# wzx99/DCFP

Measured on AMD Instinct MI355X. Metric: training images/sec at 1024x2048 DeepLabv3-R101, higher is better.
Workload: dtype f32; 1 GPU; DeepLabv3-resnet101+ASPP os8, 4x3x1024x2048 per GPU, CE+0.4*deepsup CE (fused upsample), 3x3 stride-1 convs with >= 256 channels as fp32 Winograd F(2x2,3x3) (fwd / dgrad / wgrad), all other convs direct implicit GEMM, EIC step, SGD m0.9 wd5e-4; global_batch=4, parallelism=dp1

## Files before the change

### dcfp_amd/_lib.py

```python
import ctypes as C
import os
import subprocess
import threading

_HERE = os.path.dirname(os.path.abspath(__file__))
LIB_PATH = os.environ.get("DCFP_LIB") or os.path.join(_HERE, "libdcfp_hip.so")
CSRC = os.path.join(_HERE, "csrc")

_lib = None
_lock = threading.Lock()


class ConvDesc(C.Structure):
    _fields_ = [(n, C.c_int32) for n in
                ("N", "Cin", "H", "W", "Cout", "KH", "KW", "stride", "pad", "dil", "Hout", "Wout",
                 "x_pitch", "dy_pitch")]


class ConvF16Desc(C.Structure):
    _fields_ = [(n, C.c_int32) for n in
                ("N", "H", "W", "Cin8", "x_pitch", "Cout", "K", "stride", "pad", "dil", "Hout", "Wout",
                 "y_pitch", "y_off", "res_pitch", "res_off", "relu")]


class ConvF8Desc(C.Structure):
    _fields_ = [(n, C.c_int32) for n in
                ("N", "H", "W", "Cin16", "x_pitch", "Cout", "K", "stride", "pad", "dil", "Hout", "Wout",
                 "y_pitch", "y_off", "res_pitch", "res_off", "relu")] + [("res_mul", C.c_float)]


class EicEntry(C.Structure):
    _fields_ = [("gamma", C.c_void_p), ("grad", C.c_void_p), ("eic", C.c_void_p),
                ("n", C.c_int32), ("pad_", C.c_int32)]


class SgdEntry(C.Structure):
    _fields_ = [("param", C.c_void_p), ("grad", C.c_void_p), ("momentum_buf", C.c_void_p),
                ("n", C.c_int64), ("first_chunk", C.c_int64),
                ("weight_decay", C.c_float), ("pad_", C.c_int32)]


class GateEntry(C.Structure):
    _fields_ = [("gamma", C.c_void_p), ("beta", C.c_void_p), ("ggrad", C.c_void_p), ("bgrad", C.c_void_p),
                ("score", C.c_void_p), ("n", C.c_int32), ("pad_", C.c_int32)]


class FilterEntry(C.Structure):
    _fields_ = [("w", C.c_void_p), ("g", C.c_void_p), ("out", C.c_void_p), ("rows", C.c_int32), ("K", C.c_int32),
                ("first_unit", C.c_int64)]


class FpgmEntry(C.Structure):
    _fields_ = [("w", C.c_void_p), ("out", C.c_void_p), ("C", C.c_int32), ("K", C.c_int32),
                ("first_tile", C.c_int64), ("ws_off", C.c_int64)]


class AdamEntry(C.Structure):
    _fields_ = [("param", C.c_void_p), ("grad", C.c_void_p), ("exp_avg", C.c_void_p), ("exp_avg_sq", C.c_void_p),
                ("n", C.c_int64), ("first_chunk", C.c_int64)]


class BnRunning(C.Structure):
    _fields_ = [("running_mean", C.c_void_p), ("running_var", C.c_void_p), ("num_batches_tracked", C.c_void_p),
                ("momentum", C.c_float), ("pad_", C.c_int32)]


class WpEntry(C.Structure):
    _fields_ = [("w", C.c_void_p), ("wp", C.c_void_p), ("first_block", C.c_int64), ("n_blocks", C.c_int64)] + \
               [(n, C.c_int32) for n in ("T", "Ck", "CkP", "M", "Mpad", "sAm", "sAc", "perm8")]


class AugTap(C.Structure):
    _fields_ = [(n, C.c_int32) for n in ("src", "c0", "c1", "lsrc")]


class AugSample(C.Structure):
    _fields_ = [("image", C.c_void_p), ("label", C.c_void_p)] + \
               [(n, C.c_int32) for n in ("src_h", "src_w", "col_off", "row_off", "lut_a_off", "lut_b_off",
                                         "hsv_flags", "hue_delta")] + \
               [("sat_alpha", C.c_float), ("pad_", C.c_int32)]


class CcSample(C.Structure):
    _fields_ = [("label", C.c_void_p)] + \
               [(n, C.c_int32) for n in ("src_h", "src_w", "dst_h", "dst_w", "Hp", "Wp", "row_off", "col_off", "cls",
                                         "pad_")] + \
               [("work_off", C.c_int64)]


class VoteMap(C.Structure):
    _fields_ = [("logits", C.c_void_p)] + [(n, C.c_int32) for n in ("h", "w", "hs", "ws", "flip")] + \
               [("weight", C.c_float)]


class SlidePass(C.Structure):
    _fields_ = [("logits", C.c_void_p)] + \
               [(n, C.c_int32) for n in ("lh", "lw", "hs", "ws", "th", "tw", "rows", "cols", "flip")] + \
               [("weight", C.c_float)]


class EngineInfo(C.Structure):
    _fields_ = [(n, C.c_int32) for n in ("format", "num_classes", "in_channels", "align_corner", "model", "n_records",
                                         "n_buffers", "n_slots", "has_input_table")]


SLIDE_MAX_PASSES, SLIDE_MAX_TILES_PER_AXIS = 16, 32
AUG_SATURATION, AUG_HUE = 1, 2
SGD_CHUNK = 16384
FILTER_ABS_SUM, FILTER_L2, FILTER_DOT_SQ_ACC = 0, 1, 2
FPGM_TILE = 64
CONV_FWD, CONV_DGRAD, CONV_WGRAD = 0, 1, 2
E_BADDESC, E_UNSUPPORTED, E_WORKSPACE = -1, -2, -3

_P, _I, _L, _F, _Z = C.c_void_p, C.c_int, C.c_int64, C.c_float, C.c_size_t
_D = C.POINTER(ConvDesc)
_R = C.POINTER(BnRunning)
_H = C.POINTER(ConvF16Desc)
_H8 = C.POINTER(ConvF8Desc)

SIGNATURES = {
    "dcfp_abi_version": (_I, []),
    "dcfp_conv2d_workspace_bytes": (_Z, [_D, _I]),
    "dcfp_conv2d_wp_layout": (_I, [_D, _I, C.POINTER(WpEntry)]),
    "dcfp_conv2d_permute_weights_multi_f32": (_I, [_P, _I, _L, _P]),
    "dcfp_conv2d_pitch_supported": (_I, [_D]),
    "dcfp_conv2d_kernel_name": (_I, [_D, _I, C.c_char_p, _I]),
    "dcfp_conv2d_executed_fraction": (C.c_double, [_D, _I]),
    "dcfp_conv2d_workspace_is_scratch": (_I, [_D, _I]),
    "dcfp_conv2d_dgrad_fanin_supported": (_I, [_D]),
    "dcfp_conv2d_dgrad_fanin_f32_nchw": (_I, [_D, _P, _L, _P, _P, _P, _P, _P, _Z, _I, _P]),
    "dcfp_conv2d_dgrad_fanin_red_slots": (_L, [_D]),
    "dcfp_conv2d_dgrad_fanin_red_f32_nchw": (_I, [_D, _P, _L, _P, _P, _P, _P, _P, _P, _P, _P, _P, _Z, _I, _P]),
    "dcfp_bn_bwd_sums_from_partials_f32": (_I, [_P, _L, _I, _P, _F, _P, _P, _P, _P, _P]),
    "dcfp_conv2d_xform_bytes": (_Z, [_D]),
    "dcfp_conv2d_fwd_keep_f32_nchw": (_I, [_D, _P, _P, _P, _L, _P, _Z, _P, _P, _Z, _P]),
    "dcfp_conv2d_wgrad_kept_f32_nchw": (_I, [_D, _P, _L, _P, _Z, _P, _P, _Z, _P]),
    "dcfp_conv2d_fwd_f32_nchw": (_I, [_D, _P, _P, _P, _P, _L, _P, _Z, _I, _P]),
    "dcfp_conv2d_fwd_fused_f32_nchw": (_I, [_D, _P, _P, _P, _P, _P, _I, _P, _P, _Z, _I, _P]),
    "dcfp_conv2d_dgrad_f32_nchw": (_I, [_D, _P, _L, _P, _P, _I, _P, _Z, _I, _P]),
    "dcfp_conv2d_wgrad_f32_nchw": (_I, [_D, _P, _L, _P, _P, _P, _P, _Z, _P]),
    "dcfp_bn_workspace_bytes": (_Z, [_I, _I, _I]),
    "dcfp_bn_stats_f32": (_I, [_P, _L, _I, _I, _I, _P, _P, _R, _P, _Z, _P]),
    "dcfp_bn_apply_f32": (_I, [_P, _P, _P, _P, _P, _F, _P, _I, _P, _L, _I, _I, _I, _I, _I, _P]),
    "dcfp_bn_bwd_reduce_f32": (_I, [_P, _L, _P, _P, _L, _P, _P, _P, _P, _F, _I, _I, _I, _I, _P, _P, _P, _P,
                                    _P, _Z, _P]),
    "dcfp_bn_update_running_f32": (_I, [_P, _P, _I, _F, _F, _P, _P, _P, _P]),
    "dcfp_syncbn_combine_f32": (_I, [_P, _I, _I, _P, _P, _P, _R, _P]),
    "dcfp_syncbn_p2p_mailbox_bytes": (_Z, [_I, _I]),
    "dcfp_p2p_alloc": (_I, [_Z, _I, C.POINTER(C.c_void_p)]),
    "dcfp_p2p_free": (_I, [_P]),
    "dcfp_p2p_export": (_I, [_P, _P]),
    "dcfp_p2p_import": (_I, [_P, C.POINTER(C.c_void_p)]),
    "dcfp_p2p_unmap": (_I, [_P]),
    "dcfp_syncbn_p2p_exchange_f32": (_I, [C.POINTER(C.c_void_p), _I, _I, C.c_uint32, _I, _P, _I, _I, _P, _R,
                                          C.c_uint32, _P, _P]),
    "dcfp_bn_apply_relu_mask_f32": (_I, [_P, _P, _P, _P, _P, _F, _P, _P, _P, _I, _I, _I, _P]),
    "dcfp_conv2d_fwd_stat_slots": (_L, [_D, _P, _L]),
    "dcfp_conv2d_fwd_stats_f32_nchw": (_I, [_D, _P, _P, _P, _L, _P, _P, _Z, _I, _P]),
    "dcfp_bn_stats_from_partials_f32": (_I, [_P, _L, _I, _I, _P, _P, _R, _P]),
    "dcfp_bn_bwd_apply_f32": (_I, [_P, _L, _P, _P, _L, _P, _P, _P, _P, _F, _P, _P, _F, _P, _I, _P, _P,
                                   _I, _I, _I, _I, _I, _P]),
    "dcfp_bn_bwd_fused_sync_bytes": (_Z, [_I, _I, _I]),
    "dcfp_bn_bwd_fused_f32": (_I, [_P, _L, _P, _P, _L, _P, _P, _P, _P, _F, _F, _I, _P, _P, _I, _I, _I, _I, _I,
                                   _P, _P, _P, _P, _P, _Z, C.c_uint32, C.c_uint32, _P, _P]),
    "dcfp_maxpool3x3s2_fwd_f32": (_I, [_P, _P, _P, _I, _I, _I, _I, _I, _I, _P]),
    "dcfp_maxpool3x3s2_bwd_f32": (_I, [_P, _P, _P, _I, _I, _I, _I, _I, _I, _P]),
    "dcfp_rowsum_f32": (_I, [_P, _L, _P, _F, _I, _I, _I, _P]),
    "dcfp_broadcast_hw_f32": (_I, [_P, _F, _P, _L, _I, _I, _I, _I, _P]),
    "dcfp_add_f32": (_I, [_P, _P, _P, _L, _P]),
    "dcfp_channel_scale_f32": (_I, [_P, _P, _P, _I, _I, _I, _P]),
    "dcfp_upsample_bilinear_fwd_f32": (_I, [_P, _P, _I, _I, _I, _I, _I, _I, _I, _P]),
    "dcfp_upsample_bilinear_bwd_f32": (_I, [_P, _P, _I, _I, _I, _I, _I, _I, _I, _P]),
    "dcfp_resize_bilinear_into_f32": (_I, [_P, _L, _I, _I, _I, _I, _P, _L, _I, _I, _I, _I, _P]),
    "dcfp_resize_bilinear_adjoint_f32": (_I, [_P, _L, _I, _I, _I, _I, _I, _P, _L, _I, _I, _I, _I, _P]),
    "dcfp_ppm_pool_f32": (_I, [_P, _I, _I, _I, _I, _I, _P, _P, _I, _P, _L, _I, _P]),
    "dcfp_ppm_pool_adjoint_f32": (_I, [_P, _I, _I, _I, _I, _I, _P, _P, _L, _I, _P, _P]),
    "dcfp_ppm_resize_adjoint_f32": (_I, [_P, _L, _I, _I, _I, _I, _I, _P, _P, _I, _P]),
    "dcfp_upsample_ce_workspace_bytes": (_Z, [_I, _I, _I]),
    "dcfp_upsample_ce_fwd_f32": (_I, [_P, _P, _P, _I, _I, _I, _I, _I, _I, _I, _I, _P, _P, _P, _P,
                                      _Z, _P]),
    "dcfp_upsample_ce_bwd_f32": (_I, [_P, _P, _P, _I, _I, _I, _I, _I, _I, _I, _I, _P, _P, _P, _P]),
    "dcfp_upsample_ce_bwd_plan": (_I, [_I, _I, _I, _I, _I, _I, C.POINTER(C.c_int), C.POINTER(C.c_int),
                                       C.POINTER(C.c_int)]),
    "dcfp_ohem_zoom_gt_prob_f32": (_I, [_P, _P, _P, _I, _I, _I, _I, _I, _I, _I, _I, _I, _P, _P, _P]),
    "dcfp_ohem_threshold_f32": (_I, [_P, _P, _L, _I, _F, _L, _P, _P]),
    "dcfp_ohem_keep_mask_u8": (_I, [_P, _P, _L, _P, _P]),
    "dcfp_upsample_margin_f32": (_I, [_P, _I, _I, _I, _I, _I, _I, _I, _P, _P]),
    "dcfp_maxfilter2d_s1_f32": (_I, [_P, _P, _I, _I, _I, _I, _P]),
    "dcfp_upsample_wce_workspace_bytes": (_Z, [_I, _I, _I]),
    "dcfp_upsample_wce_fwd_f32": (_I, [_P, _P, _P, _I, _I, _I, _I, _I, _I, _I, _I, _P, _P, _P, _Z, _P]),
    "dcfp_upsample_wce_bwd_f32": (_I, [_P, _P, _P, _I, _I, _I, _I, _I, _I, _I, _I, _P, _P, _P, _P]),
    "dcfp_upsample_argmax_f32": (_I, [_P, _I, _I, _I, _I, _I, _I, _I, _P, _P]),
    "dcfp_confusion_matrix_i64": (_I, [_P, _P, _I, _L, _I, _P, _P]),
    "dcfp_vote_multiscale_f32": (_I, [C.POINTER(VoteMap), _I, _I, _I, _I, _I, _I, _I, _I, _P, _P, _P, _I, _P, _P]),
    "dcfp_gather_tiles_f32": (_I, [_P, _I, _I, _I, _I, _P, _I, _P, _I, _I, _I, _I, _P, _P]),
    "dcfp_vote_sliding_f32": (_I, [C.POINTER(SlidePass), _I, _P, _P, _I, _I, _I, _I, _I, _I, _I, _P, _P, _P, _I, _P, _P]),
    "dcfp_label_boundary_workspace_bytes": (_Z, [_I, _I, _I]),
    "dcfp_label_boundary_i32": (_I, [_P, _P, _I, _I, _I, _I, _I, _I, _P, _Z, _P]),
    "dcfp_label_boundary_i64": (_I, [_P, _P, _I, _I, _I, _I, _I, _I, _P, _Z, _P]),
    "dcfp_png_deflate_bound": (_Z, [_I, _I]),
    "dcfp_png_deflate_workspace_bytes": (_Z, [_I, _I, _I, _I]),
    "dcfp_png_deflate_labels_i32": (_I, [_P, _I, _I, _I, _P, _I, _P, _Z, _P, _P, _P, _Z, _P]),
    "dcfp_augment_u8_to_f32_nchw": (_I, [C.POINTER(AugSample), _I, _I, _I, _P, _L, _P, _L, _P, _L, _P, _I, _P, _P, _P, _P]),
    "dcfp_balance_weight_f32": (_I, [_P, _P, _P, _I, _L, _I, _I, _I, C.c_double, _P, _P]),
    "dcfp_components_workspace_bytes": (_Z, [_I, _I]),
    "dcfp_label_components_u8": (_I, [C.POINTER(CcSample), _I, _P, _L, _P, _P, _Z, _P, _P]),
    "dcfp_component_pixel_i32": (_I, [C.POINTER(CcSample), _I, _P, _Z, _P, _P, _P, _P, _P]),
    "dcfp_eic_update_f32": (_I, [_P, _I, _F, _F, _P]),
    "dcfp_sgd_momentum_f32": (_I, [_P, _I, _L, _F, _F, _I, _P]),
    "dcfp_adamw_f32": (_I, [_P, _I, _L, _F, _F, _F, _F, _F, _F, _F, _P]),
    "dcfp_conv2d_fwd_f16_nhwc": (_I, [_H, _P, _P, _P, _P, _P, _P]),
    "dcfp_conv2d_fwd_f16_nhwc_to_f32_nchw": (_I, [_H, _P, _P, _P, _P, _P]),
    "dcfp_maxpool3x3s2_nhwc_f16": (_I, [_P, _P, _I, _I, _I, _I, _I, _I, _I, _I, _P]),
    "dcfp_avgpool_nhwc_f16_workspace_bytes": (_Z, [_I, _I, _L]),
    "dcfp_avgpool_nhwc_f16": (_I, [_P, _P, _I, _L, _I, _I, _I, _P, _Z, _P]),
    "dcfp_broadcast_nhwc_f16": (_I, [_P, _I, _P, _I, _L, _I, _I, _I, _P]),
    "dcfp_nchw_f32_to_nhwc_f16": (_I, [_P, _P, _I, _I, _I, _I, _I, _P]),
    "dcfp_conv2d_fwd_f8_nhwc": (_I, [_H8, _P, _P, _P, _P, _P, _P, _P]),
    "dcfp_conv2d_fwd_f8_nhwc_to_f32_nchw": (_I, [_H8, _P, _P, _P, _P, _P, _P]),
    "dcfp_cast_nhwc_f16_to_f8": (_I, [_P, _I, _P, _I, _I, _L, _I, _F, _P]),
    "dcfp_maxpool3x3s2_nhwc_f8": (_I, [_P, _P, _I, _I, _I, _I, _I, _I, _I, _I, _P]),
    "dcfp_avgpool_nhwc_f8_to_f16": (_I, [_P, _P, _I, _L, _I, _I, _I, _F, _P, _Z, _P]),
    "dcfp_broadcast_nhwc_f16_to_f8": (_I, [_P, _I, _P, _I, _L, _I, _I, _I, _F, _P]),
    "dcfp_resize_bilinear_nhwc_f16": (_I, [_P, _I, _I, _I, _I, _I, _P, _I, _I, _I, _I, _I, _P]),
    "dcfp_pyramid_pool_nhwc_f16_workspace_bytes": (_Z, [_I, _I, _I, _I, _I, _P]),
    "dcfp_pyramid_pool_nhwc_f16": (_I, [_P, _I, _I, _I, _I, _I, _I, _I, _P, _P, _P, _P, _Z, _P]),
    "dcfp_kd_workspace_bytes": (_Z, [_I, _I, _I, _I, _I]),
    "dcfp_kd_fwd_f32": (_I, [_P, _P, _I, _I, _I, _I, _I, _F, _P, _Z, _P, _P, _P]),
    "dcfp_pairwise_workspace_bytes": (_Z, [_I, _I, _I, _I, _I, _I, _I]),
    "dcfp_pairwise_fwd_f32": (_I, [_P, _P, _I, _L, _I, _I, _I, _I, _I, _I, _P, _Z, _P, _I, _P]),
    "dcfp_pairwise_bwd_f32": (_I, [_I, _I, _I, _I, _I, _I, _P, _Z, _P, _P, _P]),
    "dcfp_lovasz_workspace_bytes": (_Z, [_I, _I]),
    "dcfp_lovasz_hist_f32": (_I, [_P, _P, _I, _I, _I, _I, _I, _I, _I, _I, _I, _P, _P, _Z, _P]),
    "dcfp_lovasz_scan_f32": (_I, [_I, _I, _P, _Z, _P, _P, _P]),
    "dcfp_lovasz_bwd_f32": (_I, [_P, _P, _I, _I, _I, _I, _I, _I, _I, _I, _I, _P, _P, _P, _P, _P, _P]),
    "dcfp_lovasz_errors_u32": (_I, [_P, _P, _I, _I, _I, _I, _I, _I, _I, _I, _P, _P]),
    "dcfp_gate_taylor_f32": (_I, [_P, _I, _P]),
    "dcfp_gate_l1reg_f32": (_I, [_P, _I, _F, _P]),
    "dcfp_filter_reduce_units": (_L, [_I, _I]),
    "dcfp_filter_reduce_f32": (_I, [_P, _I, _L, _I, _P]),
    "dcfp_fpgm_workspace_bytes": (_Z, [_I]),
    "dcfp_fpgm_f32": (_I, [_P, _I, _L, _P, _Z, _P]),
    "dcfp_engine_open": (_I, [C.c_char_p, C.POINTER(_P), C.c_char_p, _Z]),
    "dcfp_engine_open_memory": (_I, [_P, _Z, C.POINTER(_P), C.c_char_p, _Z]),
    "dcfp_engine_close": (None, [_P]),
    "dcfp_engine_info": (_I, [_P, C.POINTER(EngineInfo)]),
    "dcfp_engine_weight_bytes": (_Z, [_P]),
    "dcfp_engine_upload": (_I, [_P, _P, _P]),
    "dcfp_engine_output_shape": (_I, [_P, _I, _I, _I, C.POINTER(_I), C.POINTER(_I), C.POINTER(_I)]),
    "dcfp_engine_buffer_shapes": (_I, [_P, _I, _I, C.POINTER(_I), _I]),
    "dcfp_engine_workspace_bytes": (_Z, [_P, _I, _I, _I]),
    "dcfp_engine_run_f32": (_I, [_P, _P, _P, _I, _I, _I, _P, _Z, _P, _P]),
    "dcfp_engine_run_u8": (_I, [_P, _P, _P, _Z, _I, _I, _I, _P, _Z, _P, _P]),
    "dcfp_image_u8_hwc_to_nhwc_f16": (_I, [_P, _Z, _I, _I, _I, _P, C.POINTER(_I), _P, _I, _P]),
}


def build(verbose=False):
    cmd = ["make", "-C", CSRC, "-j", str(min(8, os.cpu_count() or 1))]
    r = subprocess.run(cmd, capture_output=True, text=True)
    if verbose or r.returncode != 0:
        print(r.stdout[-4000:])
        print(r.stderr[-4000:])
    if r.returncode != 0:
        raise RuntimeError("building libdcfp_hip.so failed")
    return LIB_PATH


def lib():
    global _lib
    if _lib is not None:
        return _lib
    with _lock:
        if _lib is not None:
            return _lib
        if not os.path.exists(LIB_PATH):
            raise RuntimeError(
                f"{LIB_PATH} not found: run `python -c 'import __graft_entry__ as g; g.build()'` "
                "(or `make -C dcfp_amd/csrc`). dcfp_amd has no non-HIP fallback.")
        try:
            import torch
        except Exception:
            pass
        handle = C.CDLL(LIB_PATH, mode=C.RTLD_GLOBAL)
        for name, (res, args) in SIGNATURES.items():
            fn = getattr(handle, name)
            fn.restype = res
            fn.argtypes = args
        _lib = handle
    return _lib


def check(status, what):
    if status != 0:
        kind = "descriptor/shape" if status < 0 else "hipError_t"
        raise RuntimeError(f"{what} failed: status {status} ({kind})")
```

### dcfp_amd/csrc/conv_dispatch.h

```cpp
#pragma once
#include "common.h"
#include <stdlib.h>
#include <string.h>

struct Igemm2Params;

inline int check_desc(const DcfpConvDesc* d) {
    if (!d) return DCFP_E_BADDESC;
    if (d->N <= 0 || d->Cin <= 0 || d->Cout <= 0 || d->H <= 0 || d->W <= 0 || d->stride <= 0 ||
        d->dil <= 0 || d->pad < 0)
        return DCFP_E_BADDESC;
    if (d->KH != d->KW || (d->KH != 1 && d->KH != 3)) return DCFP_E_UNSUPPORTED;
    const int ho = (d->H + 2 * d->pad - d->dil * (d->KH - 1) - 1) / d->stride + 1;
    const int wo = (d->W + 2 * d->pad - d->dil * (d->KW - 1) - 1) / d->stride + 1;
    if (ho != d->Hout || wo != d->Wout || ho <= 0 || wo <= 0) return DCFP_E_BADDESC;
    if ((d->x_pitch != 0 && (d->x_pitch < d->W || (d->x_pitch & 3))) ||
        (d->dy_pitch != 0 && (d->dy_pitch < d->Wout || (d->dy_pitch & 3))))
        return DCFP_E_BADDESC;
    if ((long long)d->Cin * d->H * (d->x_pitch ? d->x_pitch : d->W) >= (1LL << 29) ||
        (long long)d->Cout * d->Hout * (d->dy_pitch ? d->dy_pitch : d->Wout) >= (1LL << 29) ||
        (long long)d->Cout * d->Cin * d->KH * d->KW >= (1LL << 29))
        return DCFP_E_UNSUPPORTED;
    return DCFP_OK;
}

inline bool same_size_3x3(const DcfpConvDesc* d) {
    return d->KH == 3 && d->KW == 3 && d->stride == 1 && d->pad == d->dil && d->Hout == d->H && d->Wout == d->W;
}

inline bool math_bf16x3() {
    static const bool v = [] { const char* e = getenv("DCFP_CONV_MATH"); return e && !strcmp(e, "bf16x3"); }();
    return v;
}
inline int conv_winograd_mode() {
    static const int v = [] { const char* e = getenv("DCFP_CONV_WINOGRAD"); return e ? atoi(e) : 1; }();
    return v;
}
inline bool igemm_dma_on() {
    static const bool v = [] { const char* e = getenv("DCFP_IGEMM_DMA"); return !e || atoi(e) != 0; }();
    return v;
}
inline int igemm_2d_mode() {
    static const int v = [] { const char* e = getenv("DCFP_IGEMM_2D"); return e ? atoi(e) : 5; }();
    return v;
}
inline int wino_fused_mode() {
    static const int v = [] { const char* e = getenv("DCFP_WINO_FUSED"); return e ? atoi(e) : 1; }();
    return v;
}
inline int wino_wgrad_fused_mode() {
    static const int v = [] { const char* e = getenv("DCFP_WINO_WGRAD_FUSED"); return e ? atoi(e) : 1; }();
    return v;
}
inline bool wgrad_dma_on() {
    static const bool v = [] { const char* e = getenv("DCFP_WGRAD_DMA"); return !e || atoi(e) != 0; }();
    return v;
}

struct GemmProblem {
    int T, M, Ck, N, Hi, Wi, Ho, Wo, sn, sd, off0, offstep;
    int in_pitch;
    int sAm, sAc;
    long long in_nstride, out_nstride;
    int P() const { return Ho * Wo; }
    long long px() const { return (long long)N * Ho * Wo; }
    int HiWi() const { return Hi * Wi; }
    bool pitched() const { return in_pitch > 0 && in_pitch != Wi; }
};

inline GemmProblem gemm_problem(const DcfpConvDesc* d, int pass, long long nstride_override) {
    GemmProblem g;
    g.T = d->KH * d->KW; g.N = d->N;
    if (pass == DCFP_CONV_FWD) {
        g.M = d->Cout; g.Ck = d->Cin; g.Hi = d->H; g.Wi = d->W; g.Ho = d->Hout; g.Wo = d->Wout;
        g.sn = d->stride; g.sd = 1; g.off0 = -d->pad; g.offstep = d->dil;
        g.in_pitch = d->x_pitch; g.sAm = d->Cin * g.T; g.sAc = g.T;
        g.in_nstride = (long long)d->Cin * d->H * (d->x_pitch ? d->x_pitch : d->W);
        g.out_nstride = nstride_override ? nstride_override : (long long)d->Cout * d->Hout * d->Wout;
    } else {
        g.M = d->Cin; g.Ck = d->Cout; g.Hi = d->Hout; g.Wi = d->Wout; g.Ho = d->H; g.Wo = d->W;
        g.sn = 1; g.sd = d->stride; g.off0 = d->pad; g.offstep = -d->dil;
        g.in_pitch = d->dy_pitch; g.sAm = g.T; g.sAc = d->Cin * g.T;
        g.in_nstride = nstride_override ? nstride_override
                                        : (long long)d->Cout * d->Hout * (d->dy_pitch ? d->dy_pitch : d->Wout);
        g.out_nstride = (long long)d->Cin * d->H * d->W;
    }
    return g;
}

struct WinoProblem {
    int N, H, W, d, M, Ck;
    long long in_nstride;
    int in_pitch;
};
inline WinoProblem wino_problem(const GemmProblem& g) {
    return {g.N, g.Ho, g.Wo, g.offstep < 0 ? -g.offstep : g.offstep, g.M, g.Ck, g.in_nstride, g.in_pitch};
}

struct GemmExtras {
    const float* bias = nullptr;
    const float* scale = nullptr;
    const float* shift = nullptr;
    const float* residual = nullptr;
    int relu = 0;
    float* stat_part = nullptr;
    int accumulate = 0;
    int wp_valid = 0;
    long long wp_nstride = 0;
    const float* fan_src = nullptr;
    const unsigned long long* fan_mask = nullptr;
    const Igemm2Red* red = nullptr;
    float* xform_out = nullptr;
};

enum Igemm2Family { IGEMM2_TILE, IGEMM2_DMA, IGEMM2_DMA1P, IGEMM2_DMA8 };
struct Igemm2Route {
    int family;
    int cfg, bm, bn;
    bool dma_shape;
    bool mixed;
    int Mpad, CkP, tile2d;
    int tiles_per_img, tiles_n_total, tiles_m;
    int Hc, Wc, tiles_per_phase, zfold;
};
Igemm2Route igemm2_route(const GemmProblem& g, const GemmExtras& x, bool vec_store);
int dcfp_igemm2_run(const GemmProblem& g, const float* in, const float* w, float* out, void* workspace, size_t workspace_bytes,
                    const GemmExtras& x, hipStream_t stream);
size_t dcfp_igemm2_workspace_bytes(const GemmProblem& g);
int dcfp_igemm2_cfg_id(const GemmProblem& g);
const char* dcfp_igemm2_cfg_args(const GemmProblem& g);
bool dcfp_igemm2_dma_shape(const GemmProblem& g);
bool dcfp_igemm2_use_dma8(const GemmProblem& g);
double dcfp_igemm2_exec_fraction(const GemmProblem& g);
void dcfp_igemm2_wp_layout(const GemmProblem& g, DcfpWpEntry* e);
long long dcfp_igemm2_stat_slots(const GemmProblem& g, const float* out);
bool dcfp_igemm2_persist();
int dcfp_igemm2_ck_pad();
int dcfp_igemm2_permute_multi(const DcfpWpEntry* table, int n, long long total_blocks, hipStream_t stream);
int dcfp_igemm2n_launch(const Igemm2Params& p, int T, hipStream_t stream);
int dcfp_igemm2p_launch(const Igemm2Params& p, hipStream_t stream);
bool dcfp_igemm2p_fan_red_ok(int Mpad, int CkP);

size_t dcfp_igemm3_workspace_bytes(int T, int M, int Ck);
int dcfp_igemm3_run(const GemmProblem& g, const float* in, const float* w, float* out, void* workspace, size_t workspace_bytes,
                    const GemmExtras& x, hipStream_t stream);

bool dcfp_wino_ok(const WinoProblem& q);
size_t dcfp_wino_workspace_bytes(const WinoProblem& q);
double dcfp_wino_exec_fraction(const WinoProblem& q);
long long dcfp_wino_stat_slots(const WinoProblem& q);
size_t dcfp_wino_xform_bytes(const WinoProblem& q);
int dcfp_wino_run(const GemmProblem& g, const float* in, const float* w, float* out, void* workspace, size_t workspace_bytes,
                  const GemmExtras& x, hipStream_t stream);
bool dcfp_wino_fused_ok(const WinoProblem& q);
size_t dcfp_wino_fused_workspace_bytes(const WinoProblem& q);
void dcfp_wino_fused_pads(const WinoProblem& q, int* CkP, int* Mpad);
int dcfp_wino_fused_run(const GemmProblem& g, const float* in, const float* w, float* out, void* workspace,
                        size_t workspace_bytes, const GemmExtras& x, hipStream_t stream);
bool dcfp_wino_wgrad_ok(int N, int H, int W, int d, int M, int C);
size_t dcfp_wino_wgrad_workspace_bytes(int N, int H, int W, int d, int M, int C);
int dcfp_wino_wgrad_run(const float* dy, long long dy_nstride, int dy_pitch, const float* x, long long x_nstride,
                        int x_pitch, float* dw, int N, int M, int C, int H, int W, int d, void* workspace,
                        size_t workspace_bytes, hipStream_t stream, const float* xform_in);
bool dcfp_wino_wgrad_fused_ok(int N, int H, int W, int d, int M, int C, long long x_nstride, int x_pitch,
                              long long dy_nstride, int dy_pitch);
size_t dcfp_wino_wgrad_fused_workspace_bytes(int N, int H, int W, int d, int M, int C);
int dcfp_wino_wgrad_fused_run(const float* dy, long long dy_nstride, int dy_pitch, const float* x, long long x_nstride,
                              int x_pitch, float* dw, int N, int M, int C, int H, int W, int d, void* workspace,
                              size_t workspace_bytes, hipStream_t stream);

bool dcfp_stem_shape(const DcfpConvDesc* d);
long long dcfp_stem_stat_slots(const DcfpConvDesc* d, const float* y, long long y_nstride);
int dcfp_stem_fwd(const DcfpConvDesc* d, const float* x, const float* w, float* y, long long y_nstride, const GemmExtras& ex,
                  hipStream_t stream);
size_t dcfp_stem_wgrad_workspace_bytes(const DcfpConvDesc* d);
int dcfp_stem_wgrad(const DcfpConvDesc* d, const float* dy, long long dy_nstride, const float* x, float* dw, void* workspace,
                    size_t workspace_bytes, hipStream_t stream);
bool dcfp_gemv_shape(const DcfpConvDesc* d);
int dcfp_gemv_fwd(const DcfpConvDesc* d, const float* x, const float* w, const float* bias, float* y, long long y_nstride,
                  hipStream_t stream);
int dcfp_gemv_dgrad(const DcfpConvDesc* d, const float* dy, long long dy_nstride, const float* w, float* dx, int accumulate,
                    hipStream_t stream);
int dcfp_gemv_wgrad(const DcfpConvDesc* d, const float* dy, long long dy_nstride, const float* x, float* dw, hipStream_t stream);

int dcfp_wgrad_kernel_name(const DcfpConvDesc* d, char* buf, int buf_len);
double dcfp_wgrad_exec_fraction(const DcfpConvDesc* d);
bool dcfp_wgrad_is_winograd(const DcfpConvDesc* d);
bool dcfp_wgrad_wants_xform(const DcfpConvDesc* d);
bool dcfp_wgrad_pitch_ok(const DcfpConvDesc* d);
size_t dcfp_wgrad_batched_workspace_bytes(int batch, int M, int C, long long K, int* splits_out);
int dcfp_wgrad_batched_run(const float* a, const float* bmat, float* out, int batch, int M, int C, long long K,
                           void* workspace, size_t workspace_bytes, hipStream_t stream);
int dcfp_wgrad3_launch(const float* dy, long long dy_nstride, const float* x, long long x_nstride,
                       float* out, int N, int M, int Cin, int T, int H, int W, int Ho, int Wo, int pad,
                       int dil, int Kpix, int kchunk, int splits, int tiles_m, int tiles_n,
                       hipStream_t stream);
size_t dcfp_conv2d_fwd_dgrad_workspace_bytes_(const DcfpConvDesc* d, int pass);
```

### dcfp_amd/csrc/conv_igemm.hip

```cpp
#include "conv_dispatch.h"
#include <stdio.h>

extern "C" int dcfp_abi_version(void) { return 2; }

static bool igemm3_ok(const GemmProblem& g) {
    return math_bf16x3() && g.sn == 1 && g.sd == 1 && dcfp_igemm2_cfg_id(g) == 4;
}

static int wino_kind(const DcfpConvDesc* d, int pass) {
    const int mode = conv_winograd_mode();
    if (mode == 0 || !same_size_3x3(d) || math_bf16x3()) return 0;
    const bool fwd = pass == DCFP_CONV_FWD;
    const GemmProblem g = gemm_problem(d, pass, 0);
    const WinoProblem q = wino_problem(g);
    const int M = g.M, Ck = g.Ck;
    const bool three = dcfp_wino_ok(q), fused = dcfp_wino_fused_ok(q);
    if (!three && !fused) return 0;
    if (mode == 2) return three ? 1 : 2;
    const double nominal = 2.0 * d->N * (double)d->H * d->W * (double)M * Ck * 9.0;
    const double f_direct = dcfp_igemm2_exec_fraction(g);
    const double t_direct = nominal * f_direct / (M % 256 != 0 ? 115e12 : 143e12);
    const double f_wino = dcfp_wino_exec_fraction(q);
    double t_wino = 1e30;
    if (three) {
        const double tiles = f_wino * 9.0 / 16.0 * d->N * (double)d->H * d->W;
        const double rate = Ck <= 256 ? (M >= 1024 ? 130e12 : 118e12) : (M <= 256 ? 127e12 : 135e12);
        const double pix = (double)d->N * d->H * d->W;
        const double t_in = (4.0 * pix * Ck + 64.0 * tiles * Ck) / 4.2e12;
        const double t_out = (64.0 * tiles * M + 4.0 * pix * M * (fwd ? 1.0 : 2.0)) / 5.4e12;
        const double mpad = (double)((M + 255) / 256 * 256) / M;
        t_wino = nominal * f_wino * mpad / rate + t_in + t_out + 20e-6;
    }
    if (fused) {
        const double nk = (double)((Ck + 15) / 16 * 2);
        const double mpad = (double)((M + 63) / 64 * 64) / M;
        const double t_f = nominal * f_wino * mpad / (125e12 * nk / (nk + 4.0)) + 10e-6;
        if (t_f < t_wino) t_wino = t_f;
    }
    if (!(t_wino < 0.97 * t_direct)) return 0;
    return three ? 1 : 2;
}
static bool wino_pass(const DcfpConvDesc* d, int pass) { return wino_kind(d, pass) != 0; }

static bool wino_keeps_u(const DcfpConvDesc* d, int pass) {
    static const bool on = [] { const char* e = getenv("DCFP_WINO_KEEP_U"); return !e || atoi(e) != 0; }();
    if (!on || (pass != DCFP_CONV_FWD && pass != DCFP_CONV_DGRAD) || !wino_pass(d, pass)) return false;
    const WinoProblem q = wino_problem(gemm_problem(d, pass, 0));
    if (!dcfp_wino_fused_ok(q)) return false;
    if (pass == DCFP_CONV_FWD && q.Ck > 256 && dcfp_wino_ok(q) && dcfp_conv2d_xform_bytes(d) > 0) return false;
    return true;
}

extern "C" int dcfp_conv2d_workspace_is_scratch(const DcfpConvDesc* d, int pass) {
    if (check_desc(d) != DCFP_OK || pass == DCFP_CONV_WGRAD) return 0;
    return (wino_pass(d, pass) && !wino_keeps_u(d, pass)) ? 1 : 0;
}

size_t dcfp_conv2d_fwd_dgrad_workspace_bytes_(const DcfpConvDesc* d, int pass) {
    if (check_desc(d) != DCFP_OK) return 0;
    const GemmProblem g = gemm_problem(d, pass, 0);
    if (const int wk = wino_kind(d, pass)) {
        const WinoProblem q = wino_problem(g);
        if (wino_keeps_u(d, pass)) {
            const size_t u = dcfp_wino_fused_workspace_bytes(q), direct = dcfp_igemm2_workspace_bytes(g);
            return u > direct ? u : direct;
        }
        return wk == 1 ? dcfp_wino_workspace_bytes(q) : dcfp_wino_fused_workspace_bytes(q);
    }
    const size_t b2 = dcfp_igemm2_workspace_bytes(g);
    const size_t b3 = igemm3_ok(g) ? dcfp_igemm3_workspace_bytes(g.T, g.M, g.Ck) : 0;
    return b2 > b3 ? b2 : b3;
}

extern "C" int dcfp_conv2d_kernel_name(const DcfpConvDesc* d, int pass, char* buf, int buf_len) {
    int rc = check_desc(d);
    if (rc) return rc;
    if (!buf || buf_len <= 0) return DCFP_E_BADDESC;
    if (dcfp_gemv_shape(d)) return snprintf(buf, buf_len, "gemv_1x1_map_kernel");
    if (pass == DCFP_CONV_WGRAD) return dcfp_wgrad_kernel_name(d, buf, buf_len);
    if (pass == DCFP_CONV_FWD && dcfp_stem_shape(d)) return snprintf(buf, buf_len, "stem_fwd_kernel");
    if (const int wk = wino_kind(d, pass))
        return wk == 1 ? snprintf(buf, buf_len, "winograd_f2x2_3x3 (igemm2_dma1p_kernel<false,true>)")
                       : snprintf(buf, buf_len, "winograd_f2x2_3x3 fused (wino_fused_kernel)");
    const GemmProblem g = gemm_problem(d, pass, 0);
    if (igemm3_ok(g)) return snprintf(buf, buf_len, "igemm3_kernel<%d>", g.T);
    const Igemm2Route r = igemm2_route(g, GemmExtras(), true);
    switch (r.family) {
        case IGEMM2_DMA8: return snprintf(buf, buf_len, "igemm2_dma8_kernel<%d>", g.T);
        case IGEMM2_DMA1P: return snprintf(buf, buf_len, "igemm2_dma1p_kernel");
        case IGEMM2_DMA: return snprintf(buf, buf_len, "igemm2_dma_kernel<%d,%s>", g.T, r.mixed ? "true" : "false");
        default: return snprintf(buf, buf_len, "igemm2_kernel<%d,%s>", g.T, dcfp_igemm2_cfg_args(g));
    }
}

extern "C" double dcfp_conv2d_executed_fraction(const DcfpConvDesc* d, int pass) {
    if (check_desc(d) != DCFP_OK) return 1.0;
    if (pass == DCFP_CONV_WGRAD) return dcfp_wgrad_exec_fraction(d);
    const GemmProblem g = gemm_problem(d, pass, 0);
    if (wino_pass(d, pass)) return dcfp_wino_exec_fraction(wino_problem(g));
    if (igemm3_ok(g)) return 1.0;
    return dcfp_igemm2_exec_fraction(g);
}

extern "C" size_t dcfp_conv2d_xform_bytes(const DcfpConvDesc* d) {
    if (check_desc(d) != DCFP_OK) return 0;
    if (!wino_pass(d, DCFP_CONV_FWD) || !dcfp_wgrad_wants_xform(d)) return 0;
    return dcfp_wino_xform_bytes(wino_problem(gemm_problem(d, DCFP_CONV_FWD, 0)));
}

static int wino_wp_valid(const DcfpConvDesc* d, int pass, int wp_valid) { return (wp_valid && wino_keeps_u(d, pass)) ? 1 : 0; }

extern "C" int dcfp_conv2d_fwd_keep_f32_nchw(const DcfpConvDesc* d, const float* x, const float* w, float* y,
                                             int64_t y_nstride, float* xform_out, size_t xform_bytes,
                                             float* stat_partials, void* workspace, size_t workspace_bytes,
                                             dcfp_stream_t stream) {
    int rc = check_desc(d);
    if (rc) return rc;
    if (!x || !w || !y || !xform_out) return DCFP_E_BADDESC;
    const size_t need = dcfp_conv2d_xform_bytes(d);
    if (need == 0) return DCFP_E_UNSUPPORTED;
    if (xform_bytes < need) return DCFP_E_WORKSPACE;
    GemmExtras ex;
    ex.xform_out = xform_out;
    if (stat_partials && dcfp_conv2d_fwd_stat_slots(d, y, y_nstride) > 0) ex.stat_part = stat_partials;
    return dcfp_wino_run(gemm_problem(d, DCFP_CONV_FWD, y_nstride), x, w, y, workspace, workspace_bytes, ex, dcfp_s(stream));
}

extern "C" int dcfp_conv2d_fwd_f32_nchw(const DcfpConvDesc* d, const float* x, const float* w,
                                        const float* bias, float* y, int64_t y_nstride,
                                        void* workspace, size_t workspace_bytes, int wp_valid,
                                        dcfp_stream_t stream) {
    int rc = check_desc(d);
    if (rc) return rc;
    if (!x || !w || !y) return DCFP_E_BADDESC;
    const GemmProblem g = gemm_problem(d, DCFP_CONV_FWD, y_nstride);
    if (g.pitched() && math_bf16x3()) return DCFP_E_UNSUPPORTED;
    GemmExtras ex;
    ex.bias = bias; ex.wp_valid = wp_valid;
    if (dcfp_gemv_shape(d)) return dcfp_gemv_fwd(d, x, w, bias, y, y_nstride, dcfp_s(stream));
    if (dcfp_stem_shape(d)) return dcfp_stem_fwd(d, x, w, y, y_nstride, ex, dcfp_s(stream));
    if (!bias && wino_pass(d, DCFP_CONV_FWD)) {
        ex.wp_valid = wino_wp_valid(d, DCFP_CONV_FWD, wp_valid);
        return dcfp_wino_run(g, x, w, y, workspace, workspace_bytes, ex, dcfp_s(stream));
    }
    if (!bias && igemm3_ok(g)) return dcfp_igemm3_run(g, x, w, y, workspace, workspace_bytes, ex, dcfp_s(stream));
    return dcfp_igemm2_run(g, x, w, y, workspace, workspace_bytes, ex, dcfp_s(stream));
}

extern "C" int64_t dcfp_conv2d_fwd_stat_slots(const DcfpConvDesc* d, const float* y, int64_t y_nstride) {
    if (check_desc(d) != DCFP_OK) return 0;
    if (dcfp_stem_shape(d)) return dcfp_stem_stat_slots(d, y, y_nstride);
    const GemmProblem g = gemm_problem(d, DCFP_CONV_FWD, y_nstride);
    if (wino_pass(d, DCFP_CONV_FWD))
        return (y_nstride % 4 == 0 && dcfp_aligned16(y)) ? dcfp_wino_stat_slots(wino_problem(g)) : 0;
    if (igemm3_ok(g)) return 0;
    return dcfp_igemm2_stat_slots(g, y);
}

extern "C" int dcfp_conv2d_fwd_stats_f32_nchw(const DcfpConvDesc* d, const float* x, const float* w,
                                              float* y, int64_t y_nstride, float* stat_partials,
                                              void* workspace, size_t workspace_bytes, int wp_valid,
                                              dcfp_stream_t stream) {
    int rc = check_desc(d);
    if (rc) return rc;
    if (!x || !w || !y || !stat_partials) return DCFP_E_BADDESC;
    if (dcfp_conv2d_fwd_stat_slots(d, y, y_nstride) <= 0) return DCFP_E_UNSUPPORTED;
    const GemmProblem g = gemm_problem(d, DCFP_CONV_FWD, y_nstride);
    GemmExtras ex;
    ex.stat_part = stat_partials; ex.wp_valid = wp_valid;
    if (dcfp_stem_shape(d)) return dcfp_stem_fwd(d, x, w, y, y_nstride, ex, dcfp_s(stream));
    if (wino_pass(d, DCFP_CONV_FWD)) {
        ex.wp_valid = wino_wp_valid(d, DCFP_CONV_FWD, wp_valid);
        return dcfp_wino_run(g, x, w, y, workspace, workspace_bytes, ex, dcfp_s(stream));
    }
    return dcfp_igemm2_run(g, x, w, y, workspace, workspace_bytes, ex, dcfp_s(stream));
}

extern "C" int dcfp_conv2d_dgrad_f32_nchw(const DcfpConvDesc* d, const float* dy,
                                          int64_t dy_nstride, const float* w, float* dx,
                                          int accumulate, void* workspace, size_t workspace_bytes,
                                          int wp_valid, dcfp_stream_t stream) {
    int rc = check_desc(d);
    if (rc) return rc;
    if (!dy || !w || !dx) return DCFP_E_BADDESC;
    const GemmProblem g = gemm_problem(d, DCFP_CONV_DGRAD, dy_nstride);
    if (g.pitched() && math_bf16x3()) return DCFP_E_UNSUPPORTED;
    GemmExtras ex;
    ex.accumulate = accumulate ? 1 : 0; ex.wp_valid = wp_valid;
    if (dcfp_gemv_shape(d)) return dcfp_gemv_dgrad(d, dy, dy_nstride, w, dx, ex.accumulate, dcfp_s(stream));
    if (wino_pass(d, DCFP_CONV_DGRAD)) {
        ex.wp_valid = wino_wp_valid(d, DCFP_CONV_DGRAD, wp_valid);
        return dcfp_wino_run(g, dy, w, dx, workspace, workspace_bytes, ex, dcfp_s(stream));
    }
    if (igemm3_ok(g)) return dcfp_igemm3_run(g, dy, w, dx, workspace, workspace_bytes, ex, dcfp_s(stream));
    return dcfp_igemm2_run(g, dy, w, dx, workspace, workspace_bytes, ex, dcfp_s(stream));
}

extern "C" int dcfp_conv2d_dgrad_fanin_supported(const DcfpConvDesc* d) {
    if (check_desc(d) != DCFP_OK || d->KH != 1 || d->stride != 1 || d->pad != 0 || math_bf16x3()) return 0;
    const GemmProblem g = gemm_problem(d, DCFP_CONV_DGRAD, 0);
    if (g.M % 256 != 0 || g.P() % 256 != 0 || !dcfp_igemm2_persist()) return 0;
    if (igemm3_ok(g)) return 0;
    return dcfp_igemm2_dma_shape(g) ? 1 : 0;
}

extern "C" int dcfp_conv2d_dgrad_fanin_f32_nchw(const DcfpConvDesc* d, const float* dy, int64_t dy_nstride, const float* w,
                                                float* dx, const float* fan_src, const void* fan_mask, void* workspace,
                                                size_t workspace_bytes, int wp_valid, dcfp_stream_t stream) {
    int rc = check_desc(d);
    if (rc) return rc;
    if (!dy || !w || !dx || !fan_src || !fan_mask) return DCFP_E_BADDESC;
    if (!dcfp_conv2d_dgrad_fanin_supported(d)) return DCFP_E_UNSUPPORTED;
    GemmExtras ex;
    ex.wp_valid = wp_valid; ex.fan_src = fan_src; ex.fan_mask = static_cast<const unsigned long long*>(fan_mask);
    return dcfp_igemm2_run(gemm_problem(d, DCFP_CONV_DGRAD, dy_nstride), dy, w, dx, workspace, workspace_bytes, ex, dcfp_s(stream));
}

extern "C" int64_t dcfp_conv2d_dgrad_fanin_red_slots(const DcfpConvDesc* d) {
    if (!dcfp_conv2d_dgrad_fanin_supported(d)) return 0;
    const GemmProblem g = gemm_problem(d, DCFP_CONV_DGRAD, 0);
    const Igemm2Route r = igemm2_route(g, GemmExtras(), true);
    if (!dcfp_igemm2p_fan_red_ok(r.Mpad, r.CkP)) return 0;
    return g.px() / 128;
}

extern "C" int dcfp_conv2d_dgrad_fanin_red_f32_nchw(const DcfpConvDesc* d, const float* dy, int64_t dy_nstride,
                                                    const float* w, float* dx, const float* fan_src, const void* fan_mask,
                                                    const float* red_x, const void* red_mask, const float* red_mean,
                                                    float* red_part, void* workspace, size_t workspace_bytes, int wp_valid,
                                                    dcfp_stream_t stream) {
    int rc = check_desc(d);
    if (rc) return rc;
    if (!dy || !w || !dx || !fan_src || !fan_mask || !red_x || !red_mask || !red_mean || !red_part) return DCFP_E_BADDESC;
    if (dcfp_conv2d_dgrad_fanin_red_slots(d) <= 0) return DCFP_E_UNSUPPORTED;
    if (reinterpret_cast<uintptr_t>(red_part) & 7u) return DCFP_E_BADDESC;
    const Igemm2Red red = {red_x, static_cast<const unsigned long long*>(red_mask), red_mean, red_part};
    GemmExtras ex;
    ex.wp_valid = wp_valid; ex.fan_src = fan_src; ex.fan_mask = static_cast<const unsigned long long*>(fan_mask);
    ex.red = &red;
    return dcfp_igemm2_run(gemm_problem(d, DCFP_CONV_DGRAD, dy_nstride), dy, w, dx, workspace, workspace_bytes, ex, dcfp_s(stream));
}

extern "C" int dcfp_conv2d_fwd_fused_f32_nchw(const DcfpConvDesc* d, const float* x, const float* w,
                                              const float* scale, const float* shift,
                                              const float* residual, int relu, float* y,
                                              void* workspace, size_t workspace_bytes, int wp_valid,
                                              dcfp_stream_t stream) {
    int rc = check_desc(d);
    if (rc) return rc;
    if (!x || !w || !y || !scale || !shift) return DCFP_E_BADDESC;
    const GemmProblem g = gemm_problem(d, DCFP_CONV_FWD, 0);
    GemmExtras ex;
    ex.scale = scale; ex.shift = shift; ex.residual = residual; ex.relu = relu ? 1 : 0;
    if (wino_pass(d, DCFP_CONV_FWD))
        return dcfp_wino_run(g, x, w, y, workspace, workspace_bytes, ex, dcfp_s(stream));
    ex.wp_valid = wp_valid;
    if (igemm3_ok(g)) return dcfp_igemm3_run(g, x, w, y, workspace, workspace_bytes, ex, dcfp_s(stream));
    return dcfp_igemm2_run(g, x, w, y, workspace, workspace_bytes, ex, dcfp_s(stream));
}

extern "C" int dcfp_conv2d_wp_layout(const DcfpConvDesc* d, int pass, DcfpWpEntry* e) {
    int rc = check_desc(d);
    if (rc) return rc;
    if (!e || (pass != DCFP_CONV_FWD && pass != DCFP_CONV_DGRAD)) return DCFP_E_BADDESC;
    const GemmProblem g = gemm_problem(d, pass, 0);
    if (wino_pass(d, pass)) {
        if (!wino_keeps_u(d, pass)) return DCFP_E_UNSUPPORTED;
        e->T = 16; e->M = g.M; e->Ck = g.Ck;
        dcfp_wino_fused_pads(wino_problem(g), &e->CkP, &e->Mpad);
        e->sAm = g.sAm; e->sAc = g.sAc; e->perm8 = pass == DCFP_CONV_FWD ? 2 : 3;
        const long long pairs = (long long)e->CkP * e->Mpad;
        e->n_blocks = (pairs + DCFP_WP_BLOCK_ELEMS - 1) / DCFP_WP_BLOCK_ELEMS;
        return DCFP_OK;
    }
    if (igemm3_ok(g)) return DCFP_E_UNSUPPORTED;
    dcfp_igemm2_wp_layout(g, e);
    const long long total = (long long)e->T * e->CkP * e->Mpad;
    e->n_blocks = (total + DCFP_WP_BLOCK_ELEMS - 1) / DCFP_WP_BLOCK_ELEMS;
    return DCFP_OK;
}

extern "C" int dcfp_conv2d_permute_weights_multi_f32(const DcfpWpEntry* table, int n, int64_t total_blocks,
                                                     dcfp_stream_t stream) {
    if (n == 0 || total_blocks == 0) return DCFP_OK;
    if (!table || n < 0 || total_blocks < 0 || total_blocks > 0x7fffffffLL) return DCFP_E_BADDESC;
    return dcfp_igemm2_permute_multi(table, n, total_blocks, dcfp_s(stream));
}

extern "C" int dcfp_conv2d_pitch_supported(const DcfpConvDesc* d) {
    if (check_desc(d) != DCFP_OK || math_bf16x3() || !same_size_3x3(d)) return 0;
    const int xp = d->x_pitch ? d->x_pitch : d->W, dp = d->dy_pitch ? d->dy_pitch : d->Wout;
    if (xp < d->W + d->pad && xp != d->W) return 0;
    if (dp < d->Wout + d->pad && dp != d->Wout) return 0;
    if (xp != d->W && dp != d->Wout && wino_kind(d, DCFP_CONV_FWD) == 2 && wino_kind(d, DCFP_CONV_DGRAD) == 2)
        return dcfp_wgrad_pitch_ok(d) ? 1 : 0;
    for (const int pass : {DCFP_CONV_FWD, DCFP_CONV_DGRAD}) {
        GemmProblem g = gemm_problem(d, pass, 0);
        if (!g.pitched()) g.in_pitch = g.Wi + 4;
        if (igemm2_route(g, GemmExtras(), true).family == IGEMM2_TILE) return 0;
    }
    return dcfp_wgrad_pitch_ok(d) ? 1 : 0;
}
```

### dcfp_amd/csrc/conv_wgrad.hip

```cpp
#include "conv_dispatch.h"
#include <stdio.h>
#include <type_traits>

namespace {

typedef float f32x16 __attribute__((ext_vector_type(16)));

constexpr int BK = 16;
constexpr int BKP = 20;

struct WgradParams {
    const float* dy;
    const float* x;
    float* out;
    long long dy_nstride, x_nstride;
    int N, M, Cin, Nn;
    int H, W, Ho, Wo, P, stride, pad, dil;
    int Kpix;
    int kchunk, splits, tiles_m, tiles_n;
    int quad_ok;
    int x_pitch, dy_pitch;
    int batch;
    long long dy_bstride, x_bstride;
};
// ... 571 lines not shown
        static_for<0, TM>([&](auto i_) {
            constexpr int i = decltype(i_)::value;
            af[0][i] = *reinterpret_cast<const f32x4*>(a + i * 32 * BK + f0);
        });
        static_for<0, TN>([&](auto j_) {
            constexpr int j = decltype(j_)::value;
            bf[0][j] = *reinterpret_cast<const f32x4*>(b + j * 32 * BK + f0);
        });
        static_for<0, 8>([&](auto s_) {
            constexpr int s = decltype(s_)::value;
            constexpr int kq = s / 4, e = s % 4;
            static_for<0, TM>([&](auto i_) {
                constexpr int i = decltype(i_)::value;
                static_for<0, TN>([&](auto j_) {
                    constexpr int j = decltype(j_)::value;
                    constexpr int n = i * TN + j;
                    if (!WIDE || i < nb)
                        acc[i][j] = __builtin_amdgcn_mfma_f32_32x32x2f32(af[kq][i][e], bf[kq][j][e], acc[i][j], 0, 0, 0);
                    if constexpr (s == 0 && n == 0) {
                        static_for<0, TM>([&](auto i2_) {
                            constexpr int i2 = decltype(i2_)::value;
                            af[1][i2] = *reinterpret_cast<const f32x4*>(a + i2 * 32 * BK + f1);
                        });
                        static_for<0, TN>([&](auto j2_) {
                            constexpr int j2 = decltype(j2_)::value;
                            bf[1][j2] = *reinterpret_cast<const f32x4*>(b + j2 * 32 * BK + f1);
                        });
                    }
                    if constexpr (TAPS == 1 && !MIXED) {
                        if constexpr (s == 0 && n == 1) {
                            if (more) issue1(cur ^ 1);
                            __builtin_amdgcn_sched_barrier(0);
                        }
                    } else if constexpr (s == 0 && (n & 1) == 1) {
                        if (more) {
                            constexpr int piece = n / 2;
                            if constexpr (piece < 4) issue_a(cur ^ 1, std::integral_constant<int, piece>{});
                            else issue_b(cur ^ 1, std::integral_constant<int, piece - 4>{});
                            if constexpr (piece == 7) advance();
                        }
                        __builtin_amdgcn_sched_barrier(0);
                    }
                });
            });
            __builtin_amdgcn_sched_barrier(0);
        });
        retire();
    }

    float* o = p.out + ((long long)split * p.batch + bi) * p.M * p.Nn;
    int ncol = n0 + wn * (TN * 32) + l31;
    asm volatile("" : "+v"(ncol));
#pragma unroll
    for (int i = 0; i < TM; ++i) {
#pragma unroll
        for (int r = 0; r < 16; ++r) {
            const int row = (r & 3) + 8 * (r >> 2) + 4 * lhi;
            const int m = m0 + wm * (TM * 32) + i * 32 + row;
            if (m >= p.M) continue;
#pragma unroll
            for (int j = 0; j < TN; ++j) {
                const int nn = ncol + j * 32;
                if (nn < p.Nn) o[(long long)m * p.Nn + nn] = acc[i][j][r];
            }
        }
    }
}

struct Plan {
    int bm, bn, cfg;
    int tiles_m, tiles_n, splits, kchunk;
    bool wide;
    bool half;
};

bool dma_geometry(const DcfpConvDesc* d) {
    return wgrad_dma_on() && d->stride == 1 && d->Hout == d->H && d->Wout == d->W && d->W % 16 == 0;
}

Plan make_plan(const DcfpConvDesc* d) {
    Plan pl;
    const int M = d->Cout, Nn = d->Cin * d->KH * d->KW;
    static const bool lopsided = [] { const char* e = getenv("DCFP_WGRAD_LOPSIDED"); return !e || atoi(e) != 0; }();
    if (M > 128 && Nn > 128) { pl.cfg = 0; pl.bm = 256; pl.bn = 256; }
    else if (M > 64 && Nn > 128) {
        pl.cfg = 1; pl.bm = 128; pl.bn = 256;
        static const bool t192 = [] { const char* e = getenv("DCFP_WGRAD_T192"); return !e || atoi(e) != 0; }();
        if (t192 && (Nn + 191) / 192 * 192 < (Nn + 255) / 256 * 256) { pl.cfg = 5; pl.bn = 192; }
    }
    else if (lopsided && M > 128 && Nn > 64) { pl.cfg = 3; pl.bm = 256; pl.bn = 128; }
    else if (lopsided && M > 128 && Nn > 32) { pl.cfg = 4; pl.bm = 256; pl.bn = 64; }
    else { pl.cfg = 2; pl.bm = 64; pl.bn = 64; }
    pl.wide = false;
    {
        static const int mode = [] { const char* e = getenv("DCFP_WGRAD_WIDE"); return e ? atoi(e) : 1; }();
        const bool mixed = d->KH == 3 && ((d->pad | d->dil) & 3) != 0;
        const bool x_pitched = d->x_pitch && d->x_pitch != d->W;
        const bool eligible = mode != 0 && !math_bf16x3() && dma_geometry(d) && Nn > 128 && (!mixed || x_pitched) &&
                              !(d->KH == 3 && d->pad != d->dil);
        if (eligible) {
            const long long old_rows = (long long)((M + pl.bm - 1) / pl.bm) * pl.bm, new_rows = (long long)((M + 31) / 32) * 32;
            const bool narrow = d->KH == 3 && M <= 128 && Nn <= 1152;
            if (mode == 2 || (!narrow && (pl.cfg != 0 || (M % pl.bm != 0 && 10 * new_rows <= 9 * old_rows)))) {
                pl.wide = true; pl.cfg = 0; pl.bm = 256; pl.bn = 256;
            }
        }
    }
    pl.half = false;
    {
        static const bool on = [] { const char* e = getenv("DCFP_WGRAD_HALF"); return !e || atoi(e) != 0; }();
        if (on && pl.cfg == 0 && !pl.wide && d->KH == 1 && M % 128 == 0 && !math_bf16x3() && dma_geometry(d)) {
            pl.half = true; pl.bm = 128;
        }
    }
    pl.tiles_m = (M + pl.bm - 1) / pl.bm;
    pl.tiles_n = (Nn + pl.bn - 1) / pl.bn;
    const long long tiles = (long long)pl.tiles_m * pl.tiles_n;
    const long long Kpix = (long long)d->N * d->Hout * d->Wout;
    const int cus = num_cus();
    const long long per_cu = pl.cfg == 2 ? 8 : (pl.cfg == 0 && !pl.half) ? 1 : 2;
    const long long slots = (long long)cus * per_cu;
    const long long max_splits = (Kpix + BK * 8 - 1) / (BK * 8);
    long long splits = 1;
    if (const char* e = getenv("DCFP_DBG_WGRAD_BLOCKS")) {
        splits = (atoll(e) + tiles - 1) / tiles;
    } else {
        double best = -1.0;
        for (long long sp = 1; sp <= max_splits && tiles * sp <= 4 * slots; ++sp) {
            const long long blocks = tiles * sp;
            const long long rounds = (blocks + slots - 1) / slots;
            double eff = (double)blocks / (double)(rounds * slots);
            if (blocks < slots) eff *= 0.999;
            if (eff > best + 0.02) { best = eff; splits = sp; }
        }
    }
    if (splits > max_splits) splits = max_splits;
    if (splits < 1) splits = 1;
    long long kchunk = (Kpix + splits - 1) / splits;
    kchunk = (kchunk + BK - 1) / BK * BK;
    splits = (Kpix + kchunk - 1) / kchunk;
    pl.splits = (int)splits;
    pl.kchunk = (int)kchunk;
    return pl;
}

static bool wgrad3_ok(const DcfpConvDesc* d, int cfg) {
    return math_bf16x3() && cfg == 0 && d->stride == 1 && (d->Wout % 4 == 0);
}


template <int TAPS, int TM, int TN, int WM, int WN>
int launch_cfg(const WgradParams& p, long long blocks, hipStream_t stream) {
    constexpr int BM = WM * TM * 32, BN = WN * TN * 32, NT = 64 * WM * WN;
    const size_t lds = (size_t)2 * (BM + BN) * BKP * sizeof(float);
    auto kern = wgrad2_kernel<TAPS, TM, TN, WM, WN>;
    if (lds > 64 * 1024) {
        hipError_t e = hipFuncSetAttribute(reinterpret_cast<const void*>(kern),
                                           hipFuncAttributeMaxDynamicSharedMemorySize, (int)lds);
        if (e != hipSuccess) return (int)e;
    }
    hipLaunchKernelGGL(kern, dim3((unsigned)blocks), dim3(NT), lds, stream, p);
    DCFP_RETURN_LAUNCH();
}

static bool wgrad_dma_ok(const DcfpConvDesc* d, int cfg) {
    static const bool mixed_too = [] { const char* e = getenv("DCFP_WGRAD_DMA_MIXED"); return !e || atoi(e) != 0; }();
    const bool mixed = d->KH == 3 && ((d->pad | d->dil) & 3) != 0;
    return cfg == 0 && dma_geometry(d) && (!mixed || mixed_too);
}
static bool wgrad_dma_mixed(const DcfpConvDesc* d) { return d->KH == 3 && ((d->pad | d->dil) & 3) != 0; }

template <int TAPS, bool MIXED, bool WIDE = false, bool BATCH = false, bool HALF = false>
int launch_dma(const WgradParams& p, long long blocks, hipStream_t stream) {
    const size_t lds = (size_t)2 * (HALF ? 384 : 512) * BK * sizeof(float);
    hipLaunchKernelGGL((wgrad_dma_kernel<TAPS, MIXED, WIDE, BATCH, HALF>), dim3((unsigned)blocks), dim3(256), lds, stream, p);
    DCFP_RETURN_LAUNCH();
}

template <int TAPS>
int launch_taps(const WgradParams& p, const Plan& pl, hipStream_t stream) {
    const long long blocks = (long long)pl.tiles_m * pl.tiles_n * pl.splits;
    if (blocks > 0x7fffffffLL) return DCFP_E_UNSUPPORTED;
    switch (pl.cfg) {
        case 0: return launch_cfg<TAPS, 4, 4, 2, 2>(p, blocks, stream);
        case 1: return launch_cfg<TAPS, 2, 4, 2, 2>(p, blocks, stream);
        case 3: return launch_cfg<TAPS, 4, 2, 2, 2>(p, blocks, stream);
        case 4: return launch_cfg<TAPS, 4, 1, 2, 2>(p, blocks, stream);
        case 5: return launch_cfg<TAPS, 2, 3, 2, 2>(p, blocks, stream);
        default: return launch_cfg<TAPS, 2, 2, 1, 1>(p, blocks, stream);
    }
}

}

static void launch_splitk_reduce(const float* slabs, float* out, long long wn, int splits, hipStream_t stream) {
    if (wn % 4 == 0 && dcfp_aligned16(slabs) && dcfp_aligned16(out)) {
        const long long n4 = wn / 4;
        hipLaunchKernelGGL(splitk_reduce_vec4_kernel, dim3((unsigned)((n4 + 255) / 256)), dim3(256), 0, stream, slabs, out, n4, wn,
                           splits);
    } else {
        long long b = (wn + 255) / 256;
        if (b > 4096) b = 4096;
        hipLaunchKernelGGL(splitk_reduce_kernel, dim3((unsigned)b), dim3(256), 0, stream, slabs, out, wn, splits);
    }
}

struct WgradOperands { int xp, dyp; long long xn, dyn; };
static WgradOperands wgrad_operands(const DcfpConvDesc* d, long long dy_nstride) {
    WgradOperands o;
    o.xp = d->x_pitch ? d->x_pitch : d->W;
    o.dyp = d->dy_pitch ? d->dy_pitch : d->Wout;
    o.xn = (long long)d->Cin * d->H * o.xp;
    o.dyn = dy_nstride ? dy_nstride : (long long)d->Cout * d->Hout * o.dyp;
    return o;
}

bool dcfp_wgrad_pitch_ok(const DcfpConvDesc* d) {
    if (check_desc(d) != DCFP_OK) return false;
    const Plan pl = make_plan(d);
    if (wgrad3_ok(d, pl.cfg)) return false;
    const int xp = wgrad_operands(d, 0).xp;
    if (xp != d->W && (d->KH != 3 || d->pad != d->dil || xp < d->W + d->pad)) return false;
    return true;
}

size_t dcfp_wgrad_batched_workspace_bytes(int batch, int M, int C, long long K, int* splits_out) {
    const long long tiles = (long long)((M + 255) / 256) * ((C + 255) / 256) * batch;
    const long long slots = num_cus();
    long long max_splits = K / (BK * 8);
    if (max_splits < 1) max_splits = 1;
    long long splits = 1;
    double best = -1.0;
    for (long long sp = 1; sp <= max_splits && tiles * sp <= 4 * slots; ++sp) {
        const long long blocks = tiles * sp, rounds = (blocks + slots - 1) / slots;
        double eff = (double)blocks / (double)(rounds * slots);
        if (blocks < slots) eff *= 0.999;
        if (eff > best + 0.02) { best = eff; splits = sp; }
    }
    long long kchunk = (K + splits - 1) / splits;
    kchunk = (kchunk + BK - 1) / BK * BK;
    splits = (K + kchunk - 1) / kchunk;
    if (splits_out) *splits_out = (int)splits;
    return splits > 1 ? (size_t)splits * batch * M * C * sizeof(float) : 0;
}

int dcfp_wgrad_batched_run(const float* a, const float* bmat, float* out, int batch, int M, int C, long long K,
                           void* workspace, size_t workspace_bytes, hipStream_t stream) {
    if (K % BK != 0 || K <= 0 || K >= (1LL << 30) || (long long)M * K >= (1LL << 29) || (long long)C * K >= (1LL << 29))
        return DCFP_E_UNSUPPORTED;
    int splits = 1;
    const size_t need = dcfp_wgrad_batched_workspace_bytes(batch, M, C, K, &splits);
    if (need && (!workspace || workspace_bytes < need || !dcfp_aligned16(workspace))) return DCFP_E_WORKSPACE;
    WgradParams p;
    p.dy = a; p.x = bmat;
    p.out = splits > 1 ? static_cast<float*>(workspace) : out;
    p.x_pitch = (int)K; p.dy_pitch = (int)K;
    p.dy_nstride = (long long)M * K; p.x_nstride = (long long)C * K;
    p.N = 1; p.M = M; p.Cin = C; p.Nn = C;
    p.H = 1; p.W = (int)K; p.Ho = 1; p.Wo = (int)K; p.P = (int)K;
    p.stride = 1; p.pad = 0; p.dil = 1;
    p.Kpix = (int)K;
    long long kchunk = (K + splits - 1) / splits;
    kchunk = (kchunk + BK - 1) / BK * BK;
    p.kchunk = (int)kchunk; p.splits = splits;
    p.tiles_m = (M + 255) / 256; p.tiles_n = (C + 255) / 256;
    p.quad_ok = 1;
    p.batch = batch; p.dy_bstride = (long long)M * K; p.x_bstride = (long long)C * K;
    const long long blocks = (long long)p.tiles_m * p.tiles_n * splits * batch;
    if (blocks > 0x7fffffffLL) return DCFP_E_UNSUPPORTED;
    const long long mp = (long long)p.tiles_m * 256, live = (long long)((M + 31) / 32) * 32;
    int rc = (M % 256 != 0 && 10 * live <= 9 * mp) ? launch_dma<1, false, true, true>(p, blocks, stream)
                                                   : launch_dma<1, false, false, true>(p, blocks, stream);
    if (rc) return rc;
    if (splits > 1) launch_splitk_reduce(static_cast<const float*>(workspace), out, (long long)batch * M * C, splits, stream);
    DCFP_RETURN_LAUNCH();
}

static bool wino_wgrad_pass(const DcfpConvDesc* d);
static int wino_wgrad_kind(const DcfpConvDesc* d);

int dcfp_wgrad_kernel_name(const DcfpConvDesc* d, char* buf, int buf_len) {
    if (dcfp_stem_shape(d)) return snprintf(buf, buf_len, "stem_wgrad_kernel");
    if (const int wk = wino_wgrad_kind(d))
        return wk == 2 ? snprintf(buf, buf_len, "winograd_f2x2_3x3 wgrad fused (wino_wgrad_fused_kernel)")
                       : snprintf(buf, buf_len, "winograd_f2x2_3x3 wgrad (wgrad_dma_kernel<1,false,false,true>)");
    const Plan pl = make_plan(d);
    const char* args = pl.cfg == 0 ? "4,4,2,2" : pl.cfg == 1 ? "2,4,2,2" : pl.cfg == 3 ? "4,2,2,2" :
                       pl.cfg == 4 ? "4,1,2,2" : pl.cfg == 5 ? "2,3,2,2" : "2,2,1,1";
    if (wgrad3_ok(d, pl.cfg)) return snprintf(buf, buf_len, "wgrad3_kernel<%d>", d->KH * d->KW);
    if (pl.wide) return snprintf(buf, buf_len, "wgrad_dma_kernel<%d,false,true>", d->KH * d->KW);
    if (wgrad_dma_ok(d, pl.cfg))
        return snprintf(buf, buf_len, "wgrad_dma_kernel<%d,%s>", d->KH * d->KW,
                        (wgrad_dma_mixed(d) && !(d->x_pitch && d->x_pitch != d->W)) ? "true" : "false");
    return snprintf(buf, buf_len, "wgrad2_kernel<%d,%s>", d->KH * d->KW, args);
}

static double wino_wgrad_fused_rate() {
    static const double v = [] { const char* e = getenv("DCFP_WINO_WGRAD_RATE"); return (e ? atof(e) : 118.0) * 1e12; }();
    return v;
}
static bool wino_wgrad_fused_forced() { return wino_wgrad_fused_mode() == 2; }

static double wino_fraction(const DcfpConvDesc* d) {
    return dcfp_wino_exec_fraction(wino_problem(gemm_problem(d, DCFP_CONV_FWD, 0)));
}
static int wino_wgrad_kind(const DcfpConvDesc* d) {
    const int mode = conv_winograd_mode();
    if (mode == 0 || !same_size_3x3(d) || math_bf16x3()) return 0;
    const WgradOperands o = wgrad_operands(d, 0);
    const bool batched = dcfp_wino_wgrad_ok(d->N, d->H, d->W, d->dil, d->Cout, d->Cin);
    const bool fused = dcfp_wino_wgrad_fused_ok(d->N, d->H, d->W, d->dil, d->Cout, d->Cin, o.xn, o.xp, o.dyn, o.dyp);
    if (!batched && !fused) return 0;
    if (mode == 2) return fused ? 2 : 1;
    const double pix = (double)d->N * d->H * d->W;
    const double nominal = 2.0 * pix * d->Cout * (double)d->Cin * 9.0;
    const bool dense_d1 = wgrad_dma_mixed(d) && !(d->x_pitch && d->x_pitch != d->W);
    const bool ragged = d->Cout % 256 != 0 || (d->Cin * 9) % 256 != 0;
    const double dpad = ragged ? (double)((d->Cout + 31) / 32 * 32) / d->Cout * (double)((d->Cin * 9 + 255) / 256 * 256) / (d->Cin * 9) * 1.15
                               : 1.0;
    const double t_direct = nominal * dpad / (d->Cout < 128 ? 100e12 : dense_d1 ? 123e12 : 130e12);
    const double f = wino_fraction(d);
    double t_b = 1e30, t_f = 1e30;
    if (batched) {
        const double tiles = f * 9.0 / 16.0 * pix;
        const double pad2 = (double)((d->Cout + 255) / 256 * 256) / d->Cout * (double)((d->Cin + 255) / 256 * 256) / d->Cin;
        t_b = nominal * f * pad2 / 125e12 + (4.0 * pix * d->Cin + 64.0 * tiles * d->Cin) / 4.2e12 +
              (4.0 * pix * d->Cout + 64.0 * tiles * d->Cout) / 5.0e12 + 30e-6;
    }
    if (fused) {
        const double pad64 = (double)((d->Cout + 63) / 64 * 64) / d->Cout * (double)((d->Cin + 63) / 64 * 64) / d->Cin;
        t_f = nominal * f * pad64 / wino_wgrad_fused_rate() + 40e-6;
    }
    if (fused && (t_f <= t_b || wino_wgrad_fused_forced())) return t_f < 0.97 * t_direct ? 2 : 0;
    return t_b < 0.97 * t_direct ? 1 : 0;
}
static bool wino_wgrad_pass(const DcfpConvDesc* d) { return wino_wgrad_kind(d) != 0; }

bool dcfp_wgrad_is_winograd(const DcfpConvDesc* d) { return wino_wgrad_pass(d); }
bool dcfp_wgrad_wants_xform(const DcfpConvDesc* d) { return wino_wgrad_kind(d) == 1; }

double dcfp_wgrad_exec_fraction(const DcfpConvDesc* d) {
    return wino_wgrad_pass(d) ? wino_fraction(d) : 1.0;
}

extern "C" size_t dcfp_conv2d_workspace_bytes(const DcfpConvDesc* d, int pass) {
    if (pass == DCFP_CONV_FWD || pass == DCFP_CONV_DGRAD) return dcfp_conv2d_fwd_dgrad_workspace_bytes_(d, pass);
    if (pass != DCFP_CONV_WGRAD || check_desc(d) != DCFP_OK) return 0;
    if (dcfp_stem_shape(d)) return dcfp_stem_wgrad_workspace_bytes(d);
    if (const int wk = wino_wgrad_kind(d)) {
        const size_t b1 = dcfp_wino_wgrad_ok(d->N, d->H, d->W, d->dil, d->Cout, d->Cin)
                              ? dcfp_wino_wgrad_workspace_bytes(d->N, d->H, d->W, d->dil, d->Cout, d->Cin) : 0;
        if (wk == 1) return b1;
        const size_t b2 = dcfp_wino_wgrad_fused_workspace_bytes(d->N, d->H, d->W, d->dil, d->Cout, d->Cin);
        const Plan pl = make_plan(d);
        const size_t b0 = pl.splits > 1 ? (size_t)pl.splits * d->Cout * d->Cin * d->KH * d->KW * sizeof(float) : 0;
        const size_t m = b1 > b0 ? b1 : b0;
        return b2 > m ? b2 : m;
    }
    const Plan pl = make_plan(d);
    if (pl.splits <= 1) return 0;
    return (size_t)pl.splits * d->Cout * d->Cin * d->KH * d->KW * sizeof(float);
}

extern "C" int dcfp_conv2d_wgrad_f32_nchw(const DcfpConvDesc* d, const float* dy,
                                          int64_t dy_nstride, const float* x, float* dw, float* db,
                                          void* workspace, size_t workspace_bytes,
                                          dcfp_stream_t stream) {
    int rc = check_desc(d);
    if (rc) return rc;
    if (!dy || !x || !dw) return DCFP_E_BADDESC;
    if (dcfp_gemv_shape(d) && !db)
        return dcfp_gemv_wgrad(d, dy, dy_nstride, x, dw, dcfp_s(stream));
    if (dcfp_stem_shape(d) && !db)
        return dcfp_stem_wgrad(d, dy, dy_nstride, x, dw, workspace, workspace_bytes, dcfp_s(stream));
    int wk = wino_wgrad_kind(d);
    const WgradOperands o = wgrad_operands(d, dy_nstride);
    if (wk == 2 && !dcfp_wino_wgrad_fused_ok(d->N, d->H, d->W, d->dil, d->Cout, d->Cin, o.xn, o.xp, o.dyn, o.dyp))
        wk = dcfp_wino_wgrad_ok(d->N, d->H, d->W, d->dil, d->Cout, d->Cin) ? 1 : 0;
    if (wk) {
        if (db && o.dyp != d->Wout) return DCFP_E_UNSUPPORTED;
        if (wk == 2)
            rc = dcfp_wino_wgrad_fused_run(dy, o.dyn, o.dyp, x, o.xn, o.xp, dw, d->N, d->Cout, d->Cin, d->H, d->W, d->dil,
                                           workspace, workspace_bytes, dcfp_s(stream));
        else
            rc = dcfp_wino_wgrad_run(dy, o.dyn, o.dyp, x, o.xn, o.xp, dw, d->N, d->Cout, d->Cin, d->H, d->W, d->dil, workspace,
                                     workspace_bytes, dcfp_s(stream), nullptr);
        if (rc) return rc;
        if (db)
            hipLaunchKernelGGL(bias_grad_kernel, dim3((unsigned)d->Cout), dim3(1024), 0, dcfp_s(stream), dy, o.dyn, db, d->N,
                               d->Hout * d->Wout, (int)((d->Hout * d->Wout) % 4 == 0 && o.dyn % 4 == 0 && dcfp_aligned16(dy)));
        DCFP_RETURN_LAUNCH();
    }
    const Plan pl = make_plan(d);
    const int T = d->KH * d->KW;
    const long long wn = (long long)d->Cout * d->Cin * T;
    const size_t need = pl.splits > 1 ? (size_t)pl.splits * wn * sizeof(float) : 0;
    if (need && (!workspace || workspace_bytes < need)) return DCFP_E_WORKSPACE;
    WgradParams p;
    p.dy = dy; p.x = x;
    p.out = pl.splits > 1 ? static_cast<float*>(workspace) : dw;
    p.x_pitch = o.xp; p.dy_pitch = o.dyp;
    const bool pitched = p.x_pitch != d->W || p.dy_pitch != d->Wout;
    if (pitched && !dcfp_wgrad_pitch_ok(d)) return DCFP_E_UNSUPPORTED;
    if (db && p.dy_pitch != d->Wout) return DCFP_E_UNSUPPORTED;
    p.dy_nstride = o.dyn; p.x_nstride = o.xn;
    p.N = d->N; p.M = d->Cout; p.Cin = d->Cin; p.Nn = d->Cin * T;
    p.H = d->H; p.W = d->W; p.Ho = d->Hout; p.Wo = d->Wout; p.P = d->Hout * d->Wout;
    p.stride = d->stride; p.pad = d->pad; p.dil = d->dil;
    if ((long long)d->N * p.P >= (1LL << 30)) return DCFP_E_UNSUPPORTED;
    p.Kpix = d->N * p.P;
    p.kchunk = pl.kchunk; p.splits = pl.splits; p.tiles_m = pl.tiles_m; p.tiles_n = pl.tiles_n;
    p.quad_ok = (d->Wout % 4 == 0) ? 1 : 0;
    p.batch = 1; p.dy_bstride = p.x_bstride = 0;
    {
        const long long span = (long long)pl.kchunk / p.P + 2;
        const long long big = p.dy_nstride > p.x_nstride ? p.dy_nstride : p.x_nstride;
        if (span * big * 4 >= (1LL << 31)) return DCFP_E_UNSUPPORTED;
    }
    if (wgrad3_ok(d, pl.cfg))
        rc = dcfp_wgrad3_launch(dy, p.dy_nstride, x, p.x_nstride, p.out, d->N, d->Cout, d->Cin, T, d->H, d->W,
                                d->Hout, d->Wout, d->pad, d->dil, p.Kpix, pl.kchunk, pl.splits, pl.tiles_m,
                                pl.tiles_n, dcfp_s(stream));
    else if (pl.wide) {
        const long long blocks = (long long)pl.tiles_m * pl.tiles_n * pl.splits;
        if (blocks > 0x7fffffffLL) return DCFP_E_UNSUPPORTED;
        rc = T == 1 ? launch_dma<1, false, true>(p, blocks, dcfp_s(stream)) : launch_dma<9, false, true>(p, blocks, dcfp_s(stream));
    } else if (wgrad_dma_ok(d, pl.cfg)) {
        const long long blocks = (long long)pl.tiles_m * pl.tiles_n * pl.splits;
        if (blocks > 0x7fffffffLL) return DCFP_E_UNSUPPORTED;
        rc = T == 1 ? (pl.half ? launch_dma<1, false, false, false, true>(p, blocks, dcfp_s(stream)) : launch_dma<1, false>(p, blocks, dcfp_s(stream)))
                    : (wgrad_dma_mixed(d) && p.x_pitch == d->W) ? launch_dma<9, true>(p, blocks, dcfp_s(stream))
                                                                 : launch_dma<9, false>(p, blocks, dcfp_s(stream));
    } else
        rc = T == 1 ? launch_taps<1>(p, pl, dcfp_s(stream)) : launch_taps<9>(p, pl, dcfp_s(stream));
    if (rc) return rc;
    if (pl.splits > 1) launch_splitk_reduce(static_cast<const float*>(workspace), dw, wn, pl.splits, dcfp_s(stream));
    if (db) {
        hipLaunchKernelGGL(bias_grad_kernel, dim3((unsigned)d->Cout), dim3(1024), 0, dcfp_s(stream),
                           dy, p.dy_nstride, db, d->N, p.P,
                           (int)(p.P % 4 == 0 && p.dy_nstride % 4 == 0 && dcfp_aligned16(dy) && p.dy_pitch == d->Wout));
    }
    DCFP_RETURN_LAUNCH();
}

extern "C" int dcfp_conv2d_wgrad_kept_f32_nchw(const DcfpConvDesc* d, const float* dy, int64_t dy_nstride,
                                               const float* xform, size_t xform_bytes, float* dw, void* workspace,
                                               size_t workspace_bytes, dcfp_stream_t stream) {
    int rc = check_desc(d);
    if (rc) return rc;
    if (!dy || !xform || !dw) return DCFP_E_BADDESC;
    const size_t need = dcfp_conv2d_xform_bytes(d);
    if (need == 0) return DCFP_E_UNSUPPORTED;
    if (xform_bytes < need || !dcfp_aligned16(xform)) return DCFP_E_WORKSPACE;
    const WgradOperands o = wgrad_operands(d, dy_nstride);
    return dcfp_wino_wgrad_run(dy, o.dyn, o.dyp, nullptr, 0, 0, dw, d->N, d->Cout, d->Cin, d->H, d->W, d->dil, workspace,
                               workspace_bytes, dcfp_s(stream), xform);
}
```

### dcfp_amd/csrc/conv_winograd.hip

```cpp
#include "igemm2_common.h"
#include "conv_dispatch.h"

namespace {

inline long long align64(long long v) { return (v + 63) / 64 * 64; }

struct WinoPlan {
    int TH, TW;
    long long T;
    long long T16;
    int CkP, Mpad;
    long long u_floats, v_floats, m_floats;
};

WinoPlan wino_plan(int N, int H, int W, int d, int M, int Ck) {
    WinoPlan pl;
    pl.TH = d * ((H + 2 * d - 1) / (2 * d));
    pl.TW = d * ((W + 2 * d - 1) / (2 * d));
    pl.TW = (pl.TW + 3) / 4 * 4;
    pl.T = (long long)N * pl.TH * pl.TW;
    pl.T16 = (pl.T + 15) / 16 * 16;
    pl.CkP = (Ck + dcfp_igemm2_ck_pad() - 1) / dcfp_igemm2_ck_pad() * dcfp_igemm2_ck_pad();
    pl.Mpad = (M + 255) / 256 * 256;
    pl.u_floats = align64(16LL * pl.CkP * pl.Mpad);
    pl.v_floats = align64(16LL * Ck * pl.T16);
    pl.m_floats = align64(16LL * M * pl.T16);
    return pl;
}

__global__ void __launch_bounds__(256) wino_filter_kernel(const float* __restrict__ w, int sAm, int sAc, int flip,
                                                          int M, int Ck, int CkP, int Mpad, float* __restrict__ U) {
    const long long plane = (long long)CkP * Mpad;
    for (long long idx = (long long)blockIdx.x * 256 + threadIdx.x; idx < plane; idx += (long long)gridDim.x * 256) {
        const int c = (int)(idx / Mpad), m = (int)(idx - (long long)c * Mpad);
        float g[9];
        if (m < M && c < Ck) {
            const float* src = w + (long long)m * sAm + (long long)c * sAc;
#pragma unroll
            for (int t = 0; t < 9; ++t) g[t] = src[flip ? 8 - t : t];
        } else {
#pragma unroll
            for (int t = 0; t < 9; ++t) g[t] = 0.f;
        }
        float r[4][3];
#pragma unroll
        for (int k = 0; k < 3; ++k) {
            const float g0 = g[k], g1 = g[3 + k], g2 = g[6 + k];
            r[0][k] = g0;
            r[1][k] = 0.5f * ((g0 + g2) + g1);
            r[2][k] = 0.5f * ((g0 + g2) - g1);
            r[3][k] = g2;
        }
#pragma unroll
        for (int i = 0; i < 4; ++i) {
            const float a = r[i][0], b = r[i][1], cc = r[i][2];
            U[(4 * i + 0) * plane + idx] = a;
            U[(4 * i + 1) * plane + idx] = 0.5f * ((a + cc) + b);
            U[(4 * i + 2) * plane + idx] = 0.5f * ((a + cc) - b);
            U[(4 * i + 3) * plane + idx] = cc;
        }
    }
}

template <int VEC>
struct VecT;
template <>
struct VecT<1> { typedef float type; };
template <>
struct VecT<2> { typedef float type __attribute__((ext_vector_type(2))); };
template <>
struct VecT<4> { typedef float type __attribute__((ext_vector_type(4))); };

template <int VEC>
__device__ __forceinline__ void vload(const float* p, float (&v)[VEC]) {
    if constexpr (VEC == 1) v[0] = *p;
    else {
        const typename VecT<VEC>::type t = *reinterpret_cast<const typename VecT<VEC>::type*>(p);
#pragma unroll
        for (int i = 0; i < VEC; ++i) v[i] = t[i];
    }
}
template <int VEC>
__device__ __forceinline__ void vstore(float* p, const float (&v)[VEC]) {
    if constexpr (VEC == 1) *p = v[0];
    else {
        typename VecT<VEC>::type t;
#pragma unroll
        for (int i = 0; i < VEC; ++i) t[i] = v[i];
        *reinterpret_cast<typename VecT<VEC>::type*>(p) = t;
    }
}

template <int VEC>
__global__ void __launch_bounds__(256) wino_input_kernel(const float* __restrict__ x, long long x_nstride, int pitch,
                                                         int N, int C, int H, int W, int d, int TH, int TW,
                                                         float* __restrict__ V, long long rowlen) {
    const int tpi = TH * TW;
    const long long tg = ((long long)blockIdx.x * 256 + threadIdx.x) * VEC;
    if (tg >= rowlen) return;
    const int c = blockIdx.z;
    const int n = (int)(tg / tpi), t = (int)(tg - (long long)n * tpi);
    const long long plane = (long long)C * rowlen;
    float* dst = V + (long long)c * rowlen + tg;
    float q[4][4][VEC];
    if (n >= N) {
        float z[VEC];
#pragma unroll
        for (int v = 0; v < VEC; ++v) z[v] = 0.f;
#pragma unroll
        for (int k = 0; k < 16; ++k) vstore<VEC>(dst + k * plane, z);
        return;
    }
    const int trow = t / TW, tcol = t - trow * TW;
    const int h0 = trow + d * (trow / d) - d, w0 = tcol + d * (tcol / d) - d;
    const float* src = x + (long long)n * x_nstride + (long long)c * H * pitch;
    float p[4][4][VEC];
#pragma unroll
    for (int r = 0; r < 4; ++r) {
        const int h = h0 + r * d;
        const bool hok = (unsigned)h < (unsigned)H;
#pragma unroll
        for (int s = 0; s < 4; ++s) {
            const int ww = w0 + s * d;
            if (hok && ww >= 0 && ww + VEC <= W) vload<VEC>(src + (long long)h * pitch + ww, p[r][s]);
            else {
#pragma unroll
                for (int v = 0; v < VEC; ++v)
                    p[r][s][v] = (hok && (unsigned)(ww + v) < (unsigned)W) ? src[(long long)h * pitch + ww + v] : 0.f;
            }
        }
    }
#pragma unroll
    for (int s = 0; s < 4; ++s)
#pragma unroll
        for (int v = 0; v < VEC; ++v) {
            q[0][s][v] = p[0][s][v] - p[2][s][v];
            q[1][s][v] = p[1][s][v] + p[2][s][v];
            q[2][s][v] = p[2][s][v] - p[1][s][v];
            q[3][s][v] = p[1][s][v] - p[3][s][v];
        }
#pragma unroll
    for (int r = 0; r < 4; ++r) {
        float o[4][VEC];
#pragma unroll
        for (int v = 0; v < VEC; ++v) {
            o[0][v] = q[r][0][v] - q[r][2][v];
            o[1][v] = q[r][1][v] + q[r][2][v];
            o[2][v] = q[r][2][v] - q[r][1][v];
            o[3][v] = q[r][1][v] - q[r][3][v];
        }
#pragma unroll
        for (int s = 0; s < 4; ++s) vstore<VEC>(dst + (4 * r + s) * plane, o[s]);
    }
}

template <int VEC>
__global__ void __launch_bounds__(256) wino_dy_kernel(const float* __restrict__ dy, long long dy_nstride, int pitch, int N,
                                                      int M, int H, int W, int d, int TH, int TW, float* __restrict__ Y,
                                                      long long rowlen) {
    const int tpi = TH * TW;
    const long long tg = ((long long)blockIdx.x * 256 + threadIdx.x) * VEC;
    if (tg >= rowlen) return;
    const int m = blockIdx.z;
    const int n = (int)(tg / tpi), t = (int)(tg - (long long)n * tpi);
    const long long plane = (long long)M * rowlen;
    float* dst = Y + (long long)m * rowlen + tg;
    float g[2][2][VEC];
#pragma unroll
    for (int r = 0; r < 2; ++r)
#pragma unroll
        for (int s = 0; s < 2; ++s)
#pragma unroll
            for (int v = 0; v < VEC; ++v) g[r][s][v] = 0.f;
    if (n < N) {
        const int trow = t / TW, tcol = t - trow * TW;
        const int ho = trow + d * (trow / d), wo = tcol + d * (tcol / d);
        const float* src = dy + (long long)n * dy_nstride + (long long)m * H * pitch;
#pragma unroll
        for (int r = 0; r < 2; ++r)
#pragma unroll
            for (int s = 0; s < 2; ++s) {
                const int h = ho + r * d, ww = wo + s * d;
                if (h < H && ww + VEC <= W) vload<VEC>(src + (long long)h * pitch + ww, g[r][s]);
                else {
#pragma unroll
                    for (int v = 0; v < VEC; ++v)
                        if (h < H && ww + v < W) g[r][s][v] = src[(long long)h * pitch + ww + v];
                }
            }
    }
#pragma unroll
    for (int r = 0; r < 4; ++r) {
        float o[4][VEC];
#pragma unroll
        for (int v = 0; v < VEC; ++v) {
            const float u0 = r == 0 ? g[0][0][v] : r == 1 ? g[0][0][v] + g[1][0][v] : r == 2 ? g[0][0][v] - g[1][0][v] : -g[1][0][v];
            const float u1 = r == 0 ? g[0][1][v] : r == 1 ? g[0][1][v] + g[1][1][v] : r == 2 ? g[0][1][v] - g[1][1][v] : -g[1][1][v];
            o[0][v] = u0; o[1][v] = u0 + u1; o[2][v] = u0 - u1; o[3][v] = -u1;
        }
#pragma unroll
        for (int s = 0; s < 4; ++s) vstore<VEC>(dst + (4 * r + s) * plane, o[s]);
    }
}

template <int VEC, bool STATS = false>
__global__ void __launch_bounds__(256) wino_output_kernel(const float* __restrict__ Mb, long long T, int K,
                                                          float* __restrict__ y, long long y_nstride, int H, int W,
                                                          int d, int TH, int TW, int accumulate,
                                                          float* __restrict__ stat_part,
                                                          const float* __restrict__ scale, const float* __restrict__ shift,
                                                          const float* __restrict__ residual, int relu) {
    const int tpi = TH * TW;
    const int t = (blockIdx.x * 256 + threadIdx.x) * VEC;
    if (t >= tpi) return;
    const int n = blockIdx.y, k = blockIdx.z;
    const int trow = t / TW, tcol = t - trow * TW;
    const int ho = trow + d * (trow / d), wo = tcol + d * (tcol / d);
    if (ho >= H || wo >= W) return;
    const long long plane = (long long)K * T;
    const float* src = Mb + (long long)k * T + (long long)n * tpi + t;
    float m[4][4][VEC];
#pragma unroll
    for (int r = 0; r < 4; ++r)
#pragma unroll
        for (int s = 0; s < 4; ++s) vload<VEC>(src + (4 * r + s) * plane, m[r][s]);
    float* dst = y + (long long)n * y_nstride + (long long)k * H * W;
    const float sc = scale ? scale[k] : 1.f, sf = scale ? shift[k] : 0.f;
    const float* rsd = residual ? residual + (long long)n * y_nstride + (long long)k * H * W : nullptr;
    float keep_o[2][2][VEC];
#pragma unroll
    for (int r = 0; r < 2; ++r) {
        const int h = ho + r * d;
        if (h >= H) continue;
        float u[4][VEC], o[2][VEC];
#pragma unroll
        for (int s = 0; s < 4; ++s)
#pragma unroll
            for (int v = 0; v < VEC; ++v)
                u[s][v] = r == 0 ? (m[0][s][v] + m[1][s][v]) + m[2][s][v] : (m[1][s][v] - m[2][s][v]) - m[3][s][v];
#pragma unroll
        for (int v = 0; v < VEC; ++v) {
            o[0][v] = (u[0][v] + u[1][v]) + u[2][v];
            o[1][v] = (u[1][v] - u[2][v]) - u[3][v];
            if constexpr (STATS) { keep_o[r][0][v] = o[0][v]; keep_o[r][1][v] = o[1][v]; }
        }
#pragma unroll
        for (int s = 0; s < 2; ++s) {
            const int ww = wo + s * d;
            float* e = dst + (long long)h * W + ww;
            if (scale) {
#pragma unroll
                for (int v = 0; v < VEC; ++v) {
                    float t = fmaf(o[s][v], sc, sf);
                    if (rsd && ww + v < W) t += rsd[(long long)h * W + ww + v];
                    o[s][v] = relu ? (t > 0.f ? t : 0.f) : t;
                }
            }
            if (ww + VEC <= W) {
                if (accumulate) {
                    float old[VEC];
                    vload<VEC>(e, old);
#pragma unroll
                    for (int v = 0; v < VEC; ++v) o[s][v] += old[v];
                }
                vstore<VEC>(e, o[s]);
            } else {
#pragma unroll
                for (int v = 0; v < VEC; ++v)
                    if (ww + v < W) e[v] = accumulate ? e[v] + o[s][v] : o[s][v];
            }
        }
    }
    if constexpr (STATS) {
        constexpr int G = 32 / VEC;
        float sum = 0.f;
#pragma unroll
        for (int r = 0; r < 2; ++r)
#pragma unroll
            for (int s2 = 0; s2 < 2; ++s2)
#pragma unroll
                for (int v = 0; v < VEC; ++v) sum += keep_o[r][s2][v];
#pragma unroll
        for (int off = G / 2; off > 0; off >>= 1) sum += __shfl_xor(sum, off, 64);
        const float mean = sum * (1.0f / 128.0f);
        float m2 = 0.f;
#pragma unroll
        for (int r = 0; r < 2; ++r)
#pragma unroll
            for (int s2 = 0; s2 < 2; ++s2)
#pragma unroll
                for (int v = 0; v < VEC; ++v) { const float dd = keep_o[r][s2][v] - mean; m2 += dd * dd; }
#pragma unroll
        for (int off = G / 2; off > 0; off >>= 1) m2 += __shfl_xor(m2, off, 64);
        if ((threadIdx.x & (G - 1)) == 0) {
            const long long slot = ((long long)n * tpi + t) >> 5;
            float* sp = stat_part + (slot * K + k) * 2;
            sp[0] = mean; sp[1] = m2;
        }
    }
}

__global__ void __launch_bounds__(256) wino_dw_kernel(const float* __restrict__ dU, long long mc, float* __restrict__ dw) {
    const long long i = (long long)blockIdx.x * 256 + threadIdx.x;
    if (i >= mc) return;
    float t[3][4];
#pragma unroll
    for (int s = 0; s < 4; ++s) {
        const float u0 = dU[(0 + s) * mc + i], u1 = dU[(4 + s) * mc + i], u2 = dU[(8 + s) * mc + i], u3 = dU[(12 + s) * mc + i];
        t[0][s] = u0 + 0.5f * (u1 + u2);
        t[1][s] = 0.5f * (u1 - u2);
        t[2][s] = 0.5f * (u1 + u2) + u3;
    }
    float* o = dw + i * 9;
#pragma unroll
    for (int r = 0; r < 3; ++r) {
        o[3 * r + 0] = t[r][0] + 0.5f * (t[r][1] + t[r][2]);
        o[3 * r + 1] = 0.5f * (t[r][1] - t[r][2]);
        o[3 * r + 2] = 0.5f * (t[r][1] + t[r][2]) + t[r][3];
    }
}

__global__ void __launch_bounds__(256) wino_output_kernel(const float* __restrict__ Mb, long long T, int K,
                                                          float* __restrict__ y, long long y_nstride, int H, int W,
                                                          int d, int TH, int TW, int accumulate) {
    const int tpi = TH * TW;
    const int t = blockIdx.x * 256 + threadIdx.x;
    if (t >= tpi) return;
    const int n = blockIdx.y, k = blockIdx.z;
    const int trow = t / TW, tcol = t - trow * TW;
    const int ho = trow + d * (trow / d), wo = tcol + d * (tcol / d);
    if (ho >= H || wo >= W) return;
    const long long plane = (long long)K * T;
    const float* src = Mb + (long long)k * T + (long long)n * tpi + t;
    float m[4][4];
#pragma unroll
    for (int r = 0; r < 4; ++r)
#pragma unroll
        for (int s = 0; s < 4; ++s) m[r][s] = src[(4 * r + s) * plane];
    float u[2][4];
#pragma unroll
    for (int s = 0; s < 4; ++s) {
        u[0][s] = (m[0][s] + m[1][s]) + m[2][s];
        u[1][s] = (m[1][s] - m[2][s]) - m[3][s];
    }
    float o[2][2];
#pragma unroll
    for (int r = 0; r < 2; ++r) {
        o[r][0] = (u[r][0] + u[r][1]) + u[r][2];
        o[r][1] = (u[r][1] - u[r][2]) - u[r][3];
    }
    float* dst = y + (long long)n * y_nstride + (long long)k * H * W;
#pragma unroll
    for (int r = 0; r < 2; ++r) {
        const int h = ho + r * d;
        if (h >= H) continue;
#pragma unroll
        for (int s = 0; s < 2; ++s) {
            const int ww = wo + s * d;
            if (ww >= W) continue;
            float* e = dst + (long long)h * W + ww;
            *e = accumulate ? *e + o[r][s] : o[r][s];
        }
    }
}

}

static int wino_vec(int d, int W, int pitch, const float* base, long long nstride, int TW) {
    static const int cap = [] { const char* e = getenv("DCFP_WINO_VEC"); return e ? atoi(e) : 4; }();
    for (int v = 4; v > 1; v >>= 1)
        if (v <= cap && d % v == 0 && W % v == 0 && pitch % v == 0 && nstride % v == 0 && TW % v == 0 &&
            (reinterpret_cast<uintptr_t>(base) & (4 * v - 1)) == 0)
            return v;
    return 1;
}

static WinoPlan wino_plan(const WinoProblem& q) { return wino_plan(q.N, q.H, q.W, q.d, q.M, q.Ck); }

static GemmProblem batched_gemm(const WinoPlan& pl, int M, int Ck) {
    GemmProblem g = {};
    g.T = 1; g.M = M; g.Ck = Ck; g.N = 16;
    g.Hi = g.Ho = 1; g.Wi = g.Wo = (int)pl.T16;
    g.sn = g.sd = 1; g.off0 = 0; g.offstep = 1;
    g.in_nstride = (long long)Ck * pl.T16; g.out_nstride = (long long)M * pl.T16;
    return g;
}

bool dcfp_wino_ok(const WinoProblem& q) {
    if (!dcfp_igemm2_persist()) return false;
    if (q.M < 129 || q.Ck < 128) return false;
    const WinoPlan pl = wino_plan(q);
    if (4 * pl.T > (long long)q.N * q.H * q.W * 27 / 20) return false;
    if (pl.T16 >= (1LL << 26) || 16LL * pl.T16 >= (1LL << 30)) return false;
    if ((long long)q.Ck * pl.T16 >= (1LL << 29) || (long long)q.M * pl.T16 >= (1LL << 29)) return false;
    return dcfp_igemm2_dma_shape(batched_gemm(pl, q.M, q.Ck));
}

size_t dcfp_wino_workspace_bytes(const WinoProblem& q) {
    const WinoPlan pl = wino_plan(q);
    return (size_t)(pl.u_floats + pl.v_floats + pl.m_floats) * sizeof(float);
}

double dcfp_wino_exec_fraction(const WinoProblem& q) {
    const WinoPlan pl = wino_plan(q);
    return 16.0 * (double)pl.T / (9.0 * (double)q.N * q.H * q.W);
}

long long dcfp_wino_stat_slots(const WinoProblem& q) {
    const int H = q.H, W = q.W, d = q.d;
    if (H % (2 * d) != 0 || W % (2 * d) != 0 || (W / 2) % 4 != 0) return 0;
    const long long tpi = (long long)(H / 2) * (W / 2);
    if (tpi % 32 != 0) return 0;
    return (long long)q.N * tpi / 32;
}

int dcfp_wino_run(const GemmProblem& g, const float* in, const float* w, float* out, void* workspace, size_t workspace_bytes,
                  const GemmExtras& x, hipStream_t stream) {
    const WinoProblem q = wino_problem(g);
    const int N = q.N, M = q.M, Ck = q.Ck, H = q.H, W = q.W, d = q.d, in_pitch = q.in_pitch;
    const int flip = g.offstep < 0;
    const long long in_nstride = g.in_nstride, out_nstride = g.out_nstride;
    float* const xform_out = x.xform_out;
    float* const stat_part = x.stat_part;
    const int accumulate = x.accumulate;
    const WinoPlan pl = wino_plan(q);
    if (!workspace || !dcfp_aligned16(workspace)) return DCFP_E_WORKSPACE;
    const bool three_ok = dcfp_wino_ok(q);
    const bool fused_wins = wino_fused_mode() == 2 || !three_ok || !(xform_out && Ck > 256);
    if (fused_wins && dcfp_wino_fused_ok(q) && workspace_bytes >= dcfp_wino_fused_workspace_bytes(q)) {
        if (stat_part && (!dcfp_wino_stat_slots(q) || accumulate)) return DCFP_E_UNSUPPORTED;
        return dcfp_wino_fused_run(g, in, w, out, workspace, workspace_bytes, x, stream);
    }
    if (!three_ok) return DCFP_E_UNSUPPORTED;
    if (workspace_bytes < dcfp_wino_workspace_bytes(q)) return DCFP_E_WORKSPACE;
    float* U = static_cast<float*>(workspace);
    float* V = xform_out ? xform_out : U + pl.u_floats;
    float* Mb = U + pl.u_floats + pl.v_floats;
    if (xform_out && !dcfp_aligned16(xform_out)) return DCFP_E_BADDESC;
    {
        long long b = ((long long)pl.CkP * pl.Mpad + 255) / 256;
        if (b > 4096) b = 4096;
        hipLaunchKernelGGL(wino_filter_kernel, dim3((unsigned)b), dim3(256), 0, stream, w, g.sAm, g.sAc, flip, M, Ck,
                           pl.CkP, pl.Mpad, U);
    }
    const int tpi = pl.TH * pl.TW;
    if (Ck > 65535 || M > 65535 || N > 65535) return DCFP_E_UNSUPPORTED;
    const int vec = wino_vec(d, W, in_pitch > 0 ? in_pitch : W, in, in_nstride, pl.TW);
    const unsigned gin = (unsigned)((pl.T16 / vec + 255) / 256);
#define DCFP_WINO_IN(VEC_) hipLaunchKernelGGL(wino_input_kernel<VEC_>, dim3(gin, 1, (unsigned)Ck), dim3(256), 0, stream, in, \
                                              in_nstride, in_pitch > 0 ? in_pitch : W, N, Ck, H, W, d, pl.TH, pl.TW, V, pl.T16)
    if (vec == 4) DCFP_WINO_IN(4); else if (vec == 2) DCFP_WINO_IN(2); else DCFP_WINO_IN(1);
#undef DCFP_WINO_IN
    GemmExtras gx;
    gx.wp_valid = 1;
    gx.wp_nstride = (long long)pl.CkP * pl.Mpad;
    const int rc = dcfp_igemm2_run(batched_gemm(pl, M, Ck), V, nullptr, Mb, U, (size_t)pl.u_floats * sizeof(float), gx, stream);
    if (rc) return rc;
    const int ovec = wino_vec(d, W, W, out, out_nstride, pl.TW);
    const unsigned gout = (unsigned)((tpi / ovec + 255) / 256);
#define DCFP_WINO_OUT(VEC_, ST_) hipLaunchKernelGGL((wino_output_kernel<VEC_, ST_>), dim3(gout, (unsigned)N, (unsigned)M), dim3(256), 0, \
                                               stream, Mb, pl.T16, M, out, out_nstride, H, W, d, pl.TH, pl.TW, accumulate, stat_part, x.scale, x.shift, x.residual, x.relu)
    if (stat_part) {
        if (!dcfp_wino_stat_slots(q) || accumulate) return DCFP_E_UNSUPPORTED;
        if (ovec == 4) DCFP_WINO_OUT(4, true); else if (ovec == 2) DCFP_WINO_OUT(2, true); else DCFP_WINO_OUT(1, true);
    } else if (ovec == 4) DCFP_WINO_OUT(4, false); else if (ovec == 2) DCFP_WINO_OUT(2, false); else DCFP_WINO_OUT(1, false);
#undef DCFP_WINO_OUT
    DCFP_RETURN_LAUNCH();
}


namespace {
struct WinoWgradPlan { WinoPlan pl; long long T16, v, y, du, slabs; };
WinoWgradPlan wino_wgrad_plan(int N, int H, int W, int d, int M, int C) {
    WinoWgradPlan w;
    w.pl = wino_plan(N, H, W, d, M, C);
    w.T16 = w.pl.T16;
    w.v = align64(16LL * C * w.T16);
    w.y = align64(16LL * M * w.T16);
    w.du = align64(16LL * M * C);
    w.slabs = align64((long long)(dcfp_wgrad_batched_workspace_bytes(16, M, C, w.T16, nullptr) / sizeof(float)));
    return w;
}
}

bool dcfp_wino_wgrad_ok(int N, int H, int W, int d, int M, int C) {
    if (M < 128 || C < 128) return false;
    const WinoWgradPlan w = wino_wgrad_plan(N, H, W, d, M, C);
    if (4 * w.pl.T > (long long)N * H * W * 27 / 20) return false;
    if (w.T16 >= (1LL << 30) || (long long)M * w.T16 >= (1LL << 29) || (long long)C * w.T16 >= (1LL << 29)) return false;
    return M <= 65535 && C <= 65535;
}

size_t dcfp_wino_wgrad_workspace_bytes(int N, int H, int W, int d, int M, int C) {
    const WinoWgradPlan w = wino_wgrad_plan(N, H, W, d, M, C);
    return (size_t)(w.v + w.y + w.du + w.slabs) * sizeof(float);
}

int dcfp_wino_wgrad_run(const float* dy, long long dy_nstride, int dy_pitch, const float* x, long long x_nstride,
                        int x_pitch, float* dw, int N, int M, int C, int H, int W, int d, void* workspace,
                        size_t workspace_bytes, hipStream_t stream, const float* xform_in) {
    const WinoWgradPlan w = wino_wgrad_plan(N, H, W, d, M, C);
    if (!workspace || !dcfp_aligned16(workspace) || workspace_bytes < dcfp_wino_wgrad_workspace_bytes(N, H, W, d, M, C))
        return DCFP_E_WORKSPACE;
    float* Vs = static_cast<float*>(workspace);
    const float* V = xform_in ? xform_in : Vs;
    float* Y = Vs + w.v;
    float* dU = Y + w.y;
    float* slabs = dU + w.du;
    const int xv = wino_vec(d, W, x_pitch > 0 ? x_pitch : W, x, x_nstride, w.pl.TW);
    const int yv = wino_vec(d, W, dy_pitch > 0 ? dy_pitch : W, dy, dy_nstride, w.pl.TW);
#define DCFP_WINO_IN(VEC_) hipLaunchKernelGGL(wino_input_kernel<VEC_>, dim3((unsigned)((w.T16 / VEC_ + 255) / 256), 1, (unsigned)C), \
                                              dim3(256), 0, stream, x, x_nstride, x_pitch > 0 ? x_pitch : W, N, C, H, W, d, \
                                              w.pl.TH, w.pl.TW, Vs, w.T16)
    if (xform_in) {  }
    else if (xv == 4) DCFP_WINO_IN(4); else if (xv == 2) DCFP_WINO_IN(2); else DCFP_WINO_IN(1);
#undef DCFP_WINO_IN
#define DCFP_WINO_DY(VEC_) hipLaunchKernelGGL(wino_dy_kernel<VEC_>, dim3((unsigned)((w.T16 / VEC_ + 255) / 256), 1, (unsigned)M), \
                                              dim3(256), 0, stream, dy, dy_nstride, dy_pitch > 0 ? dy_pitch : W, N, M, H, W, d, \
                                              w.pl.TH, w.pl.TW, Y, w.T16)
    if (yv == 4) DCFP_WINO_DY(4); else if (yv == 2) DCFP_WINO_DY(2); else DCFP_WINO_DY(1);
#undef DCFP_WINO_DY
    const int rc = dcfp_wgrad_batched_run(Y, V, dU, 16, M, C, w.T16, slabs, (size_t)w.slabs * sizeof(float), stream);
    if (rc) return rc;
    const long long mc = (long long)M * C;
    hipLaunchKernelGGL(wino_dw_kernel, dim3((unsigned)((mc + 255) / 256)), dim3(256), 0, stream, dU, mc, dw);
    DCFP_RETURN_LAUNCH();
}

size_t dcfp_wino_xform_bytes(const WinoProblem& q) {
    return (size_t)16 * q.Ck * wino_plan(q).T16 * sizeof(float);
}
```

### dcfp_amd/csrc/conv_winograd2.hip

```cpp
#include "wino_patch.h"
#include "conv_dispatch.h"
#include <stdlib.h>

namespace {

constexpr int FBK = 8;
constexpr int FSTAGE = 16 * FBK * 64;

struct WinoFusedParams {
    const float* in;
    const float* in_base;
    unsigned in_bytes;
    int lead;
    long long in_nstride;
    int pitch;
    const float* ug;
    float* out;
    long long out_nstride;
    float* xform_out;
    float* stat_part;
    const float* scale;
    const float* shift;
    const float* residual;
    int relu;
    int N, M, Ck, H, W, d, TH, TW;
    long long T, T16;
    int mblocks, tblocks, nk;
    int accumulate;
    int ragged_c;
    int vec_epi;
    unsigned out_bytes;
};

template <int DM, bool SIDE, bool RAGGED>
__global__ void __launch_bounds__(256, 1) wino_fused_kernel(const WinoFusedParams p) {
    constexpr int NV = PatchCfg<DM>::NV;
    extern __shared__ __attribute__((aligned(16))) float smem[];
    const int tid = threadIdx.x, lane = tid & 63, wid = tid >> 6, wm = wid >> 1, wn = wid & 1;
    const int l31 = lane & 31, lhi = lane >> 5;
    const int wid_s = __builtin_amdgcn_readfirstlane(wid);
    const int xcd = blockIdx.x & 7, jb = blockIdx.x >> 3;
    const int mb = jb % p.mblocks, tb = (jb / p.mblocks) * 8 + xcd;
    if (tb >= p.tblocks) return;
    const long long t0 = (long long)tb * 64;
    const int nk = p.nk, d = p.d, H = p.H, W = p.W, TW = p.TW, tpi = p.TH * p.TW, pitch = p.pitch;

    const unsigned lds0 = (unsigned)(size_t)(lds_ptr)smem;
    const u32x4 a_desc = make_desc(p.ug, 0x7ffffffcu);
    const unsigned lane16 = lane * 16u;

    const int ch = 2 * wid + lhi;
    const long long tp = t0 + 2 * l31;
    unsigned voff[NV];
    {
        const bool tvalid = tp < p.T;
        const long long tq = tvalid ? tp : 0;
        const int n = (int)(tq / tpi), tt = (int)(tq - (long long)n * tpi);
        const int trow = tt / TW, tcol = tt - trow * TW;
        const int h0 = trow + d * (trow / d) - d, w0 = tcol + d * (tcol / d) - d;
        const long long base = (long long)n * p.in_nstride + (long long)lhi * H * pitch + p.lead;
#pragma unroll
        for (int r = 0; r < 4; ++r) {
            const int h = h0 + r * d;
            const bool rok = tvalid && (unsigned)h < (unsigned)H;
            const long long row = base + (long long)h * pitch;
            if constexpr (DM == 1 || DM == 2) {
                voff[2 * r] = (rok && w0 < W) ? (unsigned)((row + w0) * 4) : kOob;
                voff[2 * r + 1] = (rok && w0 + 4 < W) ? (unsigned)((row + w0 + 4) * 4) : kOob;
            } else {
#pragma unroll
                for (int s = 0; s < 4; ++s) {
                    const int ww = w0 + s * d;
                    voff[4 * r + s] = (rok && (unsigned)ww < (unsigned)W) ? (unsigned)((row + ww) * 4) : kOob;
                }
            }
        }
    }
    const __amdgpu_buffer_rsrc_t in_rsrc = __builtin_amdgcn_make_buffer_rsrc(const_cast<float*>(p.in_base), 0,
                                                                             p.in_bytes, 0x00020000);
    const unsigned chan_bytes = (unsigned)(H * pitch) * 4u;
    float R[2][4][8], q[4][8];
    auto load_step = [&](int kt, auto b_) {
        constexpr int b = decltype(b_)::value;
        const unsigned soff = __builtin_amdgcn_readfirstlane((unsigned)(kt * FBK + 2 * wid_s) * chan_bytes);
        if constexpr (RAGGED) {
            unsigned vm[NV];
            const bool cok = kt * FBK + ch < p.Ck;
#pragma unroll
            for (int i = 0; i < NV; ++i) vm[i] = cok ? voff[i] : kOob;
            load_patches<DM>(in_rsrc, vm, soff, R[b]);
        } else {
            load_patches<DM>(in_rsrc, voff, soff, R[b]);
        }
    };
    auto issue_a = [&](int kt, int buf) {
        const unsigned abase = (unsigned)((kt * p.mblocks + mb) * FSTAGE) * 4u;
        static_for<0, 8>([&](auto q_) {
            constexpr int qq = decltype(q_)::value;
            const unsigned piece = (unsigned)(wid_s * 8 + qq);
            const unsigned la = __builtin_amdgcn_readfirstlane(lds0 + (unsigned)(buf * 2 * FSTAGE) * 4u + piece * 1024u);
            const unsigned a_s = __builtin_amdgcn_readfirstlane(abase + piece * 1024u);
            const unsigned av = lane16;
            const u32x4 ad = a_desc;
            asm volatile("s_mov_b32 m0, %0\n\ts_nop 0\n\tbuffer_load_dwordx4 %1, %2, %3 offen lds"
                         :: "s"(la), "v"(av), "s"(ad), "s"(a_s) : "memory", "m0");
        });
    };
    auto retire = [&]() {
        asm volatile("s_waitcnt vmcnt(0) lgkmcnt(0)" ::: "memory");
        __builtin_amdgcn_s_barrier();
    };
    auto retire_keep_loads = [&](bool stored) {
        if (SIDE && stored) {
            if constexpr (NV == 8) asm volatile("s_waitcnt vmcnt(24) lgkmcnt(0)" ::: "memory");
            else asm volatile("s_waitcnt vmcnt(32) lgkmcnt(0)" ::: "memory");
        } else {
            if constexpr (NV == 8) asm volatile("s_waitcnt vmcnt(8) lgkmcnt(0)" ::: "memory");
            else asm volatile("s_waitcnt vmcnt(16) lgkmcnt(0)" ::: "memory");
        }
        __builtin_amdgcn_s_barrier();
    };
    const long long vplane = (long long)p.Ck * p.T16;
    const unsigned vs_lane = (SIDE && tp < p.T16) ? (unsigned)(((long long)lhi * p.T16 + tp) * 4) : kOob;
    auto side_on = [&](int kt) -> bool { return SIDE && kt % p.mblocks == mb; };
    auto side_off = [&](int kt) -> unsigned {
        bool on = true;
        if constexpr (RAGGED) on = kt * FBK + ch < p.Ck;
        return on ? vs_lane : kOob;
    };
    auto side_store = [&](auto xi_, f32x2 o, int kt, unsigned vs) {
        constexpr int XI = decltype(xi_)::value;
        const __amdgpu_buffer_rsrc_t v_rsrc = __builtin_amdgcn_make_buffer_rsrc(p.xform_out + XI * vplane, 0,
                                                                                (unsigned)(vplane * 4), 0x00020000);
        const unsigned soff = __builtin_amdgcn_readfirstlane((unsigned)((long long)(kt * FBK + 2 * wid_s) * p.T16 * 4));
        __builtin_amdgcn_raw_buffer_store_b64(__builtin_bit_cast(u32x2, o), v_rsrc, vs, soff, 0);
    };
    auto produce = [&](auto xi_, int buf) -> f32x2 {
        constexpr int XI = decltype(xi_)::value;
        const f32x2 o = col_transform<DM, XI>(q);
        float* bs = smem + buf * 2 * FSTAGE + FSTAGE + (XI * FBK + ch) * 64 + 2 * l31;
        *reinterpret_cast<f32x2*>(bs) = o;
        return o;
    };

    f32x16 acc[16];
#pragma unroll
    for (int i = 0; i < 16; ++i)
#pragma unroll
        for (int r = 0; r < 16; ++r) acc[i][r] = 0.f;

    load_step(0, std::integral_constant<int, 0>{});
    row_transform<DM>(R[0], q);
    __builtin_amdgcn_sched_barrier(0);
    issue_a(0, 0);
    {
        const unsigned vs = side_off(0);
        const bool st = side_on(0);
        static_for<0, 16>([&](auto xi_) {
            const f32x2 o = produce(xi_, 0);
            if constexpr (SIDE) {
                if (st) side_store(xi_, o, 0, vs);
            }
        });
    }
    load_step(1, std::integral_constant<int, 1>{});
    __builtin_amdgcn_sched_barrier(0);
    load_step(nk > 2 ? 2 : 1, std::integral_constant<int, 0>{});
    retire();

    const int a_lane = wm * 256 + lane * 4;
    const int b_lane = lhi * 64 + wn * 32 + l31;
    f32x4 af[2] = {{0.f, 0.f, 0.f, 0.f}, {0.f, 0.f, 0.f, 0.f}};
    float bf[2][4] = {{0.f, 0.f, 0.f, 0.f}, {0.f, 0.f, 0.f, 0.f}};
    auto step = [&](auto prod_, auto par_, int kt) {
        constexpr bool PROD = decltype(prod_)::value;
        constexpr int cur = decltype(par_)::value, rb = cur ^ 1;
        unsigned vs = kOob;
        bool st = false;
        if constexpr (PROD) { vs = side_off(kt + 1); st = side_on(kt + 1); }
        const float* As = smem + cur * 2 * FSTAGE + a_lane;
        const float* Bs = smem + cur * 2 * FSTAGE + FSTAGE + b_lane;
        const int ktl = kt + 3 < nk ? kt + 3 : nk - 1;
        const unsigned l_soff = __builtin_amdgcn_readfirstlane((unsigned)(ktl * FBK + 2 * wid_s) * chan_bytes);
        unsigned vm[NV];
        if constexpr (PROD) {
#pragma unroll
            for (int i = 0; i < NV; ++i) vm[i] = voff[i];
            if constexpr (RAGGED) {
                const bool cok = ktl * FBK + ch < p.Ck;
#pragma unroll
                for (int i = 0; i < NV; ++i) vm[i] = cok ? voff[i] : kOob;
            }
        }
        const unsigned abase = (unsigned)(((kt + 1) * p.mblocks + mb) * FSTAGE) * 4u;
        f32x2 okeep[8];
        static_for<0, 16>([&](auto g_) {
            constexpr int g = decltype(g_)::value;
            constexpr int fb = g & 1, pg = (g + 15) & 15;
            af[fb] = *reinterpret_cast<const f32x4*>(As + g * 512);
#pragma unroll
            for (int kk = 0; kk < 4; ++kk) bf[fb][kk] = Bs[(g * FBK + 2 * kk) * 64];
            f32x2 o = {0.f, 0.f};
            if constexpr (PROD) {
                if constexpr (g < 4) {
                    row_transform_one<DM, g>(R[rb], q);
#pragma unroll
                    for (int c = 0; c < PatchCfg<DM>::NCOL; ++c) asm volatile("" : "+v"(q[g][c]));
                }
                o = col_transform<DM, g>(q);
                asm volatile("" : "+v"(o));
                if constexpr (g < 8) {
                    const unsigned piece = (unsigned)(wid_s * 8 + g);
                    const unsigned la = __builtin_amdgcn_readfirstlane(lds0 + (unsigned)((cur ^ 1) * 2 * FSTAGE) * 4u + piece * 1024u);
                    const unsigned a_s = __builtin_amdgcn_readfirstlane(abase + piece * 1024u);
                    const unsigned av = lane16;
                    const u32x4 ad = a_desc;
                    asm volatile("s_mov_b32 m0, %0\n\ts_nop 0\n\tbuffer_load_dwordx4 %1, %2, %3 offen lds"
                                 :: "s"(la), "v"(av), "s"(ad), "s"(a_s) : "memory", "m0");
                }
            }
            __builtin_amdgcn_sched_barrier(0);
            acc[pg] = __builtin_amdgcn_mfma_f32_32x32x2f32(af[fb ^ 1][0], bf[fb ^ 1][0], acc[pg], 0, 0, 0);
            acc[pg] = __builtin_amdgcn_mfma_f32_32x32x2f32(af[fb ^ 1][1], bf[fb ^ 1][1], acc[pg], 0, 0, 0);
            __builtin_amdgcn_sched_barrier(0);
            if constexpr (PROD) {
                float* bs = smem + (cur ^ 1) * 2 * FSTAGE + FSTAGE + (g * FBK + ch) * 64 + 2 * l31;
                *reinterpret_cast<f32x2*>(bs) = o;
                if constexpr (SIDE) {
                    if constexpr (g < 8) okeep[g] = o;
                    else if (st) {
                        side_store(std::integral_constant<int, g - 8>{}, okeep[g - 8], kt + 1, vs);
                        side_store(g_, o, kt + 1, vs);
                    }
                }
            }
            __builtin_amdgcn_sched_barrier(0);
            acc[pg] = __builtin_amdgcn_mfma_f32_32x32x2f32(af[fb ^ 1][2], bf[fb ^ 1][2], acc[pg], 0, 0, 0);
            __builtin_amdgcn_sched_barrier(0);
            if constexpr (PROD && g >= 8) {
                constexpr int per = NV / 8;
                static_for<0, per>([&](auto j_) { load_one<DM, (g - 8) * per + decltype(j_)::value>(in_rsrc, vm, l_soff, R[rb]); });
            }
            acc[pg] = __builtin_amdgcn_mfma_f32_32x32x2f32(af[fb ^ 1][3], bf[fb ^ 1][3], acc[pg], 0, 0, 0);
            __builtin_amdgcn_sched_barrier(0);
        });
    };

    constexpr std::integral_constant<int, 0> even{};
    constexpr std::integral_constant<int, 1> odd{};
    int kt = 0;
    for (; kt + 3 < nk; kt += 2) {
        step(std::true_type{}, even, kt);
        retire_keep_loads(side_on(kt + 1));
        step(std::true_type{}, odd, kt + 1);
        retire_keep_loads(side_on(kt + 2));
    }
    step(std::true_type{}, even, nk - 2);
    retire();
    step(std::false_type{}, odd, nk - 1);
#pragma unroll
    for (int kk = 0; kk < 4; ++kk)
        acc[15] = __builtin_amdgcn_mfma_f32_32x32x2f32(af[1][kk], bf[1][kk], acc[15], 0, 0, 0);

    const long long te = t0 + wn * 32 + l31;
    const bool tv = te < p.T;
    const long long tq = tv ? te : 0;
    const int n = (int)(tq / tpi), tt = (int)(tq - (long long)n * tpi);
    const int trow = tt / TW, tcol = tt - trow * TW;
    const int ho = trow + d * (trow / d), wo = tcol + d * (tcol / d);
    const bool okr0 = tv && ho < H, okr1 = tv && ho + d < H;
    const bool okc0 = wo < W, okc1 = wo + d < W;
    const long long HW = (long long)H * W;
    const int m_lane = mb * 64 + wm * 32 + 4 * lhi;
    const int acc_out = p.accumulate;
    float* const sp0 = p.stat_part;
    const long long slot = (long long)tb * 2 + wn;
    auto out_transform = [&](int r, float (&o)[2][2]) {
        float u[2][4];
#pragma unroll
        for (int s = 0; s < 4; ++s) {
            u[0][s] = (acc[0 + s][r] + acc[4 + s][r]) + acc[8 + s][r];
            u[1][s] = (acc[4 + s][r] - acc[8 + s][r]) - acc[12 + s][r];
        }
#pragma unroll
        for (int rr = 0; rr < 2; ++rr) {
            o[rr][0] = (u[rr][0] + u[rr][1]) + u[rr][2];
            o[rr][1] = (u[rr][1] - u[rr][2]) - u[rr][3];
        }
    };
    auto red32 = [&](float v) -> float {
        auto dpp = [](float x, auto ctrl_) {
            constexpr int ctrl = decltype(ctrl_)::value;
            return __builtin_bit_cast(float, __builtin_amdgcn_update_dpp(0, __builtin_bit_cast(int, x), ctrl, 0xF, 0xF, true));
        };
        v += dpp(v, std::integral_constant<int, 0xB1>{});
        v += dpp(v, std::integral_constant<int, 0x4E>{});
        v += dpp(v, std::integral_constant<int, 0x141>{});
        v += dpp(v, std::integral_constant<int, 0x140>{});
        v += __builtin_bit_cast(float, __builtin_amdgcn_update_dpp(0, __builtin_bit_cast(int, v), 0x142, 0xA, 0xF, false));
        const float lo = __builtin_bit_cast(float, __builtin_amdgcn_readlane(__builtin_bit_cast(int, v), 31));
        const float hi = __builtin_bit_cast(float, __builtin_amdgcn_readlane(__builtin_bit_cast(int, v), 63));
        return lhi ? hi : lo;
    };
    auto stats = [&](int m, const float (&o)[2][2]) {
        const float sum = red32((o[0][0] + o[0][1]) + (o[1][0] + o[1][1]));
        const float mean = sum * (1.0f / 128.0f);
        const float d0 = o[0][0] - mean, d1 = o[0][1] - mean, d2 = o[1][0] - mean, d3 = o[1][1] - mean;
        const float m2 = red32((d0 * d0 + d1 * d1) + (d2 * d2 + d3 * d3));
        if (l31 == 0 && m < p.M && t0 + wn * 32 < p.T) {
            float* sp = sp0 + (slot * p.M + m) * 2;
            sp[0] = mean; sp[1] = m2;
        }
    };
    if (p.vec_epi) {
        auto xor1 = [](float v) { return __builtin_bit_cast(float, __builtin_amdgcn_mov_dpp(__builtin_bit_cast(int, v), 0xB1, 0xF, 0xF, true)); };
        auto xor2 = [](float v) { return __builtin_bit_cast(float, __builtin_amdgcn_mov_dpp(__builtin_bit_cast(int, v), 0x4E, 0xF, 0xF, true)); };
        const bool odd = l31 & 1, hi2 = l31 & 2;
        int row, col;
        bool ok;
        if constexpr (DM == 4) {
            const int i = l31 & 3;
            row = ho + (i >> 1) * d;
            col = wo - i + (i & 1) * d;
            ok = tv && row < H && col < W;
        } else if constexpr (DM == 2) {
            row = ho + (odd ? d : 0);
            col = wo - (odd ? 1 : 0);
            ok = tv && row < H && col < W;
        } else {
            row = ho + (odd ? 1 : 0);
            col = wo - (odd ? 2 : 0);
            ok = tv && row < H && col < W;
        }
        const unsigned evoff = ok ? (unsigned)(((long long)n * p.out_nstride + (long long)m_lane * HW + (long long)row * W + col) * 4) : kOob;
        const __amdgpu_buffer_rsrc_t o_rsrc = __builtin_amdgcn_make_buffer_rsrc(p.out, 0, p.out_bytes, 0x00020000);
        const unsigned HW4 = (unsigned)HW * 4u;
        static_for<0, 16>([&](auto r_) {
            constexpr int r = decltype(r_)::value;
            constexpr int mr = (r & 3) + 8 * (r >> 2);
            float o[2][2];
            out_transform(r, o);
            if (sp0) stats(m_lane + mr, o);
            f32x4 v;
            if constexpr (DM == 4) {
                const float x0 = odd ? o[0][0] : o[0][1], x1 = odd ? o[1][0] : o[1][1];
                const float y0 = xor1(x0), y1 = xor1(x1);
                const float b0 = odd ? y0 : o[0][0], b1 = odd ? o[0][1] : y0, b2 = odd ? y1 : o[1][0], b3 = odd ? o[1][1] : y1;
                const float z0 = hi2 ? b0 : b2, z1 = hi2 ? b1 : b3;
                const float w0 = xor2(z0), w1 = xor2(z1);
                v[0] = hi2 ? w0 : b0; v[1] = hi2 ? w1 : b1; v[2] = hi2 ? b2 : w0; v[3] = hi2 ? b3 : w1;
            } else {
                const float s0 = odd ? o[0][0] : o[1][0], s1 = odd ? o[0][1] : o[1][1];
                const float r0 = xor1(s0), r1 = xor1(s1);
                if constexpr (DM == 2) {
                    v[0] = odd ? r0 : o[0][0]; v[1] = odd ? o[1][0] : r0; v[2] = odd ? r1 : o[0][1]; v[3] = odd ? o[1][1] : r1;
                } else {
                    v[0] = odd ? r0 : o[0][0]; v[1] = odd ? r1 : o[0][1]; v[2] = odd ? o[1][0] : r0; v[3] = odd ? o[1][1] : r1;
                }
            }
            const unsigned vo = (m_lane + mr < p.M) ? evoff : kOob;
            const unsigned so = __builtin_amdgcn_readfirstlane((unsigned)mr * HW4);
            if (p.scale) {
                const int mm = m_lane + mr < p.M ? m_lane + mr : p.M - 1;
                const float sc = p.scale[mm], sf = p.shift[mm];
#pragma unroll
                for (int e = 0; e < 4; ++e) v[e] = fmaf(v[e], sc, sf);
                if (p.residual) {
                    const __amdgpu_buffer_rsrc_t r_rsrc = __builtin_amdgcn_make_buffer_rsrc(const_cast<float*>(p.residual), 0,
                                                                                            p.out_bytes, 0x00020000);
                    v += __builtin_bit_cast(f32x4, __builtin_amdgcn_raw_buffer_load_b128(r_rsrc, vo, so, 0));
                }
                if (p.relu) {
#pragma unroll
                    for (int e = 0; e < 4; ++e) v[e] = v[e] > 0.f ? v[e] : 0.f;
                }
            }
            if (acc_out) v += __builtin_bit_cast(f32x4, __builtin_amdgcn_raw_buffer_load_b128(o_rsrc, vo, so, 0));
            __builtin_amdgcn_raw_buffer_store_b128(__builtin_bit_cast(u32x4, v), o_rsrc, vo, so, 0);
        });
        return;
    }
    float* obase = p.out + (long long)n * p.out_nstride + (long long)ho * W + wo;
    const long long dW = (long long)d * W;
#pragma unroll
    for (int r = 0; r < 16; ++r) {
        const int m = m_lane + (r & 3) + 8 * (r >> 2);
        float o[2][2];
        out_transform(r, o);
        if (m < p.M && p.scale) {
            const float sc = p.scale[m], sf = p.shift[m];
            const float* rs = p.residual ? p.residual + (obase - p.out) + (long long)m * HW : nullptr;
            const long long offs[2][2] = {{0, d}, {dW, dW + d}};
            const bool oks[2][2] = {{okr0 && okc0, okr0 && okc1}, {okr1 && okc0, okr1 && okc1}};
#pragma unroll
            for (int rr = 0; rr < 2; ++rr)
#pragma unroll
                for (int cc = 0; cc < 2; ++cc) {
                    float t = fmaf(o[rr][cc], sc, sf);
                    if (rs && oks[rr][cc]) t += rs[offs[rr][cc]];
                    o[rr][cc] = p.relu ? (t > 0.f ? t : 0.f) : t;
                }
        }
        if (m < p.M) {
            float* e = obase + (long long)m * HW;
            if (acc_out) {
                if (okr0 && okc0) e[0] += o[0][0];
                if (okr0 && okc1) e[d] += o[0][1];
                if (okr1 && okc0) e[dW] += o[1][0];
                if (okr1 && okc1) e[dW + d] += o[1][1];
            } else {
                if (okr0 && okc0) e[0] = o[0][0];
                if (okr0 && okc1) e[d] = o[0][1];
                if (okr1 && okc0) e[dW] = o[1][0];
                if (okr1 && okc1) e[dW + d] = o[1][1];
            }
        }
        if (sp0) stats(m, o);
    }
}

__global__ void __launch_bounds__(256) wino_filter2_kernel(const float* __restrict__ w, int sAm, int sAc, int flip, int M,
                                                           int Ck, int CkP, int Mpad, float* __restrict__ Ug) {
    const long long total = (long long)CkP * Mpad;
    for (long long idx = (long long)blockIdx.x * 256 + threadIdx.x; idx < total; idx += (long long)gridDim.x * 256)
        wino_filter2_pair(w, sAm, sAc, flip, M, Ck, Mpad, idx, Ug);
}

struct FusedPlan {
    int TH, TW, mblocks, tblocks, nk, CkP, Mpad;
    long long T, T16, ug_floats;
};
FusedPlan fused_plan(int N, int H, int W, int d, int M, int Ck) {
    FusedPlan pl;
    pl.TH = d * ((H + 2 * d - 1) / (2 * d));
    pl.TW = d * ((W + 2 * d - 1) / (2 * d));
    pl.TW = (pl.TW + 3) / 4 * 4;
    pl.T = (long long)N * pl.TH * pl.TW;
    pl.T16 = (pl.T + 15) / 16 * 16;
    pl.CkP = (Ck + 15) / 16 * 16;
    pl.Mpad = (M + 63) / 64 * 64;
    pl.mblocks = pl.Mpad / 64;
    pl.tblocks = (int)((pl.T + 63) / 64);
    pl.nk = pl.CkP / 8;
    pl.ug_floats = ((long long)16 * pl.CkP * pl.Mpad + 63) / 64 * 64;
    return pl;
}

}

static int fused_mode(const WinoProblem& q) {
    const int pitch = q.in_pitch > 0 ? q.in_pitch : q.W, d = q.d, W = q.W;
    const long long span = (long long)(q.N - 1) * q.in_nstride + (long long)((q.Ck + 15) / 16 * 16) * q.H * pitch + 64;
    if (span * 4 >= 0x7fffff00LL) return -1;
    if (d == 1 && pitch >= W + 4) return 1;
    if (d == 2 && pitch >= W + 4) return 2;
    if (d >= 4 && d % 2 == 0 && W % 2 == 0) return 4;
    return -1;
}

bool dcfp_wino_fused_ok(const WinoProblem& q) {
    if (wino_fused_mode() == 0) return false;
    if (q.M < 48 || q.Ck < 48) return false;
    const FusedPlan pl = fused_plan(q.N, q.H, q.W, q.d, q.M, q.Ck);
    if (pl.T16 >= (1LL << 30) || (long long)pl.tblocks * pl.mblocks + 8 * pl.mblocks >= (1LL << 31)) return false;
    if ((long long)pl.CkP * pl.Mpad * 16 * 4 >= 0x7fffff00LL) return false;
    return fused_mode(q) >= 0;
}

void dcfp_wino_fused_pads(const WinoProblem& q, int* CkP, int* Mpad) {
    const FusedPlan pl = fused_plan(q.N, q.H, q.W, q.d, q.M, q.Ck);
    *CkP = pl.CkP; *Mpad = pl.Mpad;
}

size_t dcfp_wino_fused_workspace_bytes(const WinoProblem& q) {
    return (size_t)fused_plan(q.N, q.H, q.W, q.d, q.M, q.Ck).ug_floats * sizeof(float);
}

int dcfp_wino_fused_run(const GemmProblem& g, const float* in, const float* w, float* out, void* workspace,
                        size_t workspace_bytes, const GemmExtras& x, hipStream_t stream) {
    const WinoProblem q = wino_problem(g);
    const int N = q.N, M = q.M, Ck = q.Ck, H = q.H, W = q.W, d = q.d;
    const int flip = g.offstep < 0;
    const long long in_nstride = g.in_nstride, out_nstride = g.out_nstride;
    float* const xform_out = x.xform_out;
    const FusedPlan pl = fused_plan(N, H, W, d, M, Ck);
    if (!workspace || !dcfp_aligned16(workspace) || workspace_bytes < (size_t)pl.ug_floats * sizeof(float))
        return DCFP_E_WORKSPACE;
    const int pitch = q.in_pitch > 0 ? q.in_pitch : W;
    const int mode = fused_mode(q);
    if (mode < 0) return DCFP_E_UNSUPPORTED;
    float* Ug = static_cast<float*>(workspace);
    if (!x.wp_valid) {
        long long b = ((long long)pl.CkP * pl.Mpad + 255) / 256;
        if (b > 4096) b = 4096;
        hipLaunchKernelGGL(wino_filter2_kernel, dim3((unsigned)b), dim3(256), 0, stream, w, g.sAm, g.sAc, flip, M, Ck, pl.CkP,
                           pl.Mpad, Ug);
    }
    WinoFusedParams p;
    p.in = in;
    p.lead = (mode == 1 || mode == 2) ? 4 : 0;
    p.in_base = in - p.lead;
    p.in_bytes = (unsigned)(((long long)(N - 1) * in_nstride + (long long)Ck * H * pitch + p.lead) * 4);
    p.in_nstride = in_nstride;
    p.pitch = pitch;
    p.ug = Ug;
    p.out = out;
    p.out_nstride = out_nstride;
    p.xform_out = xform_out;
    p.stat_part = x.stat_part;
    p.scale = x.scale; p.shift = x.shift; p.residual = x.residual; p.relu = x.relu;
    p.N = N; p.M = M; p.Ck = Ck; p.H = H; p.W = W; p.d = d; p.TH = pl.TH; p.TW = pl.TW;
    p.T = pl.T; p.T16 = pl.T16;
    p.mblocks = pl.mblocks; p.tblocks = pl.tblocks; p.nk = pl.nk;
    p.accumulate = x.accumulate;
    p.ragged_c = (Ck % 16) != 0;
    {
        const long long ospan = ((long long)(N - 1) * out_nstride + (long long)M * H * W) * 4;
        p.vec_epi = W % 4 == 0 && out_nstride % 4 == 0 && dcfp_aligned16(out) && ospan < 0x7fffff00LL &&
                    (mode != 4 || d % 4 == 0);
        p.out_bytes = p.vec_epi ? (unsigned)ospan : 0u;
        static const int no_vec = [] { const char* e = getenv("DCFP_WF_SCALAR_EPI"); return e ? atoi(e) : 0; }();
        if (no_vec) p.vec_epi = 0;
    }
    const long long grid = (long long)((pl.tblocks + 7) / 8) * 8 * pl.mblocks;
    const size_t lds = (size_t)4 * FSTAGE * sizeof(float);
    auto launch = [&](auto kern) -> int {
        hipError_t e = hipFuncSetAttribute(reinterpret_cast<const void*>(kern), hipFuncAttributeMaxDynamicSharedMemorySize,
                                           (int)lds);
        if (e != hipSuccess) return (int)e;
        hipLaunchKernelGGL(kern, dim3((unsigned)grid), dim3(256), lds, stream, p);
        DCFP_RETURN_LAUNCH();
    };
    if (xform_out && (long long)Ck * pl.T16 * 4 >= 0x7fffff00LL) return DCFP_E_UNSUPPORTED;
    const bool ragged = (Ck % 16) != 0;
#define DCFP_WF(DM_) (xform_out ? (ragged ? launch(wino_fused_kernel<DM_, true, true>) : launch(wino_fused_kernel<DM_, true, false>)) \
                                : (ragged ? launch(wino_fused_kernel<DM_, false, true>) : launch(wino_fused_kernel<DM_, false, false>)))
    switch (mode) {
        case 1: return DCFP_WF(1);
        case 2: return DCFP_WF(2);
        case 4: return DCFP_WF(4);
        default: return DCFP_E_UNSUPPORTED;
    }
#undef DCFP_WF
}
```

### dcfp_amd/csrc/conv_winograd3.hip

```cpp
#include "wino_patch.h"
#include "conv_dispatch.h"
#include <stdlib.h>

namespace {

constexpr int GBK = 8;
constexpr int GKH = 144;
constexpr int GHALF = 2 * GKH;
constexpr int GCOMP = 2 * GHALF;
constexpr int GSTAGE = 16 * GCOMP;
constexpr unsigned kSat = 0xffffffffu;

struct WinoWgParams {
    const float* x_base;
    unsigned x_bytes;
    const float* dy_base;
    unsigned dy_bytes;
    const unsigned* table;
    unsigned table_bytes;
    float* out;
    int M, C, mblocks, cblocks, nblk;
    unsigned x_chan_bytes, dy_chan_bytes;
    int kchunk;
    long long T16;
    int d;
};

__global__ void __launch_bounds__(256) wino_wg_table_kernel(unsigned* __restrict__ table, long long npairs, long long T, int N,
                                                            int H, int W, int d, int TH, int TW, long long x_nstride,
                                                            int x_pitch, int lead, long long dy_nstride, int dy_pitch, int dm) {
    const long long pi = (long long)blockIdx.x * 256 + threadIdx.x;
    if (pi >= npairs) return;
    unsigned e[8] = {kOob, kOob, kOob, kOob, kOob, kOob, 0u, 0u};
    const long long t = 2 * pi;
    if (t < T) {
        const int tpi = TH * TW;
        const int n = (int)(t / tpi), tt = (int)(t - (long long)n * tpi);
        const int trow = tt / TW, tcol = tt - trow * TW;
        const int ho = trow + d * (trow / d), wo = tcol + d * (tcol / d);
        if (ho < H && wo < W) {
            const int h0 = ho - d, w0 = wo - d;
            for (int r = 0; r < 4; ++r) {
                const int h = h0 + r * d;
                if (h >= 0 && h < H)
                    e[r] = dm == 4 ? (unsigned)(((long long)n * x_nstride + (long long)h * x_pitch) * 4)
                                   : (unsigned)(((long long)n * x_nstride + (long long)h * x_pitch + w0 + lead) * 4);
            }
            for (int r = 0; r < 2; ++r) {
                const int h = ho + r * d;
                if (h < H)
                    e[4 + r] = dm == 4 ? (unsigned)(((long long)n * dy_nstride + (long long)h * dy_pitch) * 4)
                                       : (unsigned)(((long long)n * dy_nstride + (long long)h * dy_pitch + wo) * 4);
            }
            if (dm == 4) {
                unsigned m = 0;
                for (int s = 0; s < 4; ++s)
                    if (w0 + s * d >= 0 && w0 + s * d < W) m |= 1u << s;
                for (int s = 0; s < 2; ++s)
                    if (wo + s * d < W) m |= 16u << s;
                e[6] = m;
                e[7] = (unsigned)(w0 * 4);
            }
        }
    }
    u32x4* dst = reinterpret_cast<u32x4*>(table + pi * 8);
    dst[0] = u32x4{e[0], e[1], e[2], e[3]};
    dst[1] = u32x4{e[4], e[5], e[6], e[7]};
}

__global__ void __launch_bounds__(256) wino_dw_reduce_kernel(const float* __restrict__ slabs, int splits, long long mc,
                                                             float* __restrict__ dw) {
    const long long i = (long long)blockIdx.x * 256 + threadIdx.x;
    if (i >= mc) return;
    float u[16];
#pragma unroll
    for (int k = 0; k < 16; ++k) u[k] = slabs[k * mc + i];
    int s = 1;
    for (; s + 4 <= splits; s += 4) {
        float v[4][16];
#pragma unroll
        for (int q = 0; q < 4; ++q) {
            const float* sl = slabs + (long long)(s + q) * 16 * mc + i;
#pragma unroll
            for (int k = 0; k < 16; ++k) v[q][k] = sl[k * mc];
        }
#pragma unroll
        for (int q = 0; q < 4; ++q)
#pragma unroll
            for (int k = 0; k < 16; ++k) u[k] += v[q][k];
    }
    for (; s < splits; ++s) {
        const float* sl = slabs + (long long)s * 16 * mc + i;
#pragma unroll
        for (int k = 0; k < 16; ++k) u[k] += sl[k * mc];
    }
    float t[3][4];
#pragma unroll
    for (int s = 0; s < 4; ++s) {
        const float u0 = u[0 + s], u1 = u[4 + s], u2 = u[8 + s], u3 = u[12 + s];
        t[0][s] = u0 + 0.5f * (u1 + u2);
        t[1][s] = 0.5f * (u1 - u2);
        t[2][s] = 0.5f * (u1 + u2) + u3;
    }
    float* o = dw + i * 9;
#pragma unroll
    for (int r = 0; r < 3; ++r) {
        o[3 * r + 0] = t[r][0] + 0.5f * (t[r][1] + t[r][2]);
        o[3 * r + 1] = 0.5f * (t[r][1] - t[r][2]);
        o[3 * r + 2] = 0.5f * (t[r][1] + t[r][2]) + t[r][3];
    }
}

__device__ __forceinline__ unsigned sat_add(unsigned a, unsigned b) {
    unsigned r;
    asm("v_add_u32_e64 %0, %1, %2 clamp" : "=v"(r) : "v"(a), "v"(b));
    return r;
}

template <int DM> __device__ __forceinline__ constexpr int dcolA(int s) { return DM == 1 ? s : 2 * s; }
template <int DM> __device__ __forceinline__ constexpr int dcolB(int s) { return DM == 1 ? 2 + s : 2 * s + 1; }
template <int DM> struct DyCfg { static constexpr int NY = DM == 4 ? 4 : 2; };

template <int DM, int I>
__device__ __forceinline__ void load_dy_one(const __amdgpu_buffer_rsrc_t rsrc, const unsigned (&voff)[DyCfg<DM>::NY],
                                            float (&D)[2][4]) {
    if constexpr (DM == 4) {
        constexpr int r = I >> 1, s = I & 1;
        const f32x2 a = __builtin_bit_cast(f32x2, __builtin_amdgcn_raw_buffer_load_b64(rsrc, voff[I], 0, 0));
        D[r][2 * s] = a[0]; D[r][2 * s + 1] = a[1];
    } else {
        const f32x4 a = __builtin_bit_cast(f32x4, __builtin_amdgcn_raw_buffer_load_b128(rsrc, voff[I], 0, 0));
        D[I][0] = a[0]; D[I][1] = a[1]; D[I][2] = a[2]; D[I][3] = a[3];
    }
}

template <int DM, int XI>
__device__ __forceinline__ f32x2 dy_component(const float (&U)[4][4]) {
    constexpr int i = XI >> 2, j = XI & 3;
    const float a0 = U[i][dcolA<DM>(0)], a1 = U[i][dcolA<DM>(1)], b0 = U[i][dcolB<DM>(0)], b1 = U[i][dcolB<DM>(1)];
    f32x2 o;
    if constexpr (j == 0) { o[0] = a0; o[1] = b0; }
    if constexpr (j == 1) { o[0] = a0 + a1; o[1] = b0 + b1; }
    if constexpr (j == 2) { o[0] = a0 - a1; o[1] = b0 - b1; }
    if constexpr (j == 3) { o[0] = a1; o[1] = b1; }
    return o;
}

template <int DM, bool RAGGED>
__global__ void __launch_bounds__(256, 1) wino_wgrad_fused_kernel(const WinoWgParams p) {
    constexpr int NX = PatchCfg<DM>::NV, NY = DyCfg<DM>::NY, NT = 2 + NX + NY;
    extern __shared__ __attribute__((aligned(16))) float smem[];
    const int tid = threadIdx.x, lane = tid & 63, wid = tid >> 6, wm = wid >> 1, wn = wid & 1;
    const int l31 = lane & 31, lhi = lane >> 5;
    const int per = (p.nblk + 7) >> 3;
    const int xcd = blockIdx.x & 7, jb = blockIdx.x >> 3;
    const int L = xcd * per + jb;
    if (L >= p.nblk) return;
    const int mb = L % p.mblocks, cb = (L / p.mblocks) % p.cblocks, split = L / (p.mblocks * p.cblocks);
    const long long tile0 = (long long)split * p.kchunk;
    const long long left = p.T16 - tile0;
    const int nk = (int)((left < p.kchunk ? left : (long long)p.kchunk) / GBK);

    const int j = tid & 3, cl = tid >> 2;
    const int cg = cb * 64 + cl, mg = mb * 64 + cl;
    const bool c_ok = !RAGGED || cg < p.C, m_ok = !RAGGED || mg < p.M;
    const unsigned xc = (unsigned)cg * p.x_chan_bytes, dyc = (unsigned)mg * p.dy_chan_bytes;
    const __amdgpu_buffer_rsrc_t x_rsrc = __builtin_amdgcn_make_buffer_rsrc(const_cast<float*>(p.x_base), 0, p.x_bytes, 0x00020000);
    const __amdgpu_buffer_rsrc_t y_rsrc = __builtin_amdgcn_make_buffer_rsrc(const_cast<float*>(p.dy_base), 0, p.dy_bytes, 0x00020000);
    const __amdgpu_buffer_rsrc_t t_rsrc = __builtin_amdgcn_make_buffer_rsrc(const_cast<unsigned*>(p.table), 0, p.table_bytes, 0x00020000);
    const unsigned ev = (unsigned)j * 32u;
    const unsigned e_s0 = (unsigned)(tile0 >> 1) * 32u;
    const unsigned d4 = (unsigned)p.d * 4u;

    unsigned E[8];
    auto load_entry = [&](int k) {
        const unsigned soff = __builtin_amdgcn_readfirstlane(e_s0 + (unsigned)k * 128u);
        const u32x4 a = __builtin_amdgcn_raw_buffer_load_b128(t_rsrc, ev, soff, 0);
        E[0] = a[0]; E[1] = a[1]; E[2] = a[2]; E[3] = a[3];
        if constexpr (DM == 4) {
            const u32x4 b = __builtin_amdgcn_raw_buffer_load_b128(t_rsrc, ev + 16u, soff, 0);
            E[4] = b[0]; E[5] = b[1]; E[6] = b[2]; E[7] = b[3];
        } else {
            const u32x2 b = __builtin_amdgcn_raw_buffer_load_b64(t_rsrc, ev + 16u, soff, 0);
            E[4] = b[0]; E[5] = b[1];
        }
    };
    unsigned vx[NX], vy[NY];
    auto make_offsets = [&]() {
        if constexpr (DM == 4) {
            const unsigned w0b = E[7];
            unsigned colk[4], dcol[2];
#pragma unroll
            for (int s = 0; s < 4; ++s) colk[s] = ((E[6] >> s) & 1u) && c_ok ? xc + w0b + (unsigned)s * d4 : kSat;
#pragma unroll
            for (int s = 0; s < 2; ++s) dcol[s] = ((E[6] >> (4 + s)) & 1u) && m_ok ? dyc + w0b + (unsigned)(1 + s) * d4 : kSat;
#pragma unroll
            for (int r = 0; r < 4; ++r)
#pragma unroll
                for (int s = 0; s < 4; ++s) vx[4 * r + s] = sat_add(E[r], colk[s]);
#pragma unroll
            for (int r = 0; r < 2; ++r)
#pragma unroll
                for (int s = 0; s < 2; ++s) vy[2 * r + s] = sat_add(E[4 + r], dcol[s]);
        } else {
#pragma unroll
            for (int r = 0; r < 4; ++r) {
                const unsigned a = c_ok ? E[r] + xc : kOob;
                vx[2 * r] = a; vx[2 * r + 1] = a + 16u;
            }
#pragma unroll
            for (int r = 0; r < 2; ++r) vy[r] = m_ok ? E[4 + r] + dyc : kOob;
        }
    };
    float R[2][4][8], D[2][2][4], q[4][8], U[4][4];
    auto load_all = [&](auto b_) {
        constexpr int b = decltype(b_)::value;
        static_for<0, NX>([&](auto i_) { load_one<DM, decltype(i_)::value>(x_rsrc, vx, 0u, R[b]); });
        static_for<0, NY>([&](auto i_) { load_dy_one<DM, decltype(i_)::value>(y_rsrc, vy, D[b]); });
    };
    auto vmem_op = [&](auto i_, auto b_, int k_entry) {
        constexpr int I = decltype(i_)::value, b = decltype(b_)::value;
        if constexpr (I == 0) load_entry(k_entry);
        else if constexpr (I == 1) {  }
        else if constexpr (I < 2 + NX) load_one<DM, I - 2>(x_rsrc, vx, 0u, R[b]);
        else load_dy_one<DM, I - 2 - NX>(y_rsrc, vy, D[b]);
    };
    const int pw = (cl >> 5) * GHALF + (j >> 1) * GKH + (cl & 31) * 4 + 2 * (j & 1);
    auto produce_x = [&](auto xi_, int buf) {
        constexpr int XI = decltype(xi_)::value;
        const f32x2 o = col_transform<DM, XI>(q);
        *reinterpret_cast<f32x2*>(smem + buf * 2 * GSTAGE + GSTAGE + XI * GCOMP + pw) = o;
    };
    auto produce_y = [&](auto xi_, int buf) {
        constexpr int XI = decltype(xi_)::value;
        const f32x2 o = dy_component<DM, XI>(U);
        *reinterpret_cast<f32x2*>(smem + buf * 2 * GSTAGE + XI * GCOMP + pw) = o;
    };
    auto dy_rows = [&](auto g_, const float (&Dd)[2][4]) {
        constexpr int g = decltype(g_)::value;
#pragma unroll
        for (int c = 0; c < 4; ++c) {
            if constexpr (g == 0) { U[0][c] = Dd[0][c]; U[3][c] = Dd[1][c]; }
            if constexpr (g == 1) { U[1][c] = Dd[0][c] + Dd[1][c]; asm volatile("" : "+v"(U[1][c])); }
            if constexpr (g == 2) { U[2][c] = Dd[0][c] - Dd[1][c]; asm volatile("" : "+v"(U[2][c])); }
        }
    };
    auto retire = [&]() {
        __builtin_amdgcn_s_waitcnt(0xC07F);
        __builtin_amdgcn_s_barrier();
    };

    f32x16 acc[16];
#pragma unroll
    for (int i = 0; i < 16; ++i)
#pragma unroll
        for (int r = 0; r < 16; ++r) acc[i][r] = 0.f;

    constexpr std::integral_constant<int, 0> even{};
    constexpr std::integral_constant<int, 1> odd{};
    load_entry(0); make_offsets(); load_all(even);
    load_entry(1); make_offsets(); load_all(odd);
    row_transform<DM>(R[0], q);
    static_for<0, 4>([&](auto g_) { dy_rows(g_, D[0]); });
    __builtin_amdgcn_sched_barrier(0);
    static_for<0, 16>([&](auto xi_) { produce_y(xi_, 0); produce_x(xi_, 0); });
    load_entry(nk > 2 ? 2 : 1); make_offsets(); load_all(even);
    load_entry(nk > 3 ? 3 : nk - 1);
    asm volatile("s_waitcnt vmcnt(0) lgkmcnt(0)" ::: "memory");
    __builtin_amdgcn_s_barrier();

    const int a_lane = wm * GHALF + lhi * GKH + l31 * 4;
    const int b_lane = wn * GHALF + lhi * GKH + l31 * 4;
    f32x4 af[2] = {{0.f, 0.f, 0.f, 0.f}, {0.f, 0.f, 0.f, 0.f}};
    f32x4 bf[2] = {{0.f, 0.f, 0.f, 0.f}, {0.f, 0.f, 0.f, 0.f}};
    auto step = [&](auto prod_, auto par_, int kt) {
        constexpr bool PROD = decltype(prod_)::value;
        constexpr int cur = decltype(par_)::value, rb = cur ^ 1;
        const float* As = smem + cur * 2 * GSTAGE + a_lane;
        const float* Bs = smem + cur * 2 * GSTAGE + GSTAGE + b_lane;
        const int k_entry = kt + 4 < nk ? kt + 4 : nk - 1;
        static_for<0, 16>([&](auto g_) {
            constexpr int g = decltype(g_)::value;
            constexpr int fb = g & 1, pg = (g + 15) & 15;
            af[fb] = *reinterpret_cast<const f32x4*>(As + g * GCOMP);
            bf[fb] = *reinterpret_cast<const f32x4*>(Bs + g * GCOMP);
            f32x2 ox = {0.f, 0.f}, oy = {0.f, 0.f};
            if constexpr (PROD) {
                if constexpr (g < 4) {
                    row_transform_one<DM, g>(R[rb], q);
#pragma unroll
                    for (int c = 0; c < PatchCfg<DM>::NCOL; ++c) asm volatile("" : "+v"(q[g][c]));
                    dy_rows(g_, D[rb]);
                }
                oy = dy_component<DM, g>(U);
                ox = col_transform<DM, g>(q);
                asm volatile("" : "+v"(ox), "+v"(oy));
                if constexpr (g == 7) make_offsets();
            }
            __builtin_amdgcn_sched_barrier(0);
            acc[pg] = __builtin_amdgcn_mfma_f32_32x32x2f32(af[fb ^ 1][0], bf[fb ^ 1][0], acc[pg], 0, 0, 0);
            acc[pg] = __builtin_amdgcn_mfma_f32_32x32x2f32(af[fb ^ 1][1], bf[fb ^ 1][1], acc[pg], 0, 0, 0);
            __builtin_amdgcn_sched_barrier(0);
            if constexpr (PROD) {
                *reinterpret_cast<f32x2*>(smem + rb * 2 * GSTAGE + g * GCOMP + pw) = oy;
                *reinterpret_cast<f32x2*>(smem + rb * 2 * GSTAGE + GSTAGE + g * GCOMP + pw) = ox;
            }
            __builtin_amdgcn_sched_barrier(0);
            acc[pg] = __builtin_amdgcn_mfma_f32_32x32x2f32(af[fb ^ 1][2], bf[fb ^ 1][2], acc[pg], 0, 0, 0);
            __builtin_amdgcn_sched_barrier(0);
            if constexpr (PROD && g >= 8) {
                constexpr int lo = (g - 8) * NT / 8, hi = (g - 7) * NT / 8;
                static_for<lo, hi>([&](auto i_) { vmem_op(i_, std::integral_constant<int, rb>{}, k_entry); });
            }
            acc[pg] = __builtin_amdgcn_mfma_f32_32x32x2f32(af[fb ^ 1][3], bf[fb ^ 1][3], acc[pg], 0, 0, 0);
            __builtin_amdgcn_sched_barrier(0);
        });
    };

    int kt = 0;
    for (; kt + 3 < nk; kt += 2) {
        step(std::true_type{}, even, kt);
        retire();
        step(std::true_type{}, odd, kt + 1);
        retire();
    }
    step(std::true_type{}, even, nk - 2);
    retire();
    step(std::false_type{}, odd, nk - 1);
#pragma unroll
    for (int kk = 0; kk < 4; ++kk)
        acc[15] = __builtin_amdgcn_mfma_f32_32x32x2f32(af[1][kk], bf[1][kk], acc[15], 0, 0, 0);

    const long long mc = (long long)p.M * p.C;
    const __amdgpu_buffer_rsrc_t o_rsrc = __builtin_amdgcn_make_buffer_rsrc(p.out + (long long)split * 16 * mc, 0,
                                                                            (unsigned)(16 * mc * 4), 0x00020000);
    const int m0 = mb * 64 + wm * 32 + 4 * lhi, c0 = cb * 64 + wn * 32 + l31;
    const unsigned ov = (!RAGGED || c0 < p.C) ? (unsigned)(((long long)m0 * p.C + c0) * 4) : kOob;
    const unsigned C4 = (unsigned)p.C * 4u, mc4 = (unsigned)(mc * 4);
    static_for<0, 16>([&](auto xi_) {
        constexpr int XI = decltype(xi_)::value;
        constexpr bool neg = ((XI >> 2) == 3) != ((XI & 3) == 3);
        static_for<0, 16>([&](auto r_) {
            constexpr int r = decltype(r_)::value, mr = (r & 3) + 8 * (r >> 2);
            const unsigned so = __builtin_amdgcn_readfirstlane((unsigned)XI * mc4 + (unsigned)mr * C4);
            const unsigned vo = (!RAGGED || m0 + mr < p.M) ? ov : kOob;
            const float v = neg ? -acc[XI][r] : acc[XI][r];
            __builtin_amdgcn_raw_buffer_store_b32(__builtin_bit_cast(unsigned, v), o_rsrc, vo, so, 0);
        });
    });
}

struct WgPlan {
    int TH, TW, mblocks, cblocks, splits, kchunk, mode, lead;
    long long T, T16, table_floats, slab_floats;
};

int wg_mode(int N, int H, int W, int d, int M, int C, long long x_nstride, int x_pitch, long long dy_nstride, int dy_pitch) {
    const long long xspan = ((long long)(N - 1) * x_nstride + (long long)((C + 63) / 64 * 64) * H * x_pitch + 64) * 4;
    const long long yspan = ((long long)(N - 1) * dy_nstride + (long long)((M + 63) / 64 * 64) * H * dy_pitch + 64) * 4;
    if (xspan >= 0x7fffff00LL || yspan >= 0x7fffff00LL) return -1;
    if ((d == 1 || d == 2) && x_pitch >= W + 4 && W % 4 == 0) return d;
    if (d >= 4 && d % 2 == 0 && W % 2 == 0) return 4;
    return -1;
}

WgPlan wg_plan(int N, int H, int W, int d, int M, int C) {
    WgPlan pl;
    pl.TH = d * ((H + 2 * d - 1) / (2 * d));
    pl.TW = d * ((W + 2 * d - 1) / (2 * d));
    pl.TW = (pl.TW + 3) / 4 * 4;
    pl.T = (long long)N * pl.TH * pl.TW;
    pl.T16 = (pl.T + 15) / 16 * 16;
    pl.mblocks = (M + 63) / 64;
    pl.cblocks = (C + 63) / 64;
    const long long tiles = (long long)pl.mblocks * pl.cblocks, slots = dcfp_num_cus();
    long long max_splits = pl.T16 / (32 * GBK);
    if (max_splits < 1) max_splits = 1;
    long long splits = 1;
    double best = -1.0;
    for (long long sp = 1; sp <= max_splits && tiles * sp <= 2 * slots; ++sp) {
        const long long blocks = tiles * sp, rounds = (blocks + slots - 1) / slots;
        const double eff = (double)blocks / (double)(rounds * slots);
        if (eff > best + 0.02) { best = eff; splits = sp; }
    }
    long long kchunk = (pl.T16 + splits - 1) / splits;
    kchunk = (kchunk + 15) / 16 * 16;
    splits = (pl.T16 + kchunk - 1) / kchunk;
    pl.splits = (int)splits;
    pl.kchunk = (int)kchunk;
    pl.table_floats = (pl.T16 / 2 * 8 + 63) / 64 * 64;
    pl.slab_floats = (long long)pl.splits * 16 * M * C;
    return pl;
}

}

bool dcfp_wino_wgrad_fused_ok(int N, int H, int W, int d, int M, int C, long long x_nstride, int x_pitch,
                              long long dy_nstride, int dy_pitch) {
    if (wino_wgrad_fused_mode() == 0) return false;
    if (M < 48 || C < 48) return false;
    if (x_pitch <= 0) x_pitch = W;
    if (dy_pitch <= 0) dy_pitch = W;
    if (wg_mode(N, H, W, d, M, C, x_nstride, x_pitch, dy_nstride, dy_pitch) < 0) return false;
    const WgPlan pl = wg_plan(N, H, W, d, M, C);
    if (pl.T16 >= (1LL << 30) || pl.T16 / 2 * 32 >= 0x7fffff00LL) return false;
    if (16LL * M * C * 4 >= 0x7fffff00LL) return false;
    return (long long)pl.mblocks * pl.cblocks * pl.splits < (1LL << 28);
}

size_t dcfp_wino_wgrad_fused_workspace_bytes(int N, int H, int W, int d, int M, int C) {
    const WgPlan pl = wg_plan(N, H, W, d, M, C);
    return (size_t)(pl.table_floats + pl.slab_floats) * sizeof(float);
}

int dcfp_wino_wgrad_fused_run(const float* dy, long long dy_nstride, int dy_pitch, const float* x, long long x_nstride,
                              int x_pitch, float* dw, int N, int M, int C, int H, int W, int d, void* workspace,
                              size_t workspace_bytes, hipStream_t stream) {
    if (x_pitch <= 0) x_pitch = W;
    if (dy_pitch <= 0) dy_pitch = W;
    const int mode = wg_mode(N, H, W, d, M, C, x_nstride, x_pitch, dy_nstride, dy_pitch);
    if (mode < 0) return DCFP_E_UNSUPPORTED;
    const WgPlan pl = wg_plan(N, H, W, d, M, C);
    if (!workspace || !dcfp_aligned16(workspace) || workspace_bytes < dcfp_wino_wgrad_fused_workspace_bytes(N, H, W, d, M, C))
        return DCFP_E_WORKSPACE;
    unsigned* table = static_cast<unsigned*>(workspace);
    float* slabs = static_cast<float*>(workspace) + pl.table_floats;
    const int lead = mode == 4 ? 0 : 4;
    const long long npairs = pl.T16 / 2;
    hipLaunchKernelGGL(wino_wg_table_kernel, dim3((unsigned)((npairs + 255) / 256)), dim3(256), 0, stream, table, npairs, pl.T,
                       N, H, W, d, pl.TH, pl.TW, x_nstride, x_pitch, lead, dy_nstride, dy_pitch, mode);
    WinoWgParams p;
    p.x_base = x - lead;
    p.x_bytes = (unsigned)(((long long)(N - 1) * x_nstride + (long long)C * H * x_pitch + lead) * 4);
    p.dy_base = dy;
    p.dy_bytes = (unsigned)(((long long)(N - 1) * dy_nstride + (long long)M * H * dy_pitch) * 4);
    p.table = table;
    p.table_bytes = (unsigned)(npairs * 32);
    p.out = slabs;
    p.M = M; p.C = C; p.mblocks = pl.mblocks; p.cblocks = pl.cblocks;
    p.nblk = pl.mblocks * pl.cblocks * pl.splits;
    p.x_chan_bytes = (unsigned)((long long)H * x_pitch * 4);
    p.dy_chan_bytes = (unsigned)((long long)H * dy_pitch * 4);
    p.kchunk = pl.kchunk;
    p.T16 = pl.T16;
    p.d = d;
    const unsigned grid = (unsigned)(((p.nblk + 7) / 8) * 8);
    const size_t lds = (size_t)4 * GSTAGE * sizeof(float);
    auto launch = [&](auto kern) -> int {
        hipError_t e = hipFuncSetAttribute(reinterpret_cast<const void*>(kern), hipFuncAttributeMaxDynamicSharedMemorySize,
                                           (int)lds);
        if (e != hipSuccess) return (int)e;
        hipLaunchKernelGGL(kern, dim3(grid), dim3(256), lds, stream, p);
        hipError_t e2 = hipGetLastError();
        return e2 == hipSuccess ? DCFP_OK : (int)e2;
    };
    const bool ragged = (M % 64) != 0 || (C % 64) != 0;
    int rc;
#define DCFP_WG(DM_) (ragged ? launch(wino_wgrad_fused_kernel<DM_, true>) : launch(wino_wgrad_fused_kernel<DM_, false>))
    switch (mode) {
        case 1: rc = DCFP_WG(1); break;
        case 2: rc = DCFP_WG(2); break;
        default: rc = DCFP_WG(4); break;
    }
#undef DCFP_WG
    if (rc) return rc;
    const long long mc = (long long)M * C;
    hipLaunchKernelGGL(wino_dw_reduce_kernel, dim3((unsigned)((mc + 255) / 256)), dim3(256), 0, stream, slabs, pl.splits, mc, dw);
    DCFP_RETURN_LAUNCH();
}
```

### include/dcfp_hip.h

```cpp
#ifndef DCFP_HIP_H
#define DCFP_HIP_H

#include <stddef.h>
#include <stdint.h>

#ifdef __cplusplus
extern "C" {
#endif

#define DCFP_OK 0
#define DCFP_E_BADDESC (-1)
#define DCFP_E_UNSUPPORTED (-2)
#define DCFP_E_WORKSPACE (-3)

typedef void* dcfp_stream_t;

int dcfp_abi_version(void);

typedef struct DcfpConvDesc {
    int32_t N, Cin, H, W;
    int32_t Cout, KH, KW;
    int32_t stride, pad, dil;
    int32_t Hout, Wout;
    int32_t x_pitch, dy_pitch;
} DcfpConvDesc;

enum { DCFP_CONV_FWD = 0, DCFP_CONV_DGRAD = 1, DCFP_CONV_WGRAD = 2 };

size_t dcfp_conv2d_workspace_bytes(const DcfpConvDesc* d, int pass);

#define DCFP_WP_BLOCK_ELEMS 2048
typedef struct DcfpWpEntry {
    const float* w;
    float* wp;
    int64_t first_block;
    int64_t n_blocks;
    int32_t T, Ck, CkP, M, Mpad, sAm, sAc;
    int32_t perm8;
} DcfpWpEntry;
int dcfp_conv2d_wp_layout(const DcfpConvDesc* d, int pass, DcfpWpEntry* entry);
int dcfp_conv2d_permute_weights_multi_f32(const DcfpWpEntry* table, int n_entries, int64_t total_blocks,
                                          dcfp_stream_t stream);

int dcfp_conv2d_pitch_supported(const DcfpConvDesc* d);

int dcfp_conv2d_workspace_is_scratch(const DcfpConvDesc* d, int pass);

size_t dcfp_conv2d_xform_bytes(const DcfpConvDesc* d);
int dcfp_conv2d_fwd_keep_f32_nchw(const DcfpConvDesc* d, const float* x, const float* w, float* y, int64_t y_nstride,
                                  float* xform_out, size_t xform_bytes,
                                  float* stat_partials ,
                                  void* workspace, size_t workspace_bytes, dcfp_stream_t stream);
int dcfp_conv2d_wgrad_kept_f32_nchw(const DcfpConvDesc* d, const float* dy, int64_t dy_nstride, const float* xform,
                                    size_t xform_bytes, float* dw, void* workspace, size_t workspace_bytes,
                                    dcfp_stream_t stream);

int dcfp_conv2d_dgrad_fanin_supported(const DcfpConvDesc* d);
int dcfp_conv2d_dgrad_fanin_f32_nchw(const DcfpConvDesc* d, const float* dy, int64_t dy_nstride, const float* w, float* dx,
                                     const float* fan_src, const void* fan_mask, void* workspace, size_t workspace_bytes,
                                     int wp_valid, dcfp_stream_t stream);
int64_t dcfp_conv2d_dgrad_fanin_red_slots(const DcfpConvDesc* d);
int dcfp_conv2d_dgrad_fanin_red_f32_nchw(const DcfpConvDesc* d, const float* dy, int64_t dy_nstride, const float* w,
                                         float* dx, const float* fan_src, const void* fan_mask, const float* red_x,
                                         const void* red_mask, const float* red_mean, float* red_part, void* workspace,
                                         size_t workspace_bytes, int wp_valid, dcfp_stream_t stream);
int dcfp_bn_bwd_sums_from_partials_f32(const float* partials, int64_t slots, int C, const float* var, float eps,
                                       float* sum_dy, float* sum_dy_xmu, float* dgamma ,
                                       float* dbeta , dcfp_stream_t stream);

int dcfp_conv2d_kernel_name(const DcfpConvDesc* d, int pass, char* buf, int buf_len);

double dcfp_conv2d_executed_fraction(const DcfpConvDesc* d, int pass);

int dcfp_conv2d_fwd_f32_nchw(const DcfpConvDesc* d, const float* x, const float* w,
                             const float* bias, float* y, int64_t y_nstride,
                             void* workspace, size_t workspace_bytes, int wp_valid,
                             dcfp_stream_t stream);
int dcfp_conv2d_fwd_fused_f32_nchw(const DcfpConvDesc* d, const float* x, const float* w,
                                   const float* scale, const float* shift, const float* residual,
                                   int relu, float* y, void* workspace, size_t workspace_bytes,
                                   int wp_valid, dcfp_stream_t stream);
int dcfp_conv2d_dgrad_f32_nchw(const DcfpConvDesc* d, const float* dy, int64_t dy_nstride,
                               const float* w, float* dx, int accumulate,
                               void* workspace, size_t workspace_bytes, int wp_valid,
                               dcfp_stream_t stream);
int dcfp_conv2d_wgrad_f32_nchw(const DcfpConvDesc* d, const float* dy, int64_t dy_nstride,
                               const float* x, float* dw, float* db,
                               void* workspace, size_t workspace_bytes,
                               dcfp_stream_t stream);

typedef struct DcfpBnRunning {
    float* running_mean;
    float* running_var;
    int64_t* num_batches_tracked;
    float momentum;
    int32_t pad_;
} DcfpBnRunning;
size_t dcfp_bn_workspace_bytes(int N, int C, int HW);
int dcfp_bn_stats_f32(const float* x, int64_t x_nstride, int N, int C, int HW,
                      float* mean, float* var, const DcfpBnRunning* run,
                      void* workspace, size_t workspace_bytes, dcfp_stream_t stream);
int dcfp_bn_apply_f32(const float* x, const float* mean, const float* var,
                      const float* gamma, const float* beta, float eps,
                      const float* residual, int relu, float* y, int64_t y_nstride,
                      int N, int C, int HW, int W, int y_pitch, dcfp_stream_t stream);
int dcfp_bn_bwd_reduce_f32(const float* dy, int64_t dy_nstride, const float* x,
                           const float* y, int64_t y_nstride, const float* mean,
                           const float* var, const float* gamma, const float* beta, float eps,
                           int relu, int N, int C, int HW,
                           float* sum_dy, float* sum_dy_xmu, float* dgamma ,
                           float* dbeta ,
                           void* workspace, size_t workspace_bytes, dcfp_stream_t stream);
int64_t dcfp_conv2d_fwd_stat_slots(const DcfpConvDesc* d, const float* y, int64_t y_nstride);
int dcfp_conv2d_fwd_stats_f32_nchw(const DcfpConvDesc* d, const float* x, const float* w, float* y,
                                   int64_t y_nstride, float* stat_partials, void* workspace,
                                   size_t workspace_bytes, int wp_valid, dcfp_stream_t stream);
int dcfp_bn_stats_from_partials_f32(const float* partials, int64_t slots, int slot_count, int C,
                                    float* mean, float* var, const DcfpBnRunning* run , dcfp_stream_t stream);
int dcfp_syncbn_combine_f32(const float* gathered, int world, int C, float* mean, float* var,
                            float* total_count, const DcfpBnRunning* run , dcfp_stream_t stream);
#define DCFP_P2P_HANDLE_BYTES 64
size_t dcfp_syncbn_p2p_mailbox_bytes(int world, int cap_floats);
int dcfp_p2p_alloc(size_t bytes, int kind, void** ptr);
int dcfp_p2p_free(void* ptr);
int dcfp_p2p_export(void* ptr, void* handle64);
int dcfp_p2p_import(const void* handle64, void** ptr);
int dcfp_p2p_unmap(void* ptr);
int dcfp_syncbn_p2p_exchange_f32(void* const* mailboxes, int world, int rank, uint32_t seq, int cap_floats,
                                 const float* local, int n, int mode, float* out, const DcfpBnRunning* run,
                                 uint32_t spin_limit, int32_t* status, dcfp_stream_t stream);
int dcfp_bn_update_running_f32(const float* mean, const float* var, int C, float momentum,
                               float count, const float* count_dev, float* running_mean,
                               float* running_var, dcfp_stream_t stream);
int dcfp_bn_apply_relu_mask_f32(const float* x, const float* mean, const float* var,
                                const float* gamma, const float* beta, float eps,
                                const float* residual, float* y, void* relu_mask,
                                int N, int C, int HW, dcfp_stream_t stream);
int dcfp_bn_bwd_apply_f32(const float* dy, int64_t dy_nstride, const float* x,
                          const float* y, int64_t y_nstride, const float* mean,
                          const float* var, const float* gamma, const float* beta, float eps,
                          const float* sum_dy, const float* sum_dy_xmu, float count,
                          const float* count_dev,
                          int relu, float* dx, float* d_residual,
                          int N, int C, int HW, int W, int dx_pitch ,
                          dcfp_stream_t stream);

size_t dcfp_bn_bwd_fused_sync_bytes(int N, int C, int HW);
int dcfp_bn_bwd_fused_f32(const float* dy, int64_t dy_nstride, const float* x, const float* y,
                          int64_t y_nstride, const float* mean, const float* var, const float* gamma,
                          const float* beta, float eps, float count, int relu, float* dx, float* d_residual,
                          int N, int C, int HW, int W, int dx_pitch, float* sum_dy, float* sum_dy_xmu,
                          float* dgamma, float* dbeta, void* sync, size_t sync_bytes, uint32_t epoch,
                          uint32_t spin_limit, int32_t* status, dcfp_stream_t stream);

int dcfp_maxpool3x3s2_fwd_f32(const float* x, float* y, int32_t* argmax,
                              int N, int C, int H, int W, int Hout, int Wout,
                              dcfp_stream_t stream);
int dcfp_maxpool3x3s2_bwd_f32(const float* dy, const int32_t* argmax, float* dx,
                              int N, int C, int H, int W, int Hout, int Wout,
                              dcfp_stream_t stream);
int dcfp_rowsum_f32(const float* x, int64_t x_nstride, float* y, float scale,
                    int N, int C, int HW, dcfp_stream_t stream);
int dcfp_broadcast_hw_f32(const float* v, float scale, float* y, int64_t y_nstride,
                          int accumulate, int N, int C, int HW, dcfp_stream_t stream);
int dcfp_add_f32(const float* a, const float* b, float* out, int64_t n,
                 dcfp_stream_t stream);
int dcfp_channel_scale_f32(const float* x, const float* mask, float* y,
                           int N, int C, int HW, dcfp_stream_t stream);

int dcfp_upsample_bilinear_fwd_f32(const float* x, float* y, int N, int C,
                                   int h, int w, int H, int W, int align_corners,
                                   dcfp_stream_t stream);
int dcfp_upsample_bilinear_bwd_f32(const float* dy, float* dx, int N, int C,
                                   int h, int w, int H, int W, int align_corners,
                                   dcfp_stream_t stream);
int dcfp_resize_bilinear_into_f32(const float* x, int64_t x_nstride, int N, int C, int h, int w,
                                  float* y, int64_t y_nstride, int y_pitch, int H, int W,
                                  int align_corners, dcfp_stream_t stream);
int dcfp_resize_bilinear_adjoint_f32(const float* dy, int64_t dy_nstride, int dy_pitch, int N, int C, int H, int W,
                                     float* dx, int64_t dx_nstride, int h, int w, int align_corners,
                                     int accumulate, dcfp_stream_t stream);
int dcfp_ppm_pool_f32(const float* x, int N, int C, int H, int W, int nlev, const int* level_hw,
                      float* out, int mean, float* dst, int64_t dst_nstride, int dst_pitch,
                      dcfp_stream_t stream);
int dcfp_ppm_pool_adjoint_f32(const float* dp, int N, int C, int H, int W, int nlev, const int* level_hw,
                              const float* g, int64_t g_nstride, int g_pitch, float* dx, dcfp_stream_t stream);
int dcfp_ppm_resize_adjoint_f32(const float* g, int64_t g_nstride, int g_pitch, int N, int H, int W,
                                int nlev, const int* level_chw, float* dp, int align_corners,
                                dcfp_stream_t stream);
size_t dcfp_upsample_ce_workspace_bytes(int N, int H, int W);
int dcfp_upsample_ce_fwd_f32(const float* logits, const int64_t* labels,
                             const uint8_t* pixel_keep, int ignore_index,
                             int N, int C, int h, int w, int H, int W, int align_corners,
                             float* lse, float* gt_prob, float* out2,
                             void* workspace, size_t workspace_bytes,
                             dcfp_stream_t stream);
int dcfp_upsample_ce_bwd_f32(const float* logits, const int64_t* labels,
                             const uint8_t* pixel_keep, int ignore_index,
                             int N, int C, int h, int w, int H, int W, int align_corners,
                             const float* lse, const float* grad_scale ,
                             float* dlogits, dcfp_stream_t stream);
int dcfp_upsample_ce_bwd_plan(int N, int C, int h, int w, int H, int W, int* variant, int* chunk_width, int* chunks);

int dcfp_ohem_zoom_gt_prob_f32(const float* logits, const int64_t* labels, const float* lse,
                               int N, int C, int h, int w, int H, int W, int align_corners,
                               int H8, int W8, float* pred8, int32_t* lab8,
                               dcfp_stream_t stream);

int dcfp_ohem_threshold_f32(const float* pred8, const int32_t* lab8, int64_t n, int ignore_label,
                            float thresh, int64_t min_kept, float* threshold ,
                            dcfp_stream_t stream);
int dcfp_ohem_keep_mask_u8(const float* gt_prob, const float* threshold , int64_t n,
                           uint8_t* keep, dcfp_stream_t stream);

int dcfp_upsample_margin_f32(const float* logits, int N, int C, int h, int w, int H, int W,
                             int align_corners, float* margin, dcfp_stream_t stream);
int dcfp_maxfilter2d_s1_f32(const float* x, float* y, int planes, int H, int W, int k,
                            dcfp_stream_t stream);
size_t dcfp_upsample_wce_workspace_bytes(int N, int H, int W);
int dcfp_upsample_wce_fwd_f32(const float* logits, const int64_t* labels, const float* pix_weight,
                              int ignore_index, int N, int C, int h, int w, int H, int W,
                              int align_corners, float* lse, float* out_per_image,
                              void* workspace, size_t workspace_bytes, dcfp_stream_t stream);
int dcfp_upsample_wce_bwd_f32(const float* logits, const int64_t* labels, const float* pix_weight,
                              int ignore_index, int N, int C, int h, int w, int H, int W,
                              int align_corners, const float* lse,
                              const float* grad_scale_per_image, float* dlogits,
                              dcfp_stream_t stream);

int dcfp_upsample_argmax_f32(const float* logits, int N, int C, int h, int w, int H, int W,
                             int align_corners, int32_t* pred, dcfp_stream_t stream);
int dcfp_confusion_matrix_i64(const int32_t* pred, const int64_t* gt, int ignore_index,
                              int64_t n_pixels, int C, int64_t* conf ,
                              dcfp_stream_t stream);

typedef struct DcfpVoteMap {
    const float* logits;
    int h, w;
    int hs, ws;
    int flip;
    float weight;
} DcfpVoteMap;
int dcfp_vote_multiscale_f32(const DcfpVoteMap* maps, int n_maps, int N, int C,
                             int H, int W,
                             int out_h, int out_w,
                             int align_corners,
                             float* scores,
                             int32_t* pred,
                             const int64_t* gt, int ignore_index,
                             int64_t* conf,
                             dcfp_stream_t stream);

#define DCFP_SLIDE_MAX_PASSES 16
#define DCFP_SLIDE_MAX_TILES_PER_AXIS 32
int dcfp_gather_tiles_f32(const float* image, int N, int channels, int h, int w,
                          const int32_t* ys, int rows, const int32_t* xs, int cols,
                          int th, int tw, int flip, float* tiles, dcfp_stream_t stream);

typedef struct DcfpSlidePass {
    const float* logits;
    int lh, lw;
    int hs, ws;
    int th, tw;
    int rows, cols;
    int flip;
    float weight;
} DcfpSlidePass;
int dcfp_vote_sliding_f32(const DcfpSlidePass* passes, int n_passes,
                          const int32_t* origins_host, const int32_t* origins_dev,
                          int N, int C,
                          int H, int W,
                          int out_h, int out_w,
                          int align_corners,
                          float* scores,
                          int32_t* pred,
                          const int64_t* gt, int ignore_index,
                          int64_t* conf,
                          dcfp_stream_t stream);

size_t dcfp_label_boundary_workspace_bytes(int N, int H, int W);
int dcfp_label_boundary_i32(const int32_t* labels, int32_t* out, int N, int H, int W, int num_classes, int d,
                            int background, void* workspace, size_t workspace_bytes, dcfp_stream_t stream);
int dcfp_label_boundary_i64(const int64_t* labels, int64_t* out, int N, int H, int W, int num_classes, int d,
                            int background, void* workspace, size_t workspace_bytes, dcfp_stream_t stream);

#define DCFP_AUG_SATURATION 1
#define DCFP_AUG_HUE 2
typedef struct DcfpAugTap {
    int32_t src, c0, c1, lsrc;
} DcfpAugTap;
typedef struct DcfpAugSample {
    const uint8_t* image;
    const uint8_t* label;
    int32_t src_h, src_w;
    int32_t col_off, row_off;
    int32_t lut_a_off;
    int32_t lut_b_off;
    int32_t hsv_flags;
    int32_t hue_delta;
    float sat_alpha;
    int32_t pad_;
} DcfpAugSample;
int dcfp_augment_u8_to_f32_nchw(const DcfpAugSample* samples, int N, int crop_h, int crop_w, const DcfpAugTap* taps,
                                int64_t n_taps, const uint8_t* lut_a, int64_t lut_a_bytes, const float* lut_b,
                                int64_t lut_b_floats, const uint8_t* id_table, int ignore_label, float* images,
                                int64_t* labels, int32_t* hist, dcfp_stream_t stream);
int dcfp_balance_weight_f32(const int64_t* labels, const int32_t* hist, const int32_t* target_class, int N,
                            int64_t pixels, int num_classes, int ignore_label, int balance, double beta, float* weight,
                            dcfp_stream_t stream);

typedef struct DcfpCcSample {
    const uint8_t* label;
    int32_t src_h, src_w;
    int32_t dst_h, dst_w;
    int32_t Hp, Wp;
    int32_t row_off, col_off;
    int32_t cls;
    int32_t pad_;
    int64_t work_off;
} DcfpCcSample;
size_t dcfp_components_workspace_bytes(int Hp, int Wp);
int dcfp_label_components_u8(const DcfpCcSample* samples, int N, const int32_t* maps, int64_t n_maps,
                             const uint8_t* id_table, void* work, size_t work_bytes, int32_t* counts,
                             dcfp_stream_t stream);
int dcfp_component_pixel_i32(const DcfpCcSample* samples, int N, void* work, size_t work_bytes, const int32_t* counts,
                             const int32_t* n, const int32_t* k, int32_t* yx, dcfp_stream_t stream);

typedef struct DcfpEicEntry {
    const float* gamma;
    const float* grad;
    float* eic;
    int32_t n;
    int32_t pad_;
} DcfpEicEntry;
int dcfp_eic_update_f32(const DcfpEicEntry* table, int n_layers, float r,
                        float one_minus_r ,
                        dcfp_stream_t stream);

typedef struct DcfpSgdEntry {
    float* param;
    const float* grad;
    float* momentum_buf;
    int64_t n;
    int64_t first_chunk;
    float weight_decay;
    int32_t pad_;
} DcfpSgdEntry;
#define DCFP_SGD_CHUNK 16384
int dcfp_sgd_momentum_f32(const DcfpSgdEntry* table, int n_tensors, int64_t total_chunks,
                          float lr, float momentum, int first_step, dcfp_stream_t stream);

typedef struct DcfpAdamEntry {
    float* param;
    const float* grad;
    float* exp_avg;
    float* exp_avg_sq;
    int64_t n;
    int64_t first_chunk;
} DcfpAdamEntry;
int dcfp_adamw_f32(const DcfpAdamEntry* table, int n_tensors, int64_t total_chunks,
                   float lr, float beta1, float beta2, float eps, float weight_decay,
                   float bias_correction1, float bias_correction2_sqrt, dcfp_stream_t stream);

typedef struct DcfpConvF16Desc {
    int32_t N, H, W;
    int32_t Cin8, x_pitch;
    int32_t Cout;
    int32_t K, stride, pad, dil;
    int32_t Hout, Wout;
    int32_t y_pitch, y_off;
    int32_t res_pitch, res_off;
    int32_t relu;
} DcfpConvF16Desc;
int dcfp_conv2d_fwd_f16_nhwc(const DcfpConvF16Desc* d, const void* x, const void* w_packed, const float* shift,
                             const void* residual , void* y, dcfp_stream_t stream);
// ... 145 lines not shown
```

Baseline: 12.32 images/s.

## Trim ragged Winograd tile grid and specialize edge regions by transform components

Adds a shared Winograd tile planner that sizes the tile grid to the valid output extent rather than rounding up to a multiple of 2*dilation. It also splits the tile space into up to four regions (full, last-row-half, last-column-half, corner). The fused forward/dgrad kernel dispatches region-specialized bodies that skip patch loads, transforms and MFMA groups for Winograd components that only feed discarded outputs. This cuts wasted tiles and work on dilated ASPP and backbone convs, but it adds per-block region selection, more template instantiations and register pressure. The cost model now uses the unreduced grid fraction for dispatch decisions.

Result: faster. 12.47 images/s, median of 6 (+1.2%).

```diff
diff --git a/dcfp_amd/_lib.py b/dcfp_amd/_lib.py
--- a/dcfp_amd/_lib.py
+++ b/dcfp_amd/_lib.py
@@ -126,6 +126,7 @@
     "dcfp_conv2d_pitch_supported": (_I, [_D]),
     "dcfp_conv2d_kernel_name": (_I, [_D, _I, C.c_char_p, _I]),
     "dcfp_conv2d_executed_fraction": (C.c_double, [_D, _I]),
+    "dcfp_wino_tile_plan": (_I, [_I, _I, _I, _I, _I, _I, C.POINTER(C.c_int64)]),
     "dcfp_conv2d_workspace_is_scratch": (_I, [_D, _I]),
     "dcfp_conv2d_dgrad_fanin_supported": (_I, [_D]),
     "dcfp_conv2d_dgrad_fanin_f32_nchw": (_I, [_D, _P, _L, _P, _P, _P, _P, _P, _Z, _I, _P]),
diff --git a/dcfp_amd/csrc/conv_dispatch.h b/dcfp_amd/csrc/conv_dispatch.h
--- a/dcfp_amd/csrc/conv_dispatch.h
+++ b/dcfp_amd/csrc/conv_dispatch.h
@@ -148,6 +148,7 @@
 bool dcfp_wino_ok(const WinoProblem& q);
 size_t dcfp_wino_workspace_bytes(const WinoProblem& q);
 double dcfp_wino_exec_fraction(const WinoProblem& q);
+double dcfp_wino_grid_fraction(const WinoProblem& q);
 long long dcfp_wino_stat_slots(const WinoProblem& q);
 size_t dcfp_wino_xform_bytes(const WinoProblem& q);
 int dcfp_wino_run(const GemmProblem& g, const float* in, const float* w, float* out, void* workspace, size_t workspace_bytes,
diff --git a/dcfp_amd/csrc/conv_igemm.hip b/dcfp_amd/csrc/conv_igemm.hip
--- a/dcfp_amd/csrc/conv_igemm.hip
+++ b/dcfp_amd/csrc/conv_igemm.hip
@@ -1,4 +1,5 @@
 #include "conv_dispatch.h"
+#include "wino_plan.h"
 #include <stdio.h>
 
 extern "C" int dcfp_abi_version(void) { return 2; }
@@ -20,7 +21,7 @@
     const double nominal = 2.0 * d->N * (double)d->H * d->W * (double)M * Ck * 9.0;
     const double f_direct = dcfp_igemm2_exec_fraction(g);
     const double t_direct = nominal * f_direct / (M % 256 != 0 ? 115e12 : 143e12);
-    const double f_wino = dcfp_wino_exec_fraction(q);
+    const double f_wino = dcfp_wino_grid_fraction(q);
     double t_wino = 1e30;
     if (three) {
         const double tiles = f_wino * 9.0 / 16.0 * d->N * (double)d->H * d->W;
@@ -100,6 +101,19 @@
     if (wino_pass(d, pass)) return dcfp_wino_exec_fraction(wino_problem(g));
     if (igemm3_ok(g)) return 1.0;
     return dcfp_igemm2_exec_fraction(g);
+}
+
+extern "C" int dcfp_wino_tile_plan(int N, int H, int W, int d, int ragged, int classes, int64_t* out) {
+    if (N <= 0 || H <= 0 || W <= 0 || d <= 0 || !out) return DCFP_E_BADDESC;
+    const WinoTilePlan pl = wino_tile_plan(N, H, W, d, ragged < 0 ? wino_ragged_on() : ragged != 0, classes != 0);
+    out[0] = pl.TH; out[1] = pl.TW; out[2] = pl.T; out[3] = pl.T16; out[4] = pl.nreg; out[5] = pl.tblocks;
+    for (int i = 0; i < pl.nreg; ++i) {
+        const WinoRegion& r = pl.reg[i];
+        int64_t* o = out + 6 + 8 * i;
+        o[0] = r.r0; o[1] = r.nr; o[2] = r.c0; o[3] = r.nc; o[4] = r.rows3; o[5] = r.cols3; o[6] = r.tb0; o[7] = r.nblocks;
+    }
+    out[38] = pl.issued;
+    return DCFP_OK;
 }
 
 extern "C" size_t dcfp_conv2d_xform_bytes(const DcfpConvDesc* d) {
diff --git a/dcfp_amd/csrc/conv_wgrad.hip b/dcfp_amd/csrc/conv_wgrad.hip
--- a/dcfp_amd/csrc/conv_wgrad.hip
+++ b/dcfp_amd/csrc/conv_wgrad.hip
@@ -897,7 +897,7 @@
 static bool wino_wgrad_fused_forced() { return wino_wgrad_fused_mode() == 2; }
 
 static double wino_fraction(const DcfpConvDesc* d) {
-    return dcfp_wino_exec_fraction(wino_problem(gemm_problem(d, DCFP_CONV_FWD, 0)));
+    return dcfp_wino_grid_fraction(wino_problem(gemm_problem(d, DCFP_CONV_FWD, 0)));
 }
 static int wino_wgrad_kind(const DcfpConvDesc* d) {
     const int mode = conv_winograd_mode();
@@ -935,7 +935,7 @@
 bool dcfp_wgrad_wants_xform(const DcfpConvDesc* d) { return wino_wgrad_kind(d) == 1; }
 
 double dcfp_wgrad_exec_fraction(const DcfpConvDesc* d) {
-    return wino_wgrad_pass(d) ? wino_fraction(d) : 1.0;
+    return wino_wgrad_pass(d) ? dcfp_wino_exec_fraction(wino_problem(gemm_problem(d, DCFP_CONV_FWD, 0))) : 1.0;
 }
 
 extern "C" size_t dcfp_conv2d_workspace_bytes(const DcfpConvDesc* d, int pass) {
diff --git a/dcfp_amd/csrc/conv_winograd.hip b/dcfp_amd/csrc/conv_winograd.hip
--- a/dcfp_amd/csrc/conv_winograd.hip
+++ b/dcfp_amd/csrc/conv_winograd.hip
@@ -1,5 +1,6 @@
 #include "igemm2_common.h"
 #include "conv_dispatch.h"
+#include "wino_plan.h"
 
 namespace {
 
@@ -15,11 +16,9 @@
 
 WinoPlan wino_plan(int N, int H, int W, int d, int M, int Ck) {
     WinoPlan pl;
-    pl.TH = d * ((H + 2 * d - 1) / (2 * d));
-    pl.TW = d * ((W + 2 * d - 1) / (2 * d));
-    pl.TW = (pl.TW + 3) / 4 * 4;
-    pl.T = (long long)N * pl.TH * pl.TW;
-    pl.T16 = (pl.T + 15) / 16 * 16;
+    const WinoTilePlan tp = wino_tile_plan(N, H, W, d, wino_ragged_on(), false);
+    pl.TH = tp.TH; pl.TW = tp.TW;
+    pl.T = tp.T; pl.T16 = tp.T16;
     pl.CkP = (Ck + dcfp_igemm2_ck_pad() - 1) / dcfp_igemm2_ck_pad() * dcfp_igemm2_ck_pad();
     pl.Mpad = (M + 255) / 256 * 256;
     pl.u_floats = align64(16LL * pl.CkP * pl.Mpad);
@@ -390,7 +389,7 @@
     if (!dcfp_igemm2_persist()) return false;
     if (q.M < 129 || q.Ck < 128) return false;
     const WinoPlan pl = wino_plan(q);
-    if (4 * pl.T > (long long)q.N * q.H * q.W * 27 / 20) return false;
+    if (4 * wino_tile_plan(q.N, q.H, q.W, q.d, false, false).T > (long long)q.N * q.H * q.W * 27 / 20) return false;
     if (pl.T16 >= (1LL << 26) || 16LL * pl.T16 >= (1LL << 30)) return false;
     if ((long long)q.Ck * pl.T16 >= (1LL << 29) || (long long)q.M * pl.T16 >= (1LL << 29)) return false;
     return dcfp_igemm2_dma_shape(batched_gemm(pl, q.M, q.Ck));
@@ -404,6 +403,9 @@
 double dcfp_wino_exec_fraction(const WinoProblem& q) {
     const WinoPlan pl = wino_plan(q);
     return 16.0 * (double)pl.T / (9.0 * (double)q.N * q.H * q.W);
+}
+double dcfp_wino_grid_fraction(const WinoProblem& q) {
+    return 16.0 * (double)wino_tile_plan(q.N, q.H, q.W, q.d, false, false).T / (9.0 * (double)q.N * q.H * q.W);
 }
 
 long long dcfp_wino_stat_slots(const WinoProblem& q) {
@@ -486,7 +488,7 @@
 bool dcfp_wino_wgrad_ok(int N, int H, int W, int d, int M, int C) {
     if (M < 128 || C < 128) return false;
     const WinoWgradPlan w = wino_wgrad_plan(N, H, W, d, M, C);
-    if (4 * w.pl.T > (long long)N * H * W * 27 / 20) return false;
+    if (4 * wino_tile_plan(N, H, W, d, false, false).T > (long long)N * H * W * 27 / 20) return false;
     if (w.T16 >= (1LL << 30) || (long long)M * w.T16 >= (1LL << 29) || (long long)C * w.T16 >= (1LL << 29)) return false;
     return M <= 65535 && C <= 65535;
 }
diff --git a/dcfp_amd/csrc/conv_winograd2.hip b/dcfp_amd/csrc/conv_winograd2.hip
--- a/dcfp_amd/csrc/conv_winograd2.hip
+++ b/dcfp_amd/csrc/conv_winograd2.hip
@@ -1,5 +1,6 @@
 #include "wino_patch.h"
 #include "conv_dispatch.h"
+#include "wino_plan.h"
 #include <stdlib.h>
 
 namespace {
@@ -23,8 +24,9 @@
     const float* shift;
     const float* residual;
     int relu;
-    int N, M, Ck, H, W, d, TH, TW;
-    long long T, T16;
+    int N, M, Ck, H, W, d;
+    long long T16;
+    struct Region { int tb0, r0, nr, c0, nc, cls; long long tiles; } reg[4];
     int mblocks, tblocks, nk;
     int accumulate;
     int ragged_c;
@@ -32,18 +34,39 @@
     unsigned out_bytes;
 };
 
-template <int DM, bool SIDE, bool RAGGED>
-__global__ void __launch_bounds__(256, 1) wino_fused_kernel(const WinoFusedParams p) {
+template <int DM, bool R3, bool S3> __device__ __forceinline__ constexpr bool patch_load_on(int I) {
+    if (DM == 4) return (R3 || (I >> 2) != 3) && (S3 || (I & 3) != 3);
+    return R3 || (I >> 1) != 3;
+}
+template <int DM, bool R3, bool S3> __device__ __forceinline__ constexpr int patch_loads() {
+    int n = 0;
+    for (int i = 0; i < PatchCfg<DM>::NV; ++i) n += patch_load_on<DM, R3, S3>(i) ? 1 : 0;
+    return n;
+}
+template <int DM, bool R3, bool S3> __device__ __forceinline__ constexpr int patch_load_nth(int j) {
+    for (int i = 0; i < PatchCfg<DM>::NV; ++i)
+        if (patch_load_on<DM, R3, S3>(i) && j-- == 0) return i;
+    return 0;
+}
+
+template <int DM, bool SIDE, bool RAGGED, bool R3, bool S3>
+__device__ __forceinline__ void wino_fused_body(const WinoFusedParams& p, const int mb, const int tb, const int tb0,
+                                                int r0, int nr, int c0, int nc, const long long rtiles) {
+    int tid = threadIdx.x;
+    asm volatile("" : "+s"(r0), "+s"(nr), "+s"(c0), "+s"(nc), "+v"(tid));
+    static_assert(!SIDE || (R3 && S3), "V is kept with all 16 components");
     constexpr int NV = PatchCfg<DM>::NV;
+    constexpr int NROWS = R3 ? 4 : 3, NCOLS = S3 ? 4 : 3, NC = NROWS * NCOLS;
+    constexpr int PW = S3 ? NC / 2 : 6;
+    constexpr int LS = NC == 16 ? 8 : NC == 12 ? 6 : 3, L0 = NC - LS;
+    constexpr int NVA = patch_loads<DM, R3, S3>();
+    static_assert(PW <= L0 && NROWS <= L0, "patch loads are issued behind the last LDS-DMA piece and the row transform");
     extern __shared__ __attribute__((aligned(16))) float smem[];
-    const int tid = threadIdx.x, lane = tid & 63, wid = tid >> 6, wm = wid >> 1, wn = wid & 1;
+    const int lane = tid & 63, wid = tid >> 6, wm = wid >> 1, wn = wid & 1;
     const int l31 = lane & 31, lhi = lane >> 5;
     const int wid_s = __builtin_amdgcn_readfirstlane(wid);
-    const int xcd = blockIdx.x & 7, jb = blockIdx.x >> 3;
-    const int mb = jb % p.mblocks, tb = (jb / p.mblocks) * 8 + xcd;
-    if (tb >= p.tblocks) return;
-    const long long t0 = (long long)tb * 64;
-    const int nk = p.nk, d = p.d, H = p.H, W = p.W, TW = p.TW, tpi = p.TH * p.TW, pitch = p.pitch;
+    const long long t0 = (long long)(tb - tb0) * 64;
+    const int nk = p.nk, d = p.d, H = p.H, W = p.W, tpi = nr * nc, pitch = p.pitch;
 
     const unsigned lds0 = (unsigned)(size_t)(lds_ptr)smem;
     const u32x4 a_desc = make_desc(p.ug, 0x7ffffffcu);
@@ -53,10 +76,10 @@
     const long long tp = t0 + 2 * l31;
     unsigned voff[NV];
     {
-        const bool tvalid = tp < p.T;
+        const bool tvalid = tp < rtiles;
         const long long tq = tvalid ? tp : 0;
         const int n = (int)(tq / tpi), tt = (int)(tq - (long long)n * tpi);
-        const int trow = tt / TW, tcol = tt - trow * TW;
+        const int trow = r0 + tt / nc, tcol = c0 + tt % nc;
         const int h0 = trow + d * (trow / d) - d, w0 = tcol + d * (tcol / d) - d;
         const long long base = (long long)n * p.in_nstride + (long long)lhi * H * pitch + p.lead;
 #pragma unroll
@@ -79,25 +102,26 @@
     const __amdgpu_buffer_rsrc_t in_rsrc = __builtin_amdgcn_make_buffer_rsrc(const_cast<float*>(p.in_base), 0,
                                                                              p.in_bytes, 0x00020000);
     const unsigned chan_bytes = (unsigned)(H * pitch) * 4u;
-    float R[2][4][8], q[4][8];
+    float R[2][4][8] = {}, q[4][8] = {};
     auto load_step = [&](int kt, auto b_) {
         constexpr int b = decltype(b_)::value;
         const unsigned soff = __builtin_amdgcn_readfirstlane((unsigned)(kt * FBK + 2 * wid_s) * chan_bytes);
+        unsigned vm[NV];
+#pragma unroll
+        for (int i = 0; i < NV; ++i) vm[i] = voff[i];
         if constexpr (RAGGED) {
-            unsigned vm[NV];
             const bool cok = kt * FBK + ch < p.Ck;
 #pragma unroll
             for (int i = 0; i < NV; ++i) vm[i] = cok ? voff[i] : kOob;
-            load_patches<DM>(in_rsrc, vm, soff, R[b]);
-        } else {
-            load_patches<DM>(in_rsrc, voff, soff, R[b]);
-        }
-    };
+        }
+        static_for<0, NVA>([&](auto j_) { load_one<DM, patch_load_nth<DM, R3, S3>(decltype(j_)::value)>(in_rsrc, vm, soff, R[b]); });
+    };
+    const int piece0 = S3 ? wid_s * PW : 8 * (wid_s < NROWS - 1 ? wid_s : NROWS - 1);
     auto issue_a = [&](int kt, int buf) {
         const unsigned abase = (unsigned)((kt * p.mblocks + mb) * FSTAGE) * 4u;
-        static_for<0, 8>([&](auto q_) {
+        static_for<0, PW>([&](auto q_) {
             constexpr int qq = decltype(q_)::value;
-            const unsigned piece = (unsigned)(wid_s * 8 + qq);
+            const unsigned piece = (unsigned)(piece0 + qq);
             const unsigned la = __builtin_amdgcn_readfirstlane(lds0 + (unsigned)(buf * 2 * FSTAGE) * 4u + piece * 1024u);
             const unsigned a_s = __builtin_amdgcn_readfirstlane(abase + piece * 1024u);
             const unsigned av = lane16;
@@ -111,13 +135,8 @@
         __builtin_amdgcn_s_barrier();
     };
     auto retire_keep_loads = [&](bool stored) {
-        if (SIDE && stored) {
-            if constexpr (NV == 8) asm volatile("s_waitcnt vmcnt(24) lgkmcnt(0)" ::: "memory");
-            else asm volatile("s_waitcnt vmcnt(32) lgkmcnt(0)" ::: "memory");
-        } else {
-            if constexpr (NV == 8) asm volatile("s_waitcnt vmcnt(8) lgkmcnt(0)" ::: "memory");
-            else asm volatile("s_waitcnt vmcnt(16) lgkmcnt(0)" ::: "memory");
-        }
+        if (SIDE && stored) asm volatile("s_waitcnt vmcnt(%0) lgkmcnt(0)" :: "n"(NVA + 16) : "memory");
+        else asm volatile("s_waitcnt vmcnt(%0) lgkmcnt(0)" :: "n"(NVA) : "memory");
         __builtin_amdgcn_s_barrier();
     };
     const long long vplane = (long long)p.Ck * p.T16;
@@ -150,13 +169,15 @@
         for (int r = 0; r < 16; ++r) acc[i][r] = 0.f;
 
     load_step(0, std::integral_constant<int, 0>{});
-    row_transform<DM>(R[0], q);
+    static_for<0, NROWS>([&](auto r_) { row_transform_one<DM, decltype(r_)::value>(R[0], q); });
     __builtin_amdgcn_sched_barrier(0);
     issue_a(0, 0);
     {
         const unsigned vs = side_off(0);
         const bool st = side_on(0);
-        static_for<0, 16>([&](auto xi_) {
+        static_for<0, NC>([&](auto k_) {
+            constexpr int k = decltype(k_)::value;
+            constexpr std::integral_constant<int, 4 * (k / NCOLS) + k % NCOLS> xi_{};
             const f32x2 o = produce(xi_, 0);
             if constexpr (SIDE) {
                 if (st) side_store(xi_, o, 0, vs);
@@ -194,23 +215,24 @@
         }
         const unsigned abase = (unsigned)(((kt + 1) * p.mblocks + mb) * FSTAGE) * 4u;
         f32x2 okeep[8];
-        static_for<0, 16>([&](auto g_) {
-            constexpr int g = decltype(g_)::value;
-            constexpr int fb = g & 1, pg = (g + 15) & 15;
-            af[fb] = *reinterpret_cast<const f32x4*>(As + g * 512);
-#pragma unroll
-            for (int kk = 0; kk < 4; ++kk) bf[fb][kk] = Bs[(g * FBK + 2 * kk) * 64];
+        static_for<0, NC>([&](auto g_) {
+            constexpr int g = decltype(g_)::value, gp = (g + NC - 1) % NC;
+            constexpr int xi = 4 * (g / NCOLS) + g % NCOLS, pg = 4 * (gp / NCOLS) + gp % NCOLS;
+            constexpr int fb = (g + cur * NC) & 1;
+            af[fb] = *reinterpret_cast<const f32x4*>(As + xi * 512);
+#pragma unroll
+            for (int kk = 0; kk < 4; ++kk) bf[fb][kk] = Bs[(xi * FBK + 2 * kk) * 64];
             f32x2 o = {0.f, 0.f};
             if constexpr (PROD) {
-                if constexpr (g < 4) {
+                if constexpr (g < NROWS) {
                     row_transform_one<DM, g>(R[rb], q);
 #pragma unroll
                     for (int c = 0; c < PatchCfg<DM>::NCOL; ++c) asm volatile("" : "+v"(q[g][c]));
                 }
-                o = col_transform<DM, g>(q);
+                o = col_transform<DM, xi>(q);
                 asm volatile("" : "+v"(o));
-                if constexpr (g < 8) {
-                    const unsigned piece = (unsigned)(wid_s * 8 + g);
+                if constexpr (g < PW) {
+                    const unsigned piece = (unsigned)(piece0 + g);
                     const unsigned la = __builtin_amdgcn_readfirstlane(lds0 + (unsigned)((cur ^ 1) * 2 * FSTAGE) * 4u + piece * 1024u);
                     const unsigned a_s = __builtin_amdgcn_readfirstlane(abase + piece * 1024u);
                     const unsigned av = lane16;
@@ -224,7 +246,7 @@
             acc[pg] = __builtin_amdgcn_mfma_f32_32x32x2f32(af[fb ^ 1][1], bf[fb ^ 1][1], acc[pg], 0, 0, 0);
             __builtin_amdgcn_sched_barrier(0);
             if constexpr (PROD) {
-                float* bs = smem + (cur ^ 1) * 2 * FSTAGE + FSTAGE + (g * FBK + ch) * 64 + 2 * l31;
+                float* bs = smem + (cur ^ 1) * 2 * FSTAGE + FSTAGE + (xi * FBK + ch) * 64 + 2 * l31;
                 *reinterpret_cast<f32x2*>(bs) = o;
                 if constexpr (SIDE) {
                     if constexpr (g < 8) okeep[g] = o;
@@ -237,9 +259,9 @@
             __builtin_amdgcn_sched_barrier(0);
             acc[pg] = __builtin_amdgcn_mfma_f32_32x32x2f32(af[fb ^ 1][2], bf[fb ^ 1][2], acc[pg], 0, 0, 0);
             __builtin_amdgcn_sched_barrier(0);
-            if constexpr (PROD && g >= 8) {
-                constexpr int per = NV / 8;
-                static_for<0, per>([&](auto j_) { load_one<DM, (g - 8) * per + decltype(j_)::value>(in_rsrc, vm, l_soff, R[rb]); });
+            if constexpr (PROD && g >= L0) {
+                constexpr int lo = (g - L0) * NVA / LS, hi = (g - L0 + 1) * NVA / LS;
+                static_for<lo, hi>([&](auto j_) { load_one<DM, patch_load_nth<DM, R3, S3>(decltype(j_)::value)>(in_rsrc, vm, l_soff, R[rb]); });
             }
             acc[pg] = __builtin_amdgcn_mfma_f32_32x32x2f32(af[fb ^ 1][3], bf[fb ^ 1][3], acc[pg], 0, 0, 0);
             __builtin_amdgcn_sched_barrier(0);
@@ -258,15 +280,16 @@
     step(std::true_type{}, even, nk - 2);
     retire();
     step(std::false_type{}, odd, nk - 1);
+    constexpr int xi_last = 4 * (NROWS - 1) + NCOLS - 1;
 #pragma unroll
     for (int kk = 0; kk < 4; ++kk)
-        acc[15] = __builtin_amdgcn_mfma_f32_32x32x2f32(af[1][kk], bf[1][kk], acc[15], 0, 0, 0);
+        acc[xi_last] = __builtin_amdgcn_mfma_f32_32x32x2f32(af[1][kk], bf[1][kk], acc[xi_last], 0, 0, 0);
 
     const long long te = t0 + wn * 32 + l31;
-    const bool tv = te < p.T;
+    const bool tv = te < rtiles;
     const long long tq = tv ? te : 0;
     const int n = (int)(tq / tpi), tt = (int)(tq - (long long)n * tpi);
-    const int trow = tt / TW, tcol = tt - trow * TW;
+    const int trow = r0 + tt / nc, tcol = c0 + tt % nc;
     const int ho = trow + d * (trow / d), wo = tcol + d * (tcol / d);
     const bool okr0 = tv && ho < H, okr1 = tv && ho + d < H;
     const bool okc0 = wo < W, okc1 = wo + d < W;
@@ -307,7 +330,7 @@
         const float mean = sum * (1.0f / 128.0f);
         const float d0 = o[0][0] - mean, d1 = o[0][1] - mean, d2 = o[1][0] - mean, d3 = o[1][1] - mean;
         const float m2 = red32((d0 * d0 + d1 * d1) + (d2 * d2 + d3 * d3));
-        if (l31 == 0 && m < p.M && t0 + wn * 32 < p.T) {
+        if (l31 == 0 && m < p.M && t0 + wn * 32 < rtiles) {
             float* sp = sp0 + (slot * p.M + m) * 2;
             sp[0] = mean; sp[1] = m2;
         }
@@ -378,8 +401,7 @@
             if (acc_out) v += __builtin_bit_cast(f32x4, __builtin_amdgcn_raw_buffer_load_b128(o_rsrc, vo, so, 0));
             __builtin_amdgcn_raw_buffer_store_b128(__builtin_bit_cast(u32x4, v), o_rsrc, vo, so, 0);
         });
-        return;
-    }
+    } else {
     float* obase = p.out + (long long)n * p.out_nstride + (long long)ho * W + wo;
     const long long dW = (long long)d * W;
 #pragma unroll
@@ -417,6 +439,30 @@
         }
         if (sp0) stats(m, o);
     }
+    }
+}
+
+template <int DM, bool SIDE, bool RAGGED>
+__global__ void __launch_bounds__(256, 1) wino_fused_kernel(const WinoFusedParams p) {
+    const int xcd = blockIdx.x & 7, jb = blockIdx.x >> 3;
+    const int mb = jb % p.mblocks, tb = (jb / p.mblocks) * 8 + xcd;
+    if (tb >= p.tblocks) return;
+    int tb0 = p.reg[0].tb0, r0 = p.reg[0].r0, nr = p.reg[0].nr, c0 = p.reg[0].c0, nc = p.reg[0].nc, cls = p.reg[0].cls;
+    long long tiles = p.reg[0].tiles;
+#pragma unroll
+    for (int i = 1; i < 4; ++i)
+        if (tb >= p.reg[i].tb0) {
+            tb0 = p.reg[i].tb0; r0 = p.reg[i].r0; nr = p.reg[i].nr; c0 = p.reg[i].c0; nc = p.reg[i].nc; cls = p.reg[i].cls;
+            tiles = p.reg[i].tiles;
+        }
+    if constexpr (SIDE) {
+        wino_fused_body<DM, true, RAGGED, true, true>(p, mb, tb, tb0, r0, nr, c0, nc, tiles);
+    } else {
+        if (cls == 3) wino_fused_body<DM, false, RAGGED, true, true>(p, mb, tb, tb0, r0, nr, c0, nc, tiles);
+        else if (cls == 2) wino_fused_body<DM, false, RAGGED, false, true>(p, mb, tb, tb0, r0, nr, c0, nc, tiles);
+        else if (cls == 1) wino_fused_body<DM, false, RAGGED, true, false>(p, mb, tb, tb0, r0, nr, c0, nc, tiles);
+        else wino_fused_body<DM, false, RAGGED, false, false>(p, mb, tb, tb0, r0, nr, c0, nc, tiles);
+    }
 }
 
 __global__ void __launch_bounds__(256) wino_filter2_kernel(const float* __restrict__ w, int sAm, int sAc, int flip, int M,
@@ -427,20 +473,18 @@
 }
 
 struct FusedPlan {
-    int TH, TW, mblocks, tblocks, nk, CkP, Mpad;
-    long long T, T16, ug_floats;
+    int mblocks, nk, CkP, Mpad;
+    long long tblocks, T16, ug_floats;
+    WinoTilePlan tiles;
 };
-FusedPlan fused_plan(int N, int H, int W, int d, int M, int Ck) {
+FusedPlan fused_plan(int N, int H, int W, int d, int M, int Ck, bool classes = true) {
     FusedPlan pl;
-    pl.TH = d * ((H + 2 * d - 1) / (2 * d));
-    pl.TW = d * ((W + 2 * d - 1) / (2 * d));
-    pl.TW = (pl.TW + 3) / 4 * 4;
-    pl.T = (long long)N * pl.TH * pl.TW;
-    pl.T16 = (pl.T + 15) / 16 * 16;
+    pl.tiles = wino_tile_plan(N, H, W, d, wino_ragged_on(), classes);
+    pl.T16 = pl.tiles.T16;
     pl.CkP = (Ck + 15) / 16 * 16;
     pl.Mpad = (M + 63) / 64 * 64;
     pl.mblocks = pl.Mpad / 64;
-    pl.tblocks = (int)((pl.T + 63) / 64);
+    pl.tblocks = pl.tiles.tblocks;
     pl.nk = pl.CkP / 8;
     pl.ug_floats = ((long long)16 * pl.CkP * pl.Mpad + 63) / 64 * 64;
     return pl;
@@ -462,7 +506,7 @@
     if (wino_fused_mode() == 0) return false;
     if (q.M < 48 || q.Ck < 48) return false;
     const FusedPlan pl = fused_plan(q.N, q.H, q.W, q.d, q.M, q.Ck);
-    if (pl.T16 >= (1LL << 30) || (long long)pl.tblocks * pl.mblocks + 8 * pl.mblocks >= (1LL << 31)) return false;
+    if (pl.T16 >= (1LL << 30) || pl.tblocks >= (1LL << 30) || pl.tblocks * pl.mblocks + 8 * pl.mblocks >= (1LL << 31)) return false;
     if ((long long)pl.CkP * pl.Mpad * 16 * 4 >= 0x7fffff00LL) return false;
     return fused_mode(q) >= 0;
 }
@@ -483,7 +527,7 @@
     const int flip = g.offstep < 0;
     const long long in_nstride = g.in_nstride, out_nstride = g.out_nstride;
     float* const xform_out = x.xform_out;
-    const FusedPlan pl = fused_plan(N, H, W, d, M, Ck);
+    const FusedPlan pl = fused_plan(N, H, W, d, M, Ck, !xform_out && !x.stat_part);
     if (!workspace || !dcfp_aligned16(workspace) || workspace_bytes < (size_t)pl.ug_floats * sizeof(float))
         return DCFP_E_WORKSPACE;
     const int pitch = q.in_pitch > 0 ? q.in_pitch : W;
@@ -509,9 +553,13 @@
     p.xform_out = xform_out;
     p.stat_part = x.stat_part;
     p.scale = x.scale; p.shift = x.shift; p.residual = x.residual; p.relu = x.relu;
-    p.N = N; p.M = M; p.Ck = Ck; p.H = H; p.W = W; p.d = d; p.TH = pl.TH; p.TW = pl.TW;
-    p.T = pl.T; p.T16 = pl.T16;
-    p.mblocks = pl.mblocks; p.tblocks = pl.tblocks; p.nk = pl.nk;
+    p.N = N; p.M = M; p.Ck = Ck; p.H = H; p.W = W; p.d = d;
+    p.T16 = pl.T16;
+    for (int i = 0; i < 4; ++i) {
+        const WinoRegion& r = pl.tiles.reg[i];
+        p.reg[i] = {r.tb0, r.r0, r.nr, r.c0, r.nc, (r.rows3 ? 1 : 0) | (r.cols3 ? 2 : 0), r.tiles};
+    }
+    p.mblocks = pl.mblocks; p.tblocks = (int)pl.tblocks; p.nk = pl.nk;
     p.accumulate = x.accumulate;
     p.ragged_c = (Ck % 16) != 0;
     {
@@ -522,7 +570,7 @@
         static const int no_vec = [] { const char* e = getenv("DCFP_WF_SCALAR_EPI"); return e ? atoi(e) : 0; }();
         if (no_vec) p.vec_epi = 0;
     }
-    const long long grid = (long long)((pl.tblocks + 7) / 8) * 8 * pl.mblocks;
+    const long long grid = (pl.tblocks + 7) / 8 * 8 * pl.mblocks;
     const size_t lds = (size_t)4 * FSTAGE * sizeof(float);
     auto launch = [&](auto kern) -> int {
         hipError_t e = hipFuncSetAttribute(reinterpret_cast<const void*>(kern), hipFuncAttributeMaxDynamicSharedMemorySize,
diff --git a/dcfp_amd/csrc/conv_winograd3.hip b/dcfp_amd/csrc/conv_winograd3.hip
--- a/dcfp_amd/csrc/conv_winograd3.hip
+++ b/dcfp_amd/csrc/conv_winograd3.hip
@@ -1,5 +1,6 @@
 #include "wino_patch.h"
 #include "conv_dispatch.h"
+#include "wino_plan.h"
 #include <stdlib.h>
 
 namespace {
@@ -366,11 +367,9 @@
 
 WgPlan wg_plan(int N, int H, int W, int d, int M, int C) {
     WgPlan pl;
-    pl.TH = d * ((H + 2 * d - 1) / (2 * d));
-    pl.TW = d * ((W + 2 * d - 1) / (2 * d));
-    pl.TW = (pl.TW + 3) / 4 * 4;
-    pl.T = (long long)N * pl.TH * pl.TW;
-    pl.T16 = (pl.T + 15) / 16 * 16;
+    const WinoTilePlan tp = wino_tile_plan(N, H, W, d, wino_ragged_on(), false);
+    pl.TH = tp.TH; pl.TW = tp.TW;
+    pl.T = tp.T; pl.T16 = tp.T16;
     pl.mblocks = (M + 63) / 64;
     pl.cblocks = (C + 63) / 64;
     const long long tiles = (long long)pl.mblocks * pl.cblocks, slots = dcfp_num_cus();
diff --git a/dcfp_amd/csrc/wino_plan.h b/dcfp_amd/csrc/wino_plan.h
--- /dev/null
+++ b/dcfp_amd/csrc/wino_plan.h
@@ -0,0 +1,72 @@
+#pragma once
+#include <stdlib.h>
+
+struct WinoAxis { int full, half, valid, grid; };
+
+inline WinoAxis wino_axis(int H, int d) {
+    const int k = (H + 2 * d - 1) / (2 * d) - 1;
+    auto clampd = [d](int v) { return v < 0 ? 0 : v > d ? d : v; };
+    WinoAxis a;
+    a.valid = k * d + clampd(H - 2 * k * d);
+    a.full = k * d + clampd(H - (2 * k + 1) * d);
+    a.half = a.valid - a.full;
+    a.grid = (k + 1) * d;
+    return a;
+}
+
+inline bool wino_ragged_on() {
+    static const bool v = [] { const char* e = getenv("DCFP_WINO_RAGGED"); return !e || atoi(e) != 0; }();
+    return v;
+}
+
+struct WinoRegion {
+    int r0, nr, c0, nc, rows3, cols3;
+    long long tiles;
+    int tb0, nblocks;
+    int components() const { return (rows3 ? 4 : 3) * (cols3 ? 4 : 3); }
+};
+
+struct WinoTilePlan {
+    int TH, TW;
+    long long T, T16;
+    WinoAxis rows, cols;
+    int nreg;
+    WinoRegion reg[4];
+    long long tblocks;
+    long long issued;
+};
+
+inline WinoTilePlan wino_tile_plan(int N, int H, int W, int d, bool ragged, bool classes) {
+    WinoTilePlan pl;
+    pl.rows = wino_axis(H, d);
+    pl.cols = wino_axis(W, d);
+    pl.TH = ragged ? pl.rows.valid : pl.rows.grid;
+    pl.TW = ((ragged ? pl.cols.valid : pl.cols.grid) + 3) / 4 * 4;
+    pl.T = (long long)N * pl.TH * pl.TW;
+    pl.T16 = (pl.T + 15) / 16 * 16;
+    int fr = pl.TH, fc = pl.TW;
+    if (ragged && classes) {
+        fr = pl.rows.full;
+        fc = (pl.cols.full + 3) / 4 * 4;
+        if (fc > pl.TW) fc = pl.TW;
+    }
+    const int rr[2][2] = {{0, fr}, {fr, pl.TH - fr}}, cc[2][2] = {{0, fc}, {fc, pl.TW - fc}};
+    const int order[4][2] = {{0, 0}, {1, 0}, {0, 1}, {1, 1}};
+    pl.nreg = 0;
+    pl.tblocks = 0;
+    pl.issued = 0;
+    for (int i = 0; i < 4; ++i) {
+        const int a = order[i][0], b = order[i][1];
+        if (rr[a][1] <= 0 || cc[b][1] <= 0) continue;
+        WinoRegion& g = pl.reg[pl.nreg++];
+        g.r0 = rr[a][0]; g.nr = rr[a][1]; g.c0 = cc[b][0]; g.nc = cc[b][1];
+        g.rows3 = a == 0; g.cols3 = b == 0;
+        g.tiles = (long long)N * g.nr * g.nc;
+        g.tb0 = (int)pl.tblocks;
+        g.nblocks = (int)((g.tiles + 63) / 64);
+        pl.tblocks += g.nblocks;
+        pl.issued += g.tiles * g.components();
+    }
+    for (int i = pl.nreg; i < 4; ++i) pl.reg[i] = WinoRegion{0, 0, 0, 0, 1, 1, 0, 0x7fffffff, 0};
+    return pl;
+}
diff --git a/include/dcfp_hip.h b/include/dcfp_hip.h
--- a/include/dcfp_hip.h
+++ b/include/dcfp_hip.h
@@ -71,6 +71,8 @@
 int dcfp_conv2d_kernel_name(const DcfpConvDesc* d, int pass, char* buf, int buf_len);
 
 double dcfp_conv2d_executed_fraction(const DcfpConvDesc* d, int pass);
+
+int dcfp_wino_tile_plan(int N, int H, int W, int d, int ragged, int classes, int64_t* out);
 
 int dcfp_conv2d_fwd_f32_nchw(const DcfpConvDesc* d, const float* x, const float* w,
                              const float* bias, float* y, int64_t y_nstride,
```
